# Rayhane-mamah/Tacotron-2

Measured on NVIDIA H100. Metric: wavenet_train_audio_samples_per_sec, higher is better.
Workload: dtype bf16

## Files before the change

### include/t2b200.h

```cpp
#ifndef T2B200_H_
#define T2B200_H_

#include <stdint.h>

#ifdef __cplusplus
extern "C" {
#endif

#define T2B200_ABI_VERSION 2

#define T2_OK 0
#define T2_ERR_INVALID_ARG (-1)
#define T2_ERR_UNSUPPORTED_SHAPE (-2)
#define T2_ERR_CUDA (-3)
#define T2_ERR_NCCL (-4)

const char* t2_last_error(void);
int t2_abi_version(void);
int t2_struct_size(const char* name);
long long t2_launch_count(void);

int t2_dbg_conv_gemm(const void* d_a, int B, int T, int C, int ld, const int* shifts, int nshift,
                     const void* d_w, int N, int BN, const float* d_bias, int relu, void* d_out_bf16,
                     float* d_out_f32, void* stream);
// ... 65 lines not shown
typedef struct {
  int layers, stacks, residual_channels, gate_channels, skip_out_channels, kernel_size;
  int cin_channels;
  int out_channels;
  int quantize_channels;
  int input_type;
  int legacy, residual_legacy;
  int upsample_type;
  int n_upsample;
  int upsample_scales[4];
  int freq_axis_kernel_size;
  float dropout;
  float log_scale_min;
  int B, T, Tc;
  int c_pre_upsampled;
  float log_scale_min_gauss;
  int cdf_loss;
  int split_bf16;
  int gin_channels;
  int n_speakers;
  int upsample_activation;
  float leaky_alpha;
} t2_wn_config_t;

typedef struct {
  long long n_params;
  long long packed_bytes;
  long long workspace_bytes;
  int n_tensors;
} t2_wn_sizes_t;

int t2_wn_sizes(const t2_wn_config_t* cfg, t2_wn_sizes_t* out);
int t2_wn_param_info(const t2_wn_config_t* cfg, int i, char* name, int name_cap, long long* offset, int* ndim,
                     int* shape4);
int t2_wn_init(const t2_wn_config_t* cfg, void* d_packed, void* d_workspace, void* stream);
int t2_wn_pack_weights(const t2_wn_config_t* cfg, const float* d_params, void* d_packed, void* d_workspace,
                       void* stream);
int t2_wn_forward(const t2_wn_config_t* cfg, const float* d_params, const void* d_packed, void* d_workspace,
                  const void* d_x, const float* d_c, const void* d_targets, const int* d_lengths, float* d_loss,
                  float* d_logits, int save_for_backward, unsigned long long seed,
                  const unsigned long long* d_step, void* stream);
int t2_wn_backward(const t2_wn_config_t* cfg, const float* d_params, const void* d_packed, void* d_workspace,
                   const void* d_x, const float* d_c, float* d_grads, unsigned long long seed,
                   const unsigned long long* d_step, void* stream);
int t2_wn_backward_phased(const t2_wn_config_t* cfg, const float* d_params, const void* d_packed, void* d_workspace,
                          const void* d_x, const float* d_c, float* d_grads, unsigned long long seed,
                          const unsigned long long* d_step, int phase, int n_groups, void* stream);
int t2_wn_time_kernel(const t2_wn_config_t* cfg, const float* d_params, const void* d_packed, void* d_workspace,
                      int which, int layer, int reps, float* ms_per_launch, void* stream);
int t2_wn_workspace_tensor(const t2_wn_config_t* cfg, void* d_workspace, const char* name, void** ptr,
                           long long* count, int* elem_bytes);
int t2_wn_set_speakers(const t2_wn_config_t* cfg, void* d_workspace, const int* d_speaker_ids, void* stream);
#define T2_DBG_WN_UP_FWD 1
#define T2_DBG_WN_UP_BWD_PARAM 2
#define T2_DBG_WN_UP_BWD_INPUT 3
int t2_dbg_wn_kernel(const t2_dbg_kernel_t* call, void* stream);


int t2_wn_ar_sizes(const t2_wn_config_t* cfg, int cluster_size, long long* packed_bytes, long long* workspace_bytes);
int t2_wn_ar_pack(const t2_wn_config_t* cfg, int cluster_size, const float* d_params, void* d_packed_ar,
                  void* d_workspace, void* stream);
int t2_wn_ar_generate(const t2_wn_config_t* cfg, int cluster_size, const float* d_params, const void* d_packed_ar,
                      void* d_workspace, const float* d_c, const void* d_initial, const void* d_test_inputs,
                      const float* d_u_a, const float* d_u_b, unsigned long long seed, void* d_out_samples,
                      float* d_out_raw, void* stream);
int t2_wn_ar_set_speakers(const t2_wn_config_t* cfg, int cluster_size, const float* d_params, const void* d_packed_ar,
                          void* d_workspace, const int* d_speaker_ids, void* stream);


typedef struct {
  int B, T_in, T_out;
  int n_symbols, num_mels, embedding_dim;
  int enc_conv_layers, enc_conv_kernel, enc_conv_channels, encoder_lstm_units;
  int attention_dim, attention_filters, attention_kernel;
  int prenet1, prenet2, decoder_lstm_units;
  int postnet_layers, postnet_kernel, postnet_channels;
  int clip_outputs;
  float dropout_rate;
  float zoneout_rate;
  float reg_weight;
  float max_abs_value, lower_bound_decay;
  int split_bf16;
  int mask_decoder;
  float cross_entropy_pos_weight;
  int unmasked_encoder;
  int noncumulative_weights;
  float teacher_forcing_ratio;
} t2_taco_config_t;

int t2_taco_sizes(const t2_taco_config_t* cfg, long long* n_params, long long* packed_bytes, long long* workspace_bytes,
                  int* n_tensors);
int t2_taco_param_info(const t2_taco_config_t* cfg, int i, char* name, int name_cap, long long* offset, int* ndim,
                       int* shape4, int* trainable);
int t2_taco_init(const t2_taco_config_t* cfg, void* d_packed, void* d_workspace, void* stream);
int t2_taco_pack_weights(const t2_taco_config_t* cfg, const float* d_params, void* d_packed, void* d_workspace, void* stream);
int t2_taco_forward(const t2_taco_config_t* cfg, float* d_params, const void* d_packed, void* d_workspace,
                    const int* d_inputs, const int* d_input_lengths, const float* d_mel_targets,
                    const float* d_stop_targets, float* d_loss, int training, unsigned long long seed,
                    const unsigned long long* d_step, void* stream);
int t2_taco_set_target_lengths(const t2_taco_config_t* cfg, void* d_workspace, const int* d_target_lengths, void* stream);
int t2_taco_backward(const t2_taco_config_t* cfg, const float* d_params, const void* d_packed, void* d_workspace,
                     const int* d_inputs, const int* d_input_lengths, const float* d_mel_targets,
                     const float* d_stop_targets, float* d_grads, unsigned long long seed,
                     const unsigned long long* d_step, void* stream);
int t2_taco_backward_ex(const t2_taco_config_t* cfg, const float* d_params, const void* d_packed, void* d_workspace,
                     const int* d_inputs, const int* d_input_lengths, const float* d_mel_targets,
                     const float* d_stop_targets, float* d_grads, const float* d_mel_outputs_grad, unsigned long long seed,
                     const unsigned long long* d_step, void* stream);
int t2_taco_infer_begin(const t2_taco_config_t* cfg, float* d_params, const void* d_packed, void* d_workspace,
                        const int* d_inputs, const int* d_input_lengths, void* stream);
int t2_taco_infer_steps(const t2_taco_config_t* cfg, float* d_params, const void* d_packed, void* d_workspace,
                        const int* d_input_lengths, int t_begin, int t_end, unsigned long long seed, void* stream);
int t2_taco_infer_finish(const t2_taco_config_t* cfg, float* d_params, const void* d_packed, void* d_workspace, int T_used,
                         void* stream);
int t2_rng_uniform_f32(unsigned long long seed, unsigned int stream_id, long long first_index, long long n, float* d_out,
                       void* stream);
int t2_dbg_att_stamps(long long* d_buf);
int t2_dbg_ar_stamps(long long* d_buf);
int t2_taco_workspace_tensor(const t2_taco_config_t* cfg, void* d_workspace, const char* name, void** ptr,
                             long long* count, int* elem_bytes);

typedef struct {
  int B, T;
  int num_mels;
  int kernels;
  int conv_channels;
  int pool_size;
  int projection;
  int projection_kernel_size;
  int highwaynet_layers;
  int highway_units;
  int rnn_units;
  int num_freq;
  int n_priority_freq;
  int clip_outputs, mask_decoder;
  float max_abs_value, lower_bound_decay, reg_weight;
} t2_cbhg_config_t;
int t2_cbhg_sizes(const t2_cbhg_config_t* cfg, long long* n_params, long long* packed_bytes, long long* workspace_bytes, int* n_tensors);
int t2_cbhg_param_info(const t2_cbhg_config_t* cfg, int i, char* name, int name_cap, long long* offset, int* ndim, int* shape4,
                       int* trainable);
int t2_cbhg_init(const t2_cbhg_config_t* cfg, void* d_packed, void* d_workspace, void* stream);
int t2_cbhg_pack_weights(const t2_cbhg_config_t* cfg, const float* d_params, void* d_packed, void* d_workspace, void* stream);
int t2_cbhg_set_target_lengths(const t2_cbhg_config_t* cfg, void* d_workspace, const int* d_target_lengths, void* stream);
int t2_cbhg_forward(const t2_cbhg_config_t* cfg, float* d_params, const void* d_packed, void* d_workspace, const float* d_mel,
                    const float* d_linear_targets, float* d_loss, int training, void* stream);
int t2_cbhg_backward(const t2_cbhg_config_t* cfg, const float* d_params, const void* d_packed, void* d_workspace, const float* d_mel,
                     float* d_grads, float* d_mel_grad, void* stream);
int t2_cbhg_workspace_tensor(const t2_cbhg_config_t* cfg, void* d_workspace, const char* name, void** ptr, long long* count);

int t2_adam_step(float* d_params, const float* d_grads, float* d_m, float* d_v, float* d_ema,
                 const long long* d_offsets, int n_tensors, long long n_total, float lr, float beta1, float beta2,
                 float eps, int step, float grad_scale, float max_norm, float max_value, float global_norm_clip,
                 float ema_decay, float* d_scratch, void* stream);

typedef struct {
  int sample_rate, n_fft, hop_size, win_size, num_mels;
  float fmin, fmax;
  float magnitude_power;
  float min_level_db, ref_level_db, max_abs_value;
  int symmetric_mels, allow_clipping_in_normalization, signal_normalization;
} t2_audio_config_t;

int t2_stft_mel_plan_bytes(const t2_audio_config_t* cfg, long long* bytes);
int t2_stft_mel_plan_init(const t2_audio_config_t* cfg, void* d_plan, void* stream);
int t2_stft_mel_frames(const t2_audio_config_t* cfg, int n_samples);
int t2_stft_mel_f32(const t2_audio_config_t* cfg, const void* d_plan, const float* d_wav, int B, int n_samples,
                    float preemphasis, float gain, float* d_mel, float* d_linear, int time_major, void* stream);
int t2_mel_basis_f64(const t2_audio_config_t* cfg, double* h_basis);
int t2_griffin_lim_bytes(const t2_audio_config_t* cfg, int B, int frames, long long* bytes);
int t2_griffin_lim_f32(const t2_audio_config_t* cfg, const void* d_plan, const float* d_mag, float* d_phase_io, int B, int frames,
                       int iters, unsigned long long seed, void* d_workspace, float* d_wav, void* stream);
int t2_preemphasis_f32(const float* d_x, float* d_y, int B, int n_samples, float k, void* stream);
int t2_mulaw_quantize_f32_i32(const float* d_in, int* d_out, long long n, void* stream);
int t2_inv_mulaw_quantize_i32_f32(const int* d_in, float* d_out, long long n, void* stream);
int t2_mulaw_f32(const float* d_in, float* d_out, long long n, void* stream);
int t2_inv_mulaw_f32(const float* d_in, float* d_out, long long n, void* stream);

#ifdef __cplusplus
}
#endif
#endif
```

### tacotron-2_b200/csrc/t2_common.cuh

```cuda
#pragma once
#include <cuda.h>
#include <cuda_bf16.h>
#include <cuda_runtime.h>
#include <stdint.h>

#define T2_OK 0
#define T2_ERR_INVALID_ARG (-1)
#define T2_ERR_UNSUPPORTED_SHAPE (-2)
#define T2_ERR_CUDA (-3)
#define T2_ERR_NCCL (-4)

int t2_set_error(int code, const char* fmt, ...);
void t2_count_launch(int n = 1);
#define T2_CHECK_CUDA(expr)                                                              \
  do {                                                                                   \
    cudaError_t _e = (expr);                                                             \
    if (_e != cudaSuccess)                                                               \
      return t2_set_error(T2_ERR_CUDA, "%s:%d %s -> %s", __FILE__, __LINE__, #expr,      \
                          cudaGetErrorString(_e));                                       \
  } while (0)
#define T2_REQUIRE(cond, code, ...)                                                      \
  do {                                                                                   \
    if (!(cond)) return t2_set_error(code, __VA_ARGS__);                                 \
  } while (0)

namespace t2 {

__device__ __forceinline__ uint32_t smem_u32(const void* p) {
  return static_cast<uint32_t>(__cvta_generic_to_shared(p));
}
__device__ __forceinline__ bool elect_one() {
  uint32_t pred = 0;
  asm volatile(
      "{\n\t.reg .pred P;\n\telect.sync _|P, 0xffffffff;\n\tselp.u32 %0, 1, 0, P;\n\t}\n"
      : "=r"(pred));
  return pred != 0;
}
__device__ __forceinline__ float warp_sum(float v) {
#pragma unroll
  for (int o = 16; o > 0; o >>= 1) v += __shfl_xor_sync(0xffffffffu, v, o);
  return v;
}
__device__ __forceinline__ float warp_max(float v) {
#pragma unroll
  for (int o = 16; o > 0; o >>= 1) v = fmaxf(v, __shfl_xor_sync(0xffffffffu, v, o));
  return v;
}
__device__ __forceinline__ float frcp_fast(float x) {
  float r;
  asm("rcp.approx.ftz.f32 %0, %1;" : "=f"(r) : "f"(x));
  return r;
}
__device__ __forceinline__ float sigmoidf_(float x) { return frcp_fast(1.f + __expf(-x)); }
__device__ __forceinline__ float tanhf_(float x) {
  const float e = __expf(-2.f * fabsf(x));
  const float t = (1.f - e) * frcp_fast(1.f + e);
  return copysignf(t, x);
}
__device__ __forceinline__ float tanh_approx_(float x) {
  float y;
  asm("tanh.approx.f32 %0, %1;" : "=f"(y) : "f"(x));
  return y;
}
__device__ __forceinline__ float sigmoid_approx_(float x) { return fmaf(0.5f, tanh_approx_(0.5f * x), 0.5f); }
__device__ __forceinline__ uint32_t pack_bf16x2(float lo, float hi) {
  __nv_bfloat162 v = __floats2bfloat162_rn(lo, hi);
  return *reinterpret_cast<uint32_t*>(&v);
}
__device__ __forceinline__ float bf16lo(uint32_t v) { return __uint_as_float(v << 16); }
__device__ __forceinline__ float bf16hi(uint32_t v) { return __uint_as_float(v & 0xffff0000u); }

__device__ __forceinline__ long long globaltimer_ns() {
  long long t;
  asm volatile("mov.u64 %0, %%globaltimer;" : "=l"(t));
  return t;
}
__device__ __forceinline__ long long smid() {
  unsigned int r;
  asm volatile("mov.u32 %0, %%smid;" : "=r"(r));
  return r;
}

__device__ __host__ __forceinline__ uint32_t hash_u32(uint64_t seed, uint64_t idx) {
  uint64_t z = seed + 0x9E3779B97F4A7C15ull * (idx + 1);
  z = (z ^ (z >> 30)) * 0xBF58476D1CE4E5B9ull;
  z = (z ^ (z >> 27)) * 0x94D049BB133111EBull;
  z = z ^ (z >> 31);
  return static_cast<uint32_t>(z >> 32);
}
__device__ __host__ __forceinline__ float hash_uniform(uint64_t seed, uint64_t idx) {
  return (hash_u32(seed, idx) >> 8) * (1.0f / 16777216.0f);
}
__device__ __host__ __forceinline__ uint32_t hash_seed(uint64_t seed, uint32_t stream) {
  return hash_u32(seed, stream);
}
__device__ __host__ __forceinline__ uint32_t hash_bits32(uint32_t hs, uint64_t idx) {
  uint32_t h = hs ^ (uint32_t(idx) * 0x9E3779B1u) ^ (uint32_t(idx >> 32) * 0x85EBCA77u);
  h ^= h >> 16; h *= 0x85EBCA6Bu; h ^= h >> 13; h *= 0xC2B2AE35u; h ^= h >> 16;
  return h;
}
__device__ __host__ __forceinline__ float hash_uniform32(uint32_t hs, uint64_t idx) {
  return (hash_bits32(hs, idx) >> 8) * (1.0f / 16777216.0f);
}
__device__ __host__ __forceinline__ bool hash_keep16(uint32_t hs, uint64_t idx, uint32_t thr16) {
  const uint32_t h = hash_bits32(hs, idx >> 1);
  return ((idx & 1) ? (h >> 16) : (h & 0xFFFFu)) >= thr16;
}

constexpr long long kFxPoison = -0x7fffffffffffffffll - 1;
constexpr long long kFxRange = 1ll << 62;
__device__ __forceinline__ bool fx_in_range(long long a) { return a > -kFxRange && a < kFxRange; }
struct FxAdd {
  unsigned long long* d;
  long long a, old;
};
__device__ __forceinline__ FxAdd fx_issue(long long* dst, float v) {
  FxAdd x{reinterpret_cast<unsigned long long*>(dst), 0, 0};
  if (!(fabsf(v) < 4194304.f)) {
    x.old = kFxPoison;
  } else {
    x.a = llrintf(v * 1099511627776.f);
    x.old = static_cast<long long>(atomicAdd(x.d, static_cast<unsigned long long>(x.a)));
  }
  return x;
}
__device__ __forceinline__ FxAdd fx_issue_total(long long* dst, long long v) {
  FxAdd x{reinterpret_cast<unsigned long long*>(dst), 0, kFxPoison};
  if (fx_in_range(v)) {
    x.a = v;
    x.old = static_cast<long long>(atomicAdd(x.d, static_cast<unsigned long long>(v)));
  }
  return x;
}
__device__ __forceinline__ void fx_check(const FxAdd& x) {
  if (!fx_in_range(x.old) || !fx_in_range(x.old + x.a)) atomicExch(x.d, static_cast<unsigned long long>(kFxPoison));
}
__device__ __forceinline__ void fx_add(long long* dst, float v) { fx_check(fx_issue(dst, v)); }
__device__ __forceinline__ float fx_value(long long a) {
  return fx_in_range(a) ? float(double(a) * (1.0 / 1099511627776.0)) : __int_as_float(0x7fffffff);
}
int launch_fx_finalize(const long long* acc, float* out, long long n, cudaStream_t st);

__device__ __forceinline__ void mbar_init(uint64_t* bar, uint32_t count) {
  asm volatile("mbarrier.init.shared::cta.b64 [%0], %1;\n" ::"r"(smem_u32(bar)), "r"(count));
}
__device__ __forceinline__ void fence_barrier_init() {
  asm volatile("fence.mbarrier_init.release.cluster;\n" ::: "memory");
}
__device__ __forceinline__ void fence_proxy_async() {
  asm volatile("fence.proxy.async.shared::cta;\n" ::: "memory");
}
__device__ __forceinline__ void mbar_expect_tx(uint64_t* bar, uint32_t bytes) {
  asm volatile("mbarrier.arrive.expect_tx.shared::cta.b64 _, [%0], %1;\n" ::"r"(smem_u32(bar)),
               "r"(bytes)
               : "memory");
}
__device__ __forceinline__ void mbar_arrive(uint64_t* bar) {
  asm volatile("mbarrier.arrive.shared::cta.b64 _, [%0];\n" ::"r"(smem_u32(bar)) : "memory");
}
__device__ __forceinline__ bool mbar_try_wait(uint64_t* bar, uint32_t parity) {
  uint32_t ok;
  asm volatile(
      "{\n\t.reg .pred P;\n\t"
      "mbarrier.try_wait.parity.shared::cta.b64 P, [%1], %2;\n\t"
      "selp.u32 %0, 1, 0, P;\n\t}\n"
      : "=r"(ok)
      : "r"(smem_u32(bar)), "r"(parity)
      : "memory");
  return ok != 0;
}
__device__ __forceinline__ void mbar_wait(uint64_t* bar, uint32_t parity) {
  while (!mbar_try_wait(bar, parity)) {
  }
}

__device__ __forceinline__ void tma_prefetch_desc(const CUtensorMap* m) {
  asm volatile("prefetch.tensormap [%0];\n" ::"l"(reinterpret_cast<uint64_t>(m)) : "memory");
}
__device__ __forceinline__ void tma_load_2d(void* smem, const CUtensorMap* m, uint64_t* bar, int c0,
                                            int c1) {
  asm volatile(
      "cp.async.bulk.tensor.2d.shared::cluster.global.tile.mbarrier::complete_tx::bytes "
      "[%0], [%1, {%3, %4}], [%2];\n" ::"r"(smem_u32(smem)),
      "l"(reinterpret_cast<uint64_t>(m)), "r"(smem_u32(bar)), "r"(c0), "r"(c1)
      : "memory");
}
__device__ __forceinline__ void tma_load_3d(void* smem, const CUtensorMap* m, uint64_t* bar, int c0,
                                            int c1, int c2) {
  asm volatile(
      "cp.async.bulk.tensor.3d.shared::cluster.global.tile.mbarrier::complete_tx::bytes "
      "[%0], [%1, {%3, %4, %5}], [%2];\n" ::"r"(smem_u32(smem)),
      "l"(reinterpret_cast<uint64_t>(m)), "r"(smem_u32(bar)), "r"(c0), "r"(c1), "r"(c2)
      : "memory");
}
__device__ __forceinline__ void tma_load_4d(void* smem, const CUtensorMap* m, uint64_t* bar, int c0,
                                            int c1, int c2, int c3) {
  asm volatile(
      "cp.async.bulk.tensor.4d.shared::cluster.global.tile.mbarrier::complete_tx::bytes "
      "[%0], [%1, {%3, %4, %5, %6}], [%2];\n" ::"r"(smem_u32(smem)),
      "l"(reinterpret_cast<uint64_t>(m)), "r"(smem_u32(bar)), "r"(c0), "r"(c1), "r"(c2), "r"(c3)
      : "memory");
}

__device__ __forceinline__ void tma_load_3d_mc(void* smem, const CUtensorMap* m, uint64_t* bar, int c0, int c1, int c2, uint16_t cta_mask) {
  asm volatile(
      "cp.async.bulk.tensor.3d.shared::cluster.global.tile.mbarrier::complete_tx::bytes.multicast::cluster "
      "[%0], [%1, {%3, %4, %5}], [%2], %6;\n" ::"r"(smem_u32(smem)),
      "l"(reinterpret_cast<uint64_t>(m)), "r"(smem_u32(bar)), "r"(c0), "r"(c1), "r"(c2), "h"(cta_mask)
      : "memory");
}
__device__ __forceinline__ void tma_store_3d(const CUtensorMap* m, const void* smem, int c0, int c1, int c2) {
  asm volatile("cp.async.bulk.tensor.3d.global.shared::cta.bulk_group [%0, {%2, %3, %4}], [%1];\n" ::"l"(reinterpret_cast<uint64_t>(m)),
               "r"(smem_u32(smem)), "r"(c0), "r"(c1), "r"(c2)
               : "memory");
}
__device__ __forceinline__ void bulk_commit() { asm volatile("cp.async.bulk.commit_group;\n" ::: "memory"); }
template <int N>
__device__ __forceinline__ void bulk_wait_read() { asm volatile("cp.async.bulk.wait_group.read %0;\n" ::"n"(N) : "memory"); }
__device__ __forceinline__ void bulk_wait_all() { asm volatile("cp.async.bulk.wait_group 0;\n" ::: "memory"); }
__device__ __forceinline__ void fence_proxy_async_smem() { asm volatile("fence.proxy.async.shared::cta;\n" ::: "memory"); }
__device__ __forceinline__ uint32_t mapa_cluster(const void* ptr, uint32_t rank) {
  uint32_t r;
  asm volatile("mapa.shared::cluster.u32 %0, %1, %2;" : "=r"(r) : "r"(smem_u32(ptr)), "r"(rank));
  return r;
}
__device__ __forceinline__ uint32_t cluster_ctarank() {
  uint32_t r;
  asm volatile("mov.u32 %0, %%cluster_ctarank;" : "=r"(r));
  return r;
}
__device__ __forceinline__ uint32_t cluster_nctarank() {
  uint32_t r;
  asm volatile("mov.u32 %0, %%cluster_nctarank;" : "=r"(r));
  return r;
}
__device__ __forceinline__ void cluster_sync_all() {
  asm volatile("barrier.cluster.arrive.release.aligned;\n" ::: "memory");
  asm volatile("barrier.cluster.wait.acquire.aligned;\n" ::: "memory");
}
__device__ __forceinline__ void mbar_arrive_cluster(uint64_t* bar, uint32_t rank) {
  asm volatile("mbarrier.arrive.release.cluster.shared::cluster.b64 _, [%0];\n" ::"r"(mapa_cluster(bar, rank)) : "memory");
}

__device__ __forceinline__ void bulk_load_1d(void* smem_dst, const void* gmem_src, uint32_t bytes, uint64_t* bar) {
  asm volatile("cp.async.bulk.shared::cluster.global.mbarrier::complete_tx::bytes [%0], [%1], %2, [%3];\n" ::"r"(smem_u32(smem_dst)),
               "l"(gmem_src), "r"(bytes), "r"(smem_u32(bar))
               : "memory");
}

__device__ __forceinline__ void pdl_wait() { asm volatile("griddepcontrol.wait;" ::: "memory"); }
__device__ __forceinline__ void pdl_launch_dependents() { asm volatile("griddepcontrol.launch_dependents;" ::: "memory"); }

__device__ __forceinline__ void wgmma_fence() { asm volatile("wgmma.fence.sync.aligned;\n" ::: "memory"); }
__device__ __forceinline__ void wgmma_commit() { asm volatile("wgmma.commit_group.sync.aligned;\n" ::: "memory"); }
template <int N>
__device__ __forceinline__ void wgmma_wait() { asm volatile("wgmma.wait_group.sync.aligned %0;\n" ::"n"(N) : "memory"); }
template <int R>
__device__ __forceinline__ void wgmma_fence_regs(float (&d)[R]) {
#pragma unroll
  for (int i = 0; i < R; ++i) asm volatile("" : "+f"(d[i])::"memory");
}
template <int N, int TA, int TB> struct Wgmma;
template <int TA, int TB>
struct Wgmma<16, TA, TB> {
  static __device__ __forceinline__ void mma(float (&d)[8], uint64_t da, uint64_t db, uint32_t scale_d) {
    asm volatile(
        "{\n.reg .pred p;\nsetp.ne.b32 p, %10, 0;\n"
        "wgmma.mma_async.sync.aligned.m64n16k16.f32.bf16.bf16 {"
        "%0, %1, %2, %3, %4, %5, %6, %7"
        "}, %8, %9, p, 1, 1, %11, %12;\n}\n"
        : "+f"(d[0]), "+f"(d[1]), "+f"(d[2]), "+f"(d[3]), "+f"(d[4]), "+f"(d[5]), "+f"(d[6]), "+f"(d[7])
        : "l"(da), "l"(db), "r"(scale_d), "n"(TA), "n"(TB));
  }
};
template <int TA, int TB>
struct Wgmma<64, TA, TB> {
  static __device__ __forceinline__ void mma(float (&d)[32], uint64_t da, uint64_t db, uint32_t scale_d) {
    asm volatile(
        "{\n.reg .pred p;\nsetp.ne.b32 p, %34, 0;\n"
        "wgmma.mma_async.sync.aligned.m64n64k16.f32.bf16.bf16 {"
        "%0, %1, %2, %3, %4, %5, %6, %7, %8, %9, %10, %11, %12, %13, %14, %15, "
        "%16, %17, %18, %19, %20, %21, %22, %23, %24, %25, %26, %27, %28, %29, %30, %31"
        "}, %32, %33, p, 1, 1, %35, %36;\n}\n"
        : "+f"(d[0]), "+f"(d[1]), "+f"(d[2]), "+f"(d[3]), "+f"(d[4]), "+f"(d[5]), "+f"(d[6]), "+f"(d[7]),
          "+f"(d[8]), "+f"(d[9]), "+f"(d[10]), "+f"(d[11]), "+f"(d[12]), "+f"(d[13]), "+f"(d[14]), "+f"(d[15]),
          "+f"(d[16]), "+f"(d[17]), "+f"(d[18]), "+f"(d[19]), "+f"(d[20]), "+f"(d[21]), "+f"(d[22]), "+f"(d[23]),
          "+f"(d[24]), "+f"(d[25]), "+f"(d[26]), "+f"(d[27]), "+f"(d[28]), "+f"(d[29]), "+f"(d[30]), "+f"(d[31])
        : "l"(da), "l"(db), "r"(scale_d), "n"(TA), "n"(TB));
  }
};
template <int TA, int TB>
struct Wgmma<128, TA, TB> {
  static __device__ __forceinline__ void mma(float (&d)[64], uint64_t da, uint64_t db, uint32_t scale_d) {
    asm volatile(
// ... 92 lines not shown
```

### tacotron-2_b200/csrc/t2_optim.cu

```cuda
#include "../../include/t2b200.h"
#include "t2_common.cuh"

namespace t2 {
namespace {

__device__ __forceinline__ int find_tensor(const long long* __restrict__ offs, int n, long long e) {
  int lo = 0, hi = n;
  while (hi - lo > 1) {
    const int mid = (lo + hi) >> 1;
    if (offs[mid] <= e) lo = mid; else hi = mid;
  }
  return lo;
}

__global__ void sumsq_kernel(const float* __restrict__ g, const long long* __restrict__ offs, int nt, long long n,
                             float gscale, float* __restrict__ norms) {
  const long long chunk = 4096;
  const long long e0 = blockIdx.x * chunk;
  const long long e1 = e0 + chunk < n ? e0 + chunk : n;
  int t = find_tensor(offs, nt, e0);
  float acc = 0.f;
  __shared__ float red[8];
  long long e = e0 + threadIdx.x;
  while (true) {
    const long long tend = offs[t + 1] < e1 ? offs[t + 1] : e1;
    acc = 0.f;
    for (; e < tend; e += blockDim.x) {
      const float v = g[e] * gscale;
      acc += v * v;
    }
    acc = warp_sum(acc);
    if ((threadIdx.x & 31) == 0) red[threadIdx.x >> 5] = acc;
    __syncthreads();
    if (threadIdx.x == 0) {
      float s = 0.f;
      for (int i = 0; i < (blockDim.x >> 5); ++i) s += red[i];
      if (s != 0.f) atomicAdd(norms + t, s);
    }
    __syncthreads();
    if (tend >= e1) break;
    ++t;
    e = offs[t] + threadIdx.x;
  }
}

struct AdamArgs {
  float* p; const float* g; float* m; float* v; float* ema;
  const long long* offs; int nt; long long n;
  float lr_t, b1, b2, eps, gscale, max_norm, max_value, gclip, ema_decay;
  const float* norms;
};
__global__ void adam_kernel(AdamArgs a) {
  const long long e = (blockIdx.x * (long long)blockDim.x + threadIdx.x) * 4;
  if (e >= a.n) return;
  float gs = a.gscale;
  if (a.gclip > 0.f) {
    gs *= a.gclip / fmaxf(sqrtf(a.norms[a.nt]), a.gclip);
  } else if (a.max_norm > 0.f) {
    const int t = find_tensor(a.offs, a.nt, e);
    gs *= a.max_norm / fmaxf(sqrtf(a.norms[t]), a.max_norm);
  }
  const float4 g4 = *reinterpret_cast<const float4*>(a.g + e);
  float4 m4 = *reinterpret_cast<const float4*>(a.m + e);
  float4 v4 = *reinterpret_cast<const float4*>(a.v + e);
  float4 p4 = *reinterpret_cast<const float4*>(a.p + e);
  float4 e4 = a.ema ? *reinterpret_cast<const float4*>(a.ema + e) : make_float4(0, 0, 0, 0);
  float* gp = const_cast<float*>(reinterpret_cast<const float*>(&g4));
  float* mp = reinterpret_cast<float*>(&m4);
  float* vp = reinterpret_cast<float*>(&v4);
  float* pp = reinterpret_cast<float*>(&p4);
  float* ep = reinterpret_cast<float*>(&e4);
#pragma unroll
  for (int i = 0; i < 4; ++i) {
    float g = gp[i] * gs;
    if (a.max_value > 0.f) g = fminf(fmaxf(g, -a.max_value), a.max_value);
    mp[i] = a.b1 * mp[i] + (1.f - a.b1) * g;
    vp[i] = a.b2 * vp[i] + (1.f - a.b2) * g * g;
    pp[i] = pp[i] - a.lr_t * mp[i] / (sqrtf(vp[i]) + a.eps);
    ep[i] -= (1.f - a.ema_decay) * (ep[i] - pp[i]);
  }
  *reinterpret_cast<float4*>(a.m + e) = m4;
  *reinterpret_cast<float4*>(a.v + e) = v4;
  *reinterpret_cast<float4*>(a.p + e) = p4;
  if (a.ema) *reinterpret_cast<float4*>(a.ema + e) = e4;
}
__global__ void total_kernel(float* norms, int nt) {
  float s = 0.f;
  for (int i = threadIdx.x; i < nt; i += 32) s += norms[i];
  s = warp_sum(s);
  if (threadIdx.x == 0) norms[nt] = s;
}

}
}

extern "C" int t2_adam_step(float* d_params, const float* d_grads, float* d_m, float* d_v, float* d_ema,
                            const long long* d_offsets, int n_tensors, long long n_total, float lr, float beta1,
                            float beta2, float eps, int step, float grad_scale, float max_norm, float max_value,
                            float global_norm_clip, float ema_decay, float* d_scratch, void* stream) {
  using namespace t2;
  T2_REQUIRE(d_params && d_grads && d_m && d_v && d_offsets && d_scratch, T2_ERR_INVALID_ARG, "adam: null pointer");
  T2_REQUIRE(step >= 1 && n_tensors >= 1 && n_total >= 1, T2_ERR_INVALID_ARG, "adam: bad step / sizes");
  cudaStream_t st = static_cast<cudaStream_t>(stream);
  const bool need_norms = max_norm > 0.f || global_norm_clip > 0.f;
  if (need_norms) {
    T2_CHECK_CUDA(cudaMemsetAsync(d_scratch, 0, (n_tensors + 1) * sizeof(float), st));
    sumsq_kernel<<<(unsigned)((n_total + 4095) / 4096), 256, 0, st>>>(d_grads, d_offsets, n_tensors, n_total, grad_scale, d_scratch); t2_count_launch();
    if (global_norm_clip > 0.f) total_kernel<<<1, 32, 0, st>>>(d_scratch, n_tensors); t2_count_launch();
  }
  AdamArgs a;
  a.p = d_params; a.g = d_grads; a.m = d_m; a.v = d_v; a.ema = d_ema; a.offs = d_offsets; a.nt = n_tensors; a.n = n_total;
  a.lr_t = float(double(lr) * sqrt(1.0 - pow(double(beta2), step)) / (1.0 - pow(double(beta1), step)));
  a.b1 = beta1; a.b2 = beta2; a.eps = eps; a.gscale = grad_scale; a.max_norm = max_norm; a.max_value = max_value;
  a.gclip = global_norm_clip; a.ema_decay = ema_decay; a.norms = d_scratch;
  T2_REQUIRE(n_total % 4 == 0, T2_ERR_INVALID_ARG, "adam: flat buffers must hold a multiple of 4 elements (16-byte aligned tensors)");
  adam_kernel<<<(unsigned)((n_total / 4 + 255) / 256), 256, 0, st>>>(a); t2_count_launch();
  T2_CHECK_CUDA(cudaGetLastError());
  return T2_OK;
}
```

### tacotron-2_b200/csrc/t2_wavenet.cu

```cuda
#include <stdlib.h>
#include <math.h>
#include <stdio.h>
#include <string.h>

#include <algorithm>
#include <string>
#include <vector>

#include "../../include/t2b200.h"
#include "t2_common.cuh"
#include "t2_gemm.h"

namespace t2 {
namespace {

typedef __nv_bfloat16 bf16;

struct PackJob {
  long long src_off;
  int K, N;
  long long dst_off;
  int dst_ld;
  int transpose;
  int col0;
  float scale;
  int perm_gh;
  int part;
};
struct ColsumJob {
  long long src_off;
  long long rows;
  int C, ld;
  long long dst_off, dst2_off;
  float scale;
  int div_scalar;
};

inline long long align_up(long long v, long long a) { return (v + a - 1) / a * a; }

struct ParamT {
  std::string name;
  long long off;
  int ndim;
  int shape[4];
};

struct Layout {
  t2_wn_config_t c;
  int L, R, G, Gh, S, C, O, Q, B, T, Tc, Kg, ldo, Op;
  bool split;
  int xm;
  bool scalar_in, mol, gauss;
  int Gi, NS;
  float res_scale;
  std::vector<float> skip_scale;
  std::vector<ParamT> params;
  long long n_params;
  long long p_in_k, p_in_b, p_f1_k, p_f1_b, p_f2_k, p_f2_b;
  std::vector<long long> p_dil_k, p_dil_b, p_c_k, p_c_b, p_s_k, p_s_b, p_o_k, p_o_b, p_up_k, p_up_b;
  std::vector<long long> p_g_k, p_g_b;
  long long p_emb;
  long long layer_stride;
  long long k_Wg, k_Wo, k_Ws, k_Wf1, k_Wf2, k_WozT, k_WdT, k_WcT, k_Wf1T, k_Wf2T, k_bias_g, k_bias_skip;
  long long packed_bytes;
  long long w_cup, w_x, w_xd, w_ta, w_sb, w_z, w_h1, w_h2, w_dlog, w_dh2, w_dskip, w_dxin, w_dg, w_dcup;
  long long w_skipsum;
  long long w_spk;
  long long w_gbias;
  long long w_gsum;
  long long w_gfx;
  long long w_upgrad[2], w_scalars, w_tiles_main, w_tiles_head, w_packjobs, w_colsum, w_tables;
  std::vector<long long> w_upout;
  std::vector<int> up_w;
  long long workspace_bytes;
  int n_tiles_main, n_tiles_head, n_packjobs, n_colsum;
  std::vector<PackJob> packjobs;
  std::vector<ColsumJob> colsums;
  std::vector<WgradTile> tiles_main, tiles_head;
  std::vector<int> tile_start;
  int dil(int l) const { return 1 << (l % (L / c.stacks)); }
};

long long add_param(Layout& lo, const std::string& name, std::initializer_list<int> shape) {
  ParamT p;
  p.name = name;
  p.off = lo.n_params;
  p.ndim = int(shape.size());
  long long n = 1;
  int i = 0;
  for (int s : shape) { p.shape[i++] = s; n *= s; }
  for (; i < 4; ++i) p.shape[i] = 1;
  lo.n_params += align_up(n, 4);
  lo.params.push_back(p);
  return p.off;
}

int build_layout(const t2_wn_config_t* cfg, Layout& lo) {
  T2_REQUIRE(cfg != nullptr, T2_ERR_INVALID_ARG, "null config");
  lo.c = *cfg;
  lo.L = cfg->layers; lo.R = cfg->residual_channels; lo.G = cfg->gate_channels; lo.Gh = lo.G / 2;
  lo.S = cfg->skip_out_channels; lo.C = cfg->cin_channels; lo.O = cfg->out_channels;
  lo.Q = cfg->quantize_channels; lo.B = cfg->B; lo.T = cfg->T; lo.Tc = cfg->Tc;
  lo.split = cfg->split_bf16 != 0;
  lo.xm = lo.split ? 2 : 1;
  T2_REQUIRE(!lo.split || cfg->dropout == 0.f, T2_ERR_INVALID_ARG, "split_bf16 (fp32-class forward) needs dropout = 0");
  lo.scalar_in = cfg->input_type != 2;
  lo.mol = lo.scalar_in;
  T2_REQUIRE(lo.L >= 1 && cfg->stacks >= 1 && lo.L % cfg->stacks == 0, T2_ERR_INVALID_ARG, "layers %% stacks != 0");
  T2_REQUIRE(cfg->kernel_size == 3, T2_ERR_UNSUPPORTED_SHAPE, "kernel_size must be 3");
  T2_REQUIRE(lo.R == 128 || lo.R == 256, T2_ERR_UNSUPPORTED_SHAPE, "residual_channels must be 128 or 256 (got %d)", lo.R);
  T2_REQUIRE(lo.S == 128 || lo.S == 256, T2_ERR_UNSUPPORTED_SHAPE, "skip_out_channels must be 128 or 256 (got %d)", lo.S);
  T2_REQUIRE(lo.Gh == 128 || lo.Gh == 256, T2_ERR_UNSUPPORTED_SHAPE, "gate_channels must be 256 or 512 (got %d)", lo.G);
  T2_REQUIRE(lo.C == 0 || (lo.C % 8 == 0 && lo.C <= 128), T2_ERR_UNSUPPORTED_SHAPE, "cin_channels must be 0 or a multiple of 8 <= 128");
  lo.gauss = lo.scalar_in && lo.O == 2;
  if (lo.mol) {
    T2_REQUIRE(lo.gauss || (lo.O % 3 == 0 && lo.O >= 3 && lo.O <= 30), T2_ERR_UNSUPPORTED_SHAPE,
               "scalar input needs out_channels = 2 (Gaussian) or 3 * nr_mix <= 30 (mixture of logistics), got %d", lo.O);
  } else {
    T2_REQUIRE(lo.O == 256 && lo.Q == 256, T2_ERR_UNSUPPORTED_SHAPE, "mulaw-quantize needs out_channels == quantize_channels == 256");
  }
  T2_REQUIRE(lo.B >= 1 && lo.T >= 1, T2_ERR_INVALID_ARG, "bad B/T");
  lo.Gi = cfg->gin_channels; lo.NS = cfg->n_speakers;
  T2_REQUIRE(lo.Gi >= 0 && (lo.Gi == 0 || lo.NS >= 1), T2_ERR_INVALID_ARG,
             "gin_channels must be >= 0, and n_speakers >= 1 when gin_channels > 0 (got %d / %d)", lo.Gi, lo.NS);
  T2_REQUIRE(cfg->upsample_type >= 0 && cfg->upsample_type <= 2, T2_ERR_INVALID_ARG,
             "upsample_type must be 0 (SubPixel), 1 (2D) or 2 (1D), got %d", cfg->upsample_type);
  T2_REQUIRE(cfg->upsample_activation >= 0 && cfg->upsample_activation <= 2, T2_ERR_INVALID_ARG,
             "upsample_activation must be 0 (ReLU), 1 (LeakyReLU) or 2 (none), got %d", cfg->upsample_activation);
  T2_REQUIRE(cfg->leaky_alpha >= 0.f && cfg->leaky_alpha <= 1.f, T2_ERR_INVALID_ARG, "leaky_alpha must be in [0, 1], got %g",
             double(cfg->leaky_alpha));
  lo.Kg = 3 * lo.R + (lo.C > 0 ? 128 : 0);
  lo.ldo = lo.mol ? 64 : 512;
  lo.Op = lo.mol ? 64 : 512;
  lo.res_scale = cfg->residual_legacy ? float(sqrt(0.5)) : 1.f;
  lo.skip_scale.resize(lo.L);
  for (int l = 0; l < lo.L; ++l) {
    int e = cfg->legacy ? (l == 0 ? lo.L - 1 : lo.L - l) : 0;
    lo.skip_scale[l] = float(pow(sqrt(0.5), e));
  }
  lo.up_w.clear();
  if (lo.C > 0 && !cfg->c_pre_upsampled) {
    T2_REQUIRE(cfg->n_upsample >= 1 && cfg->n_upsample <= 4, T2_ERR_INVALID_ARG, "n_upsample out of range");
    T2_REQUIRE(cfg->upsample_type == 2 || cfg->freq_axis_kernel_size == 3, T2_ERR_UNSUPPORTED_SHAPE,
               "freq_axis_kernel_size must be 3");
    for (int i = 0; i < cfg->n_upsample; ++i)
      T2_REQUIRE(cfg->upsample_scales[i] >= 1, T2_ERR_INVALID_ARG, "upsample_scales[%d] = %d < 1", i, cfg->upsample_scales[i]);
    int w = lo.Tc;
    for (int i = 0; i < cfg->n_upsample; ++i) { w *= cfg->upsample_scales[i]; lo.up_w.push_back(w); }
    T2_REQUIRE(w == lo.T, T2_ERR_INVALID_ARG, "Tc * prod(upsample_scales) = %d != T = %d", w, lo.T);
  }
  lo.n_params = 0;
  lo.params.clear();
  const int cin = lo.scalar_in ? 1 : lo.Q;
  lo.p_in_k = add_param(lo, "input_convolution/kernel", {1, cin, lo.R});
  lo.p_in_b = add_param(lo, "input_convolution/bias", {lo.R});
  for (int l = 0; l < lo.L; ++l) {
    char p[64];
    snprintf(p, sizeof(p), "ResidualConv1DGLU_%d/", l);
    std::string s(p);
    lo.p_dil_k.push_back(add_param(lo, s + "residual_block_causal_conv/kernel", {3, lo.R, lo.G}));
    lo.p_dil_b.push_back(add_param(lo, s + "residual_block_causal_conv/bias", {lo.G}));
    if (lo.C > 0) {
      lo.p_c_k.push_back(add_param(lo, s + "residual_block_cin_conv/kernel", {1, lo.C, lo.G}));
      lo.p_c_b.push_back(add_param(lo, s + "residual_block_cin_conv/bias", {lo.G}));
    }
    if (lo.Gi > 0) {
      lo.p_g_k.push_back(add_param(lo, s + "residual_block_gin_conv/kernel", {1, lo.Gi, lo.G}));
      lo.p_g_b.push_back(add_param(lo, s + "residual_block_gin_conv/bias", {lo.G}));
    }
    lo.p_s_k.push_back(add_param(lo, s + "residual_block_skip_conv/kernel", {1, lo.Gh, lo.S}));
    lo.p_s_b.push_back(add_param(lo, s + "residual_block_skip_conv/bias", {lo.S}));
    lo.p_o_k.push_back(add_param(lo, s + "residual_block_out_conv/kernel", {1, lo.Gh, lo.R}));
    lo.p_o_b.push_back(add_param(lo, s + "residual_block_out_conv/bias", {lo.R}));
  }
  lo.p_f1_k = add_param(lo, "final_convolution_1/kernel", {1, lo.S, lo.S});
  lo.p_f1_b = add_param(lo, "final_convolution_1/bias", {lo.S});
  lo.p_f2_k = add_param(lo, "final_convolution_2/kernel", {1, lo.S, lo.O});
  lo.p_f2_b = add_param(lo, "final_convolution_2/bias", {lo.O});
  lo.p_emb = lo.Gi > 0 ? add_param(lo, "gc_embedding", {lo.NS, lo.Gi}) : -1;
  lo.layer_stride = lo.L > 1 ? lo.p_dil_k[1] - lo.p_dil_k[0] : 0;
  for (size_t i = 0; i < lo.up_w.size(); ++i) {
    char p[64];
    snprintf(p, sizeof(p), "local_conditioning_upsampling_%d/", int(i) + 1);
    std::string s(p);
    const int sc = cfg->upsample_scales[i];
    if (cfg->upsample_type == 0) {
      lo.p_up_k.push_back(add_param(lo, s + "kernel", {3, 3, 1, sc}));
      lo.p_up_b.push_back(add_param(lo, s + "bias", {sc}));
    } else if (cfg->upsample_type == 2) {
      lo.p_up_k.push_back(add_param(lo, s + "kernel", {1, sc, lo.C, lo.C}));
      lo.p_up_b.push_back(add_param(lo, s + "bias", {lo.C}));
    } else {
      lo.p_up_k.push_back(add_param(lo, s + "kernel", {3, sc, 1, 1}));
      lo.p_up_b.push_back(add_param(lo, s + "bias", {1}));
    }
  }
  long long o = 0;
  auto takeb = [&](long long bytes) { long long r = o; o = align_up(o + bytes, 256); return r; };
  const long long L = lo.L;
  const long long km = lo.split ? 3 : 1;
  lo.k_Wg = takeb(L * lo.G * lo.Kg * km * 2);
  lo.k_Wo = takeb(L * lo.R * lo.Gh * km * 2);
  lo.k_Ws = takeb((long long)lo.S * L * lo.Gh * km * 2);
  lo.k_Wf1 = takeb((long long)lo.S * lo.S * km * 2);
  lo.k_Wf2 = takeb((long long)(lo.O < 32 ? 32 : lo.O) * lo.S * km * 2);
  lo.k_WozT = takeb(L * lo.Gh * (lo.R + lo.S) * 2);
  lo.k_WdT = takeb(L * lo.R * 3 * lo.G * 2);
  lo.k_WcT = takeb((long long)(lo.C > 0 ? lo.C : 8) * L * lo.G * 2);
  lo.k_Wf1T = takeb((long long)lo.S * lo.S * 2);
  lo.k_Wf2T = takeb((long long)lo.S * lo.Op * 2);
  lo.k_bias_g = takeb(L * lo.G * 4);
  lo.k_bias_skip = takeb(lo.S * 4);
  lo.packed_bytes = o;
  o = 0;
  const long long BT = (long long)lo.B * lo.T;
  lo.w_cup = takeb(BT * (lo.split ? 256 : (lo.C > 0 ? lo.C : 8)) * 2);
  lo.w_upout.clear();
  for (size_t i = 0; i < lo.up_w.size(); ++i) lo.w_upout.push_back(takeb((long long)lo.B * lo.C * lo.up_w[i] * 4));
  lo.w_upgrad[0] = takeb(BT * (lo.C > 0 ? lo.C : 8) * 4);
  lo.w_upgrad[1] = takeb(BT * (lo.C > 0 ? lo.C : 8) * 4);
  lo.w_x = takeb(L * BT * lo.R * 2 * lo.xm);
  lo.w_xd = cfg->dropout > 0.f ? takeb(L * BT * lo.R * 2) : lo.w_x;
  lo.w_ta = takeb(L * BT * lo.Gh * 2);
  lo.w_sb = takeb(L * BT * lo.Gh * 2);
  lo.w_z = takeb(L * BT * lo.Gh * 2 * lo.xm);
  lo.w_h1 = takeb(BT * lo.S * 2 * lo.xm);
  lo.w_h2 = takeb(BT * lo.S * 2 * lo.xm);
  lo.w_dlog = takeb(BT * lo.ldo * 2);
  lo.w_dh2 = takeb(BT * lo.S * 2);
  lo.w_dskip = takeb(BT * lo.S * 2);
  lo.w_dxin = takeb(L * BT * lo.R * 2);
  lo.w_dg = takeb(L * BT * lo.G * 2);
  lo.w_dcup = takeb(BT * (lo.C > 0 ? lo.C : 8) * 4);
  lo.w_scalars = takeb(64 * 4);
  lo.w_skipsum = takeb(lo.S * 8);
  lo.w_gfx = takeb(lo.n_params * 8);

  lo.packjobs.clear();
  auto pj = [&](long long src, int K, int N, long long dst_bytes, int ld, int transpose, int col0, float scale, int perm) {
    PackJob j; j.src_off = src; j.K = K; j.N = N; j.dst_off = dst_bytes / 2; j.dst_ld = ld; j.transpose = transpose;
    j.col0 = col0; j.scale = scale; j.perm_gh = perm; j.part = 0; lo.packjobs.push_back(j);
  };
  auto pj3 = [&](long long src, int K, int N, long long dst_bytes, int ld, int col_hi, int col_lo, int slot, float scale, int perm) {
    pj(src, K, N, dst_bytes, ld, 1, col_hi, scale, perm);
    pj(src, K, N, dst_bytes, ld, 1, col_hi + slot, scale, perm);
    pj(src, K, N, dst_bytes, ld, 1, col_lo, scale, perm);
    lo.packjobs.back().part = 2;
  };
  for (int l = 0; l < lo.L; ++l) {
    const long long wg = lo.k_Wg + (long long)l * lo.G * lo.Kg * km * 2;
    if (lo.split) {
      const int R = lo.R, Gh = lo.Gh;
      for (int j = 0; j < 3; ++j) pj3(lo.p_dil_k[l] + (long long)j * R * lo.G, R, lo.G, wg, 3 * lo.Kg, j * 3 * R, j * 3 * R + 2 * R, R, 1.f, Gh);
      if (lo.C > 0) pj3(lo.p_c_k[l], lo.C, lo.G, wg, 3 * lo.Kg, 9 * R, 9 * R + 256, 128, 1.f, Gh);
      pj3(lo.p_o_k[l], Gh, R, lo.k_Wo + (long long)l * R * Gh * 3 * 2, 3 * Gh, 0, 2 * Gh, Gh, 1.f, 0);
      pj3(lo.p_s_k[l], Gh, lo.S, lo.k_Ws, 3 * lo.L * Gh, l * 2 * Gh, 2 * lo.L * Gh + l * Gh, Gh, lo.skip_scale[l], 0);
    } else {
    for (int j = 0; j < 3; ++j) pj(lo.p_dil_k[l] + (long long)j * lo.R * lo.G, lo.R, lo.G, wg, lo.Kg, 1, j * lo.R, 1.f, lo.Gh);
    if (lo.C > 0) pj(lo.p_c_k[l], lo.C, lo.G, wg, lo.Kg, 1, 3 * lo.R, 1.f, lo.Gh);
    pj(lo.p_o_k[l], lo.Gh, lo.R, lo.k_Wo + (long long)l * lo.R * lo.Gh * 2, lo.Gh, 1, 0, 1.f, 0);
    pj(lo.p_s_k[l], lo.Gh, lo.S, lo.k_Ws, lo.L * lo.Gh, 1, l * lo.Gh, lo.skip_scale[l], 0);
    }
    const long long woz = lo.k_WozT + (long long)l * lo.Gh * (lo.R + lo.S) * 2;
    pj(lo.p_o_k[l], lo.Gh, lo.R, woz, lo.R + lo.S, 0, 0, lo.res_scale, 0);
    pj(lo.p_s_k[l], lo.Gh, lo.S, woz, lo.R + lo.S, 0, lo.R, lo.skip_scale[l], 0);
    const long long wd = lo.k_WdT + (long long)l * lo.R * 3 * lo.G * 2;
    for (int j = 0; j < 3; ++j) pj(lo.p_dil_k[l] + (long long)j * lo.R * lo.G, lo.R, lo.G, wd, 3 * lo.G, 0, j * lo.G, 1.f, 0);
    if (lo.C > 0) pj(lo.p_c_k[l], lo.C, lo.G, lo.k_WcT, lo.L * lo.G, 0, l * lo.G, 1.f, 0);
  }
  if (lo.split) {
    pj3(lo.p_f1_k, lo.S, lo.S, lo.k_Wf1, 3 * lo.S, 0, 2 * lo.S, lo.S, 1.f, 0);
    pj3(lo.p_f2_k, lo.S, lo.O, lo.k_Wf2, 3 * lo.S, 0, 2 * lo.S, lo.S, 1.f, 0);
  } else {
    pj(lo.p_f1_k, lo.S, lo.S, lo.k_Wf1, lo.S, 1, 0, 1.f, 0);
    pj(lo.p_f2_k, lo.S, lo.O, lo.k_Wf2, lo.S, 1, 0, 1.f, 0);
  }
  pj(lo.p_f1_k, lo.S, lo.S, lo.k_Wf1T, lo.S, 0, 0, 1.f, 0);
  pj(lo.p_f2_k, lo.S, lo.O, lo.k_Wf2T, lo.Op, 0, 0, 1.f, 0);
  if (!lo.mol) pj(lo.p_f2_k, lo.S, lo.O, lo.k_Wf2T, lo.Op, 0, 256, 1.f, 0);
  lo.n_packjobs = int(lo.packjobs.size());

  lo.tiles_main.clear();
  auto wt = [&](std::vector<WgradTile>& v, int am, int ach, int ash, int al, int bm, int bch, int bl, long long off,
                int ldc, int mv, int nv, float scale, const float* div) {
    WgradTile t; memset(&t, 0, sizeof(t));
    t.a_map = am; t.a_ch0 = ach; t.a_shift = ash; t.a_layer = al; t.b_map = bm; t.b_ch0 = bch; t.b_shift = 0; t.b_layer = bl;
    t.out_off = off; t.ldc = ldc; t.m_valid = mv; t.n_valid = nv; t.scale = scale; t.accumulate = 0; t.div = div;
    v.push_back(t);
  };
  const int WN = 256;
  auto nmin = [&](int rem) { return rem < WN ? rem : WN; };
  lo.tile_start.assign(lo.L + 1, 0);
  for (int l = 0; l < lo.L; ++l) {
    const int d = lo.dil(l);
    lo.tile_start[l] = int(lo.tiles_main.size());
    for (int j = 0; j < 3; ++j)
      for (int m0 = 0; m0 < lo.R; m0 += 128)
        for (int n0 = 0; n0 < lo.G; n0 += WN)
          wt(lo.tiles_main, 0, m0, -(2 - j) * d, l, 1, n0, l, lo.p_dil_k[l] + (long long)j * lo.R * lo.G + (long long)m0 * lo.G + n0,
             lo.G, 128, nmin(lo.G - n0), 1.f, nullptr);
    if (lo.C > 0)
      for (int n0 = 0; n0 < lo.G; n0 += WN)
        wt(lo.tiles_main, 2, 0, 0, 0, 1, n0, l, lo.p_c_k[l] + n0, lo.G, lo.C, nmin(lo.G - n0), 1.f, nullptr);
    for (int m0 = 0; m0 < lo.Gh; m0 += 128) {
      if (l < lo.L - 1)
        for (int n0 = 0; n0 < lo.R; n0 += WN)
          wt(lo.tiles_main, 3, m0, 0, l, 4, n0, l + 1, lo.p_o_k[l] + (long long)m0 * lo.R + n0, lo.R, 128, nmin(lo.R - n0), lo.res_scale, nullptr);
      for (int n0 = 0; n0 < lo.S; n0 += WN)
        wt(lo.tiles_main, 3, m0, 0, l, 5, n0, 0, lo.p_s_k[l] + (long long)m0 * lo.S + n0, lo.S, 128, nmin(lo.S - n0), lo.skip_scale[l], nullptr);
    }
  }
  lo.tiles_head.clear();
  for (int m0 = 0; m0 < lo.S; m0 += 128) {
    for (int n0 = 0; n0 < lo.S; n0 += WN)
      wt(lo.tiles_head, 0, m0, 0, 0, 1, n0, 0, lo.p_f1_k + (long long)m0 * lo.S + n0, lo.S, 128, nmin(lo.S - n0), 1.f, nullptr);
    for (int n0 = 0; n0 < lo.O; n0 += WN)
      for (int part = 0; part < (lo.mol ? 1 : 2); ++part) {
        wt(lo.tiles_head, 2, m0, 0, 0, 3, part * 256 + n0, 0, lo.p_f2_k + (long long)m0 * lo.O + n0, lo.O, 128,
           nmin(lo.O - n0), 1.f, reinterpret_cast<const float*>(1) );
        lo.tiles_head.back().accumulate = 2;
      }
  }
  lo.n_tiles_main = int(lo.tiles_main.size());
  lo.tile_start[lo.L] = lo.n_tiles_main;
  lo.n_tiles_head = int(lo.tiles_head.size());

  lo.colsums.clear();
  auto cs = [&](long long src, long long rows, int C, int ld, long long dst, long long dst2, float scale, int div) {
    ColsumJob j; j.src_off = src; j.rows = rows; j.C = C; j.ld = ld; j.dst_off = dst; j.dst2_off = dst2; j.scale = scale;
    j.div_scalar = div; lo.colsums.push_back(j);
  };
  cs(lo.w_dlog, BT, lo.O, lo.ldo, lo.p_f2_b, -1, 1.f, 1);
  if (!lo.mol) cs(lo.w_dlog + 256 * 2, BT, lo.O, lo.ldo, lo.p_f2_b, -1, 1.f, 1);
  lo.n_colsum = int(lo.colsums.size());

  lo.w_tiles_main = takeb((long long)lo.n_tiles_main * sizeof(WgradTile));
  lo.w_tiles_head = takeb((long long)lo.n_tiles_head * sizeof(WgradTile));
  lo.w_packjobs = takeb((long long)lo.n_packjobs * sizeof(PackJob));
  lo.w_colsum = takeb((long long)lo.n_colsum * sizeof(ColsumJob));
  lo.w_tables = takeb((long long)lo.L * (3 * sizeof(long long) + sizeof(float)));
  lo.w_spk = lo.w_gbias = lo.w_gsum = -1;
  if (lo.Gi > 0) {
    lo.w_spk = takeb((1LL + lo.B) * 4);
    lo.w_gbias = takeb(L * lo.B * lo.G * 4);
    lo.w_gsum = takeb(L * lo.B * lo.G * 8);
  }
  lo.workspace_bytes = o;
  return T2_OK;
}

__global__ void pack_kernel(const float* __restrict__ params, bf16* __restrict__ packed, const PackJob* __restrict__ jobs) {
  __shared__ float tile[64][65];
  const PackJob j = jobs[blockIdx.y];
  const int tiles_n = (j.N + 63) / 64, tiles_k = (j.K + 63) / 64;
  const int tx = threadIdx.x, ty = threadIdx.y;
  const bool vec_src = ((j.N | int(j.src_off)) & 1) == 0;
  const bool vec_dst = ((j.dst_ld | j.col0 | int(j.dst_off)) & 1) == 0;
  for (int ti = blockIdx.x; ti < tiles_n * tiles_k; ti += gridDim.x) {
    const int k0 = (ti / tiles_n) * 64, n0 = (ti % tiles_n) * 64;
    for (int r = ty; r < 64; r += 8) {
      const int k = k0 + r, n = n0 + 2 * tx;
      float a = 0.f, b = 0.f;
      if (k < j.K) {
        const float* src = params + j.src_off + (long long)k * j.N + n;
        if (vec_src && n + 1 < j.N) { const float2 v = *reinterpret_cast<const float2*>(src); a = v.x; b = v.y; }
        else { if (n < j.N) a = src[0]; if (n + 1 < j.N) b = src[1]; }
      }
      a *= j.scale; b *= j.scale;
      if (j.part == 2) { a -= __bfloat162float(__float2bfloat16(a)); b -= __bfloat162float(__float2bfloat16(b)); }
      tile[r][2 * tx] = a; tile[r][2 * tx + 1] = b;
    }
    __syncthreads();
    if (j.transpose) {
      for (int r = ty; r < 64; r += 8) {
        const int n = n0 + r, k = k0 + 2 * tx;
        if (n < j.N && k < j.K) {
          int row = n;
          if (j.perm_gh > 0) {
            const int half = n / j.perm_gh, idx = n % j.perm_gh;
            row = (idx / 128) * 256 + half * 128 + (idx % 128);
          }
          bf16* dst = packed + j.dst_off + (long long)row * j.dst_ld + j.col0 + k;
          if (vec_dst && k + 1 < j.K) *reinterpret_cast<uint32_t*>(dst) = pack_bf16x2(tile[2 * tx][r], tile[2 * tx + 1][r]);
          else { dst[0] = __float2bfloat16(tile[2 * tx][r]); if (k + 1 < j.K) dst[1] = __float2bfloat16(tile[2 * tx + 1][r]); }
        }
      }
    } else {
      for (int r = ty; r < 64; r += 8) {
        const int k = k0 + r, n = n0 + 2 * tx;
        if (n < j.N && k < j.K) {
          bf16* dst = packed + j.dst_off + (long long)k * j.dst_ld + j.col0 + n;
          if (vec_dst && n + 1 < j.N) *reinterpret_cast<uint32_t*>(dst) = pack_bf16x2(tile[r][2 * tx], tile[r][2 * tx + 1]);
          else { dst[0] = __float2bfloat16(tile[r][2 * tx]); if (n + 1 < j.N) dst[1] = __float2bfloat16(tile[r][2 * tx + 1]); }
        }
      }
    }
    __syncthreads();
  }
}

struct DerivedArgs {
  const float* params;
  float* bias_g;
  float* bias_skip;
  const long long* offs;
  const float* scales;
  int L, G, S;
};
__global__ void derived_bias_kernel(DerivedArgs a) {
  const int i = blockIdx.x * blockDim.x + threadIdx.x;
  if (i < a.L * a.G) {
    const int l = i / a.G, g = i % a.G;
    float v = a.params[a.offs[3 * l] + g];
    if (a.offs[3 * l + 1] >= 0) v += a.params[a.offs[3 * l + 1] + g];
    a.bias_g[i] = v;
  }
  if (i < a.S) {
    float v = 0.f;
    for (int l = 0; l < a.L; ++l) v += a.scales[l] * a.params[a.offs[3 * l + 2] + i];
    a.bias_skip[i] = v;
  }
}

struct GinArgs {
  const float* params;
  const float* bias;
  long long bias_ld;
  const int* on;
  const int* ids;
  float* out;
  long long out_l, out_b;
  long long p_k, p_b, p_stride, p_emb;
  int L, B, G, Gi, NS;
};
__global__ void gin_bias_kernel(GinArgs a) {
  const long long i = blockIdx.x * (long long)blockDim.x + threadIdx.x;
  if (i >= (long long)a.L * a.B * a.G) return;
  const int g = int(i % a.G), b = int((i / a.G) % a.B), l = int(i / ((long long)a.G * a.B));
  float v = a.bias[l * a.bias_ld + g];
  if (a.ids && (!a.on || *a.on)) {
    const int id = a.ids[b];
    float s = __int_as_float(0x7fffffff);
    if (id >= 0 && id < a.NS) {
      const float* W = a.params + a.p_k + l * a.p_stride + g;
      const float* e = a.params + a.p_emb + (long long)id * a.Gi;
      s = a.params[a.p_b + l * a.p_stride + g];
      for (int k = 0; k < a.Gi; ++k) s += W[(long long)k * a.G] * e[k];
    }
    v += s;
  }
  a.out[l * a.out_l + b * a.out_b + g] = v;
}
__global__ void set_speakers_kernel(int* __restrict__ spk, const int* __restrict__ ids, int B) {
  const int i = blockIdx.x * blockDim.x + threadIdx.x;
  if (i == 0) spk[0] = ids != nullptr;
  if (ids && i < B) spk[1 + i] = ids[i];
}
struct GinGradArgs {
  const float* params;
  const int* spk;
  const long long* S;
  long long* gfx;
  float* grads;
  const long long* offs;
  long long p_k, p_b, p_stride, p_emb;
  int L, B, G, Gi, NS;
};
__global__ void gin_wgrad_kernel(GinGradArgs a) {
  const int i = blockIdx.x * blockDim.x + threadIdx.x;
  if (i >= a.L * a.G) return;
  const int l = i / a.G, g = i % a.G;
  const long long* S = a.S + (long long)l * a.B * a.G + g;
  long long tot = 0;
  bool poison = false;
  for (int b = 0; b < a.B; ++b) {
    const long long s = S[(long long)b * a.G];
    if (!fx_in_range(s)) poison = true;
    else if (!fx_in_range(tot += s)) poison = true;
  }
  if (poison) tot = kFxPoison;
  a.gfx[a.offs[3 * l] + g] = tot;
  if (a.offs[3 * l + 1] >= 0) a.gfx[a.offs[3 * l + 1] + g] = tot;
  if (!a.spk[0]) return;
  a.gfx[a.p_b + l * a.p_stride + g] = tot;
  float* dW = a.grads + a.p_k + l * a.p_stride + g;
  for (int k = 0; k < a.Gi; ++k) {
    float acc = 0.f;
    for (int b = 0; b < a.B; ++b) {
      const int id = a.spk[1 + b];
      const float e = (id >= 0 && id < a.NS) ? a.params[a.p_emb + (long long)id * a.Gi + k] : __int_as_float(0x7fffffff);
      acc += e * fx_value(S[(long long)b * a.G]);
    }
    dW[(long long)k * a.G] = acc;
  }
}
constexpr int kGinThreads = 256;
__global__ void __launch_bounds__(kGinThreads) gin_demb_kernel(GinGradArgs a) {
  __shared__ float red[kGinThreads];
  if (!a.spk[0]) return;
  const int s = blockIdx.x, k = blockIdx.y, tid = threadIdx.x;
  {
    float acc = 0.f;
    for (int b = 0; b < a.B; ++b) {
      if (a.spk[1 + b] != s) continue;
      float part = 0.f;
      for (int l = 0; l < a.L; ++l) {
        const float* W = a.params + a.p_k + l * a.p_stride + (long long)k * a.G;
        const long long* S = a.S + ((long long)l * a.B + b) * a.G;
        for (int g = tid; g < a.G; g += kGinThreads) part += W[g] * fx_value(S[g]);
      }
      red[tid] = part;
      __syncthreads();
      for (int h = kGinThreads / 2; h > 0; h >>= 1) {
        if (tid < h) red[tid] += red[tid + h];
        __syncthreads();
      }
      if (tid == 0) acc += red[0];
      __syncthreads();
    }
    if (tid == 0) a.grads[a.p_emb + (long long)s * a.Gi + k] = acc;
  }
}

__global__ void first_conv_kernel(const void* __restrict__ xin, int scalar_in, const float* __restrict__ W,
                                  const float* __restrict__ bias, bf16* __restrict__ x, bf16* __restrict__ xd,
                                  long long npos, int R, float p, unsigned long long seed,
                                  const unsigned long long* __restrict__ step, int split) {
  if (step) seed += *step;
  const long long e8 = blockIdx.x * (long long)blockDim.x + threadIdx.x;
  const int R8 = R >> 3;
  if (e8 >= npos * R8) return;
  const long long pos = e8 / R8;
  const int r = int(e8 % R8) * 8;
  float v[8];
  const float4 b0 = __ldg(reinterpret_cast<const float4*>(bias + r)), b1 = __ldg(reinterpret_cast<const float4*>(bias + r + 4));
  if (scalar_in) {
    const float xv = static_cast<const float*>(xin)[pos];
    const float4 w0 = __ldg(reinterpret_cast<const float4*>(W + r)), w1 = __ldg(reinterpret_cast<const float4*>(W + r + 4));
    v[0] = xv * w0.x + b0.x; v[1] = xv * w0.y + b0.y; v[2] = xv * w0.z + b0.z; v[3] = xv * w0.w + b0.w;
    v[4] = xv * w1.x + b1.x; v[5] = xv * w1.y + b1.y; v[6] = xv * w1.z + b1.z; v[7] = xv * w1.w + b1.w;
  } else {
    const float* row = W + (long long)static_cast<const int*>(xin)[pos] * R + r;
    const float4 w0 = __ldg(reinterpret_cast<const float4*>(row)), w1 = __ldg(reinterpret_cast<const float4*>(row + 4));
    v[0] = w0.x + b0.x; v[1] = w0.y + b0.y; v[2] = w0.z + b0.z; v[3] = w0.w + b0.w;
    v[4] = w1.x + b1.x; v[5] = w1.y + b1.y; v[6] = w1.z + b1.z; v[7] = w1.w + b1.w;
  }
  const long long e = pos * R + r;
  uint4 o;
  if (split) {
    float hi[8], lo8[8];
#pragma unroll
    for (int j = 0; j < 8; ++j) { hi[j] = __bfloat162float(__float2bfloat16(v[j])); lo8[j] = v[j] - hi[j]; }
    o.x = pack_bf16x2(hi[0], hi[1]); o.y = pack_bf16x2(hi[2], hi[3]); o.z = pack_bf16x2(hi[4], hi[5]); o.w = pack_bf16x2(hi[6], hi[7]);
    *reinterpret_cast<uint4*>(x + pos * 2 * R + r) = o;
    o.x = pack_bf16x2(lo8[0], lo8[1]); o.y = pack_bf16x2(lo8[2], lo8[3]); o.z = pack_bf16x2(lo8[4], lo8[5]); o.w = pack_bf16x2(lo8[6], lo8[7]);
    *reinterpret_cast<uint4*>(x + pos * 2 * R + R + r) = o;
    return;
  }
  o.x = pack_bf16x2(v[0], v[1]); o.y = pack_bf16x2(v[2], v[3]); o.z = pack_bf16x2(v[4], v[5]); o.w = pack_bf16x2(v[6], v[7]);
  *reinterpret_cast<uint4*>(x + e) = o;
  if (xd != x && xd != nullptr) {
    const float keep_inv = 1.f / (1.f - p);
    const uint32_t hs = hash_seed(seed, 0u), thr = uint32_t(p * 65536.f);
#pragma unroll
    for (int j = 0; j < 8; ++j) v[j] = hash_keep16(hs, (unsigned long long)(e + j), thr) ? v[j] * keep_inv : 0.f;
    o.x = pack_bf16x2(v[0], v[1]); o.y = pack_bf16x2(v[2], v[3]); o.z = pack_bf16x2(v[4], v[5]); o.w = pack_bf16x2(v[6], v[7]);
    *reinterpret_cast<uint4*>(xd + e) = o;
  }
}
__global__ void first_conv_bwd_kernel(const void* __restrict__ xin, int scalar_in, const bf16* __restrict__ dx0,
                                      long long* __restrict__ dW, long long npos, int R) {
  const int r = threadIdx.x;
  const long long p0 = (long long)blockIdx.x * 64;
  if (scalar_in) {
    float acc = 0.f;
    for (int i = 0; i < 64 && p0 + i < npos; ++i)
      acc += static_cast<const float*>(xin)[p0 + i] * __bfloat162float(dx0[(p0 + i) * R + r]);
    fx_add(dW + r, acc);
  } else {
    const int n = npos - p0 < 64 ? int(npos - p0) : 64;
    for (int i0 = 0; i0 < n; i0 += 8) {
      FxAdd x[8];
#pragma unroll
      for (int i = 0; i < 8; ++i)
        if (i0 + i < n)
          x[i] = fx_issue(dW + (long long)static_cast<const int*>(xin)[p0 + i0 + i] * R + r, __bfloat162float(dx0[(p0 + i0 + i) * R + r]));
#pragma unroll
      for (int i = 0; i < 8; ++i)
        if (i0 + i < n) fx_check(x[i]);
    }
  }
}

__global__ void colsum_kernel(const uint8_t* __restrict__ ws, long long* __restrict__ grads, const ColsumJob* __restrict__ jobs,
                              const float* __restrict__ scalars) {
  const ColsumJob j = jobs[blockIdx.y];
  const bf16* src = reinterpret_cast<const bf16*>(ws + j.src_off);
  const long long rows_per = (j.rows + gridDim.x - 1) / gridDim.x;
  const long long r0 = blockIdx.x * rows_per;
  const long long r1 = r0 + rows_per < j.rows ? r0 + rows_per : j.rows;
  float sc = j.scale;
  if (j.div_scalar >= 0) sc /= fmaxf(scalars[j.div_scalar], 1e-20f);
  for (int c = 2 * threadIdx.x; c < j.C; c += 2 * blockDim.x) {
    float a0 = 0.f, a1 = 0.f;
    long long r = r0;
    for (; r + 4 <= r1; r += 4) {
      uint32_t u[4];
#pragma unroll
      for (int i = 0; i < 4; ++i) u[i] = __ldg(reinterpret_cast<const uint32_t*>(src + (r + i) * j.ld + c));
#pragma unroll
      for (int i = 0; i < 4; ++i) { a0 += bf16lo(u[i]); a1 += bf16hi(u[i]); }
    }
    for (; r < r1; ++r) {
      const uint32_t u = __ldg(reinterpret_cast<const uint32_t*>(src + r * j.ld + c));
      a0 += bf16lo(u); a1 += bf16hi(u);
    }
    a0 *= sc; a1 *= sc;
    const bool two = c + 1 < j.C, dup = j.dst2_off >= 0;
    FxAdd x[4];
    x[0] = fx_issue(grads + j.dst_off + c, a0);
    if (two) x[1] = fx_issue(grads + j.dst_off + c + 1, a1);
    if (dup) {
      x[2] = fx_issue(grads + j.dst2_off + c, a0);
      if (two) x[3] = fx_issue(grads + j.dst2_off + c + 1, a1);
    }
    fx_check(x[0]);
    if (two) fx_check(x[1]);
    if (dup) {
      fx_check(x[2]);
      if (two) fx_check(x[3]);
    }
  }
}

__device__ __forceinline__ float up_act(float x, int act, float alpha) {
  return act == 0 ? fmaxf(x, 0.f) : act == 1 ? fmaxf(alpha * x, x) : x;
}
// ... 209 lines not shown
        const float v = up_act(bias[co] + acc[k], act, alpha);
        out[((long long)b * C + co) * Wo + xo] = v;
        if (out_cl && split) {
          const bf16 hi = __float2bfloat16(v);
          bf16* row = out_cl + ((long long)b * Wo + xo) * 256;
          row[co] = hi;
          row[128 + co] = __float2bfloat16(v - __bfloat162float(hi));
        } else if (out_cl) out_cl[((long long)b * Wo + xo) * C + co] = __float2bfloat16(v);
      }
    }
  }
}
__global__ void __launch_bounds__(kUp1Tw * kUp1Rows) up1d_bwd_input_kernel(const float* __restrict__ out, const float* __restrict__ dout,
                                                                          const float* __restrict__ K, float* __restrict__ din, int C, int W,
                                                                          int s, int act, float alpha) {
  extern __shared__ float sm[];
  float* kt = sm;
  float* gs = sm + C * C;
  const int tx = threadIdx.x, ty = threadIdx.y, tid = ty * kUp1Tw + tx;
  const int w0 = blockIdx.x * kUp1Tw, b = blockIdx.y;
  const int nw = min(kUp1Tw, W - w0);
  const long long Wo = (long long)W * s;
  float acc[kUp1MaxK];
#pragma unroll
  for (int k = 0; k < kUp1MaxK; ++k) acc[k] = 0.f;
  for (int j = 0; j < s; ++j) {
    __syncthreads();
    const float* Kj = K + (long long)j * C * C;
    for (int e = tid; e < C * C; e += kUp1Tw * kUp1Rows) kt[e] = Kj[(e % C) * C + e / C];
    for (int e = tid; e < C * kUp1Tw; e += kUp1Tw * kUp1Rows) {
      const int co = e / kUp1Tw, t = e % kUp1Tw;
      float g = 0.f;
      if (t < nw) {
        const long long i = ((long long)b * C + co) * Wo + (long long)(w0 + t) * s + j;
        g = up_dact(out[i], dout[i], act, alpha);
      }
      gs[e] = g;
    }
    __syncthreads();
    if ((C & 3) == 0) {
      for (int co = 0; co < C; co += 4) {
        const float g0 = gs[co * kUp1Tw + tx], g1 = gs[(co + 1) * kUp1Tw + tx], g2 = gs[(co + 2) * kUp1Tw + tx], g3 = gs[(co + 3) * kUp1Tw + tx];
#pragma unroll
        for (int k = 0; k < kUp1MaxK; ++k) {
          const int ci = ty + kUp1Rows * k;
          if (ci < C) {
            const float4 kv = *reinterpret_cast<const float4*>(kt + ci * C + co);
            acc[k] = fmaf(kv.x, g0, acc[k]); acc[k] = fmaf(kv.y, g1, acc[k]); acc[k] = fmaf(kv.z, g2, acc[k]); acc[k] = fmaf(kv.w, g3, acc[k]);
          }
        }
      }
    } else {
      for (int co = 0; co < C; ++co) {
        const float g = gs[co * kUp1Tw + tx];
#pragma unroll
        for (int k = 0; k < kUp1MaxK; ++k) {
          const int ci = ty + kUp1Rows * k;
          if (ci < C) acc[k] = fmaf(kt[ci * C + co], g, acc[k]);
        }
      }
    }
  }
  if (tx < nw) {
#pragma unroll
    for (int k = 0; k < kUp1MaxK; ++k) {
      const int ci = ty + kUp1Rows * k;
      if (ci < C) din[((long long)b * C + ci) * W + w0 + tx] = acc[k];
    }
  }
}
constexpr int kUp1MaxM = 4;
inline size_t up1d_param_smem(int C) { return sizeof(float) * 2 * kUp1Tw * size_t(C + 1); }
__global__ void __launch_bounds__(kUp1Tw * kUp1Rows) up1d_bwd_param_kernel(const float* __restrict__ in, const float* __restrict__ out,
                                                                          const float* __restrict__ dout, long long* __restrict__ dK,
                                                                          long long* __restrict__ dbias, int B, int C, int W, int s, int act,
                                                                          float alpha) {
  extern __shared__ float sm[];
  const int ld = C + 1;
  float* xs = sm;
  float* gs = sm + kUp1Tw * ld;
  const int tx = threadIdx.x, ty = threadIdx.y, tid = ty * kUp1Tw + tx;
  const int j = blockIdx.x;
  const long long npos = (long long)B * W, Wo = (long long)W * s;
  const long long nchunk = (npos + kUp1Tw - 1) / kUp1Tw;
  float acc[kUp1MaxM][kUp1MaxK];
#pragma unroll
  for (int m = 0; m < kUp1MaxM; ++m)
#pragma unroll
    for (int k = 0; k < kUp1MaxK; ++k) acc[m][k] = 0.f;
  float bsum = 0.f;
  for (long long ch = blockIdx.y; ch < nchunk; ch += gridDim.y) {
    __syncthreads();
    for (int e = tid; e < C * kUp1Tw; e += kUp1Tw * kUp1Rows) {
      const int c = e / kUp1Tw, t = e % kUp1Tw;
      const long long p = ch * kUp1Tw + t;
      float x = 0.f, g = 0.f;
      if (p < npos) {
        const long long b = p / W, w = p % W;
        x = in[(b * C + c) * W + w];
        const long long i = (b * C + c) * Wo + w * s + j;
        g = up_dact(out[i], dout[i], act, alpha);
      }
      xs[t * ld + c] = x;
      gs[t * ld + c] = g;
    }
    __syncthreads();
    if (tid < C)
      for (int t = 0; t < kUp1Tw; ++t) bsum += gs[t * ld + tid];
    for (int t = 0; t < kUp1Tw; ++t) {
      float x[kUp1MaxM];
#pragma unroll
      for (int m = 0; m < kUp1MaxM; ++m) x[m] = tx + kUp1Tw * m < C ? xs[t * ld + tx + kUp1Tw * m] : 0.f;
#pragma unroll
      for (int k = 0; k < kUp1MaxK; ++k) {
        const int co = ty + kUp1Rows * k;
        if (co < C) {
          const float g = gs[t * ld + co];
#pragma unroll
          for (int m = 0; m < kUp1MaxM; ++m) acc[m][k] = fmaf(g, x[m], acc[m][k]);
        }
      }
    }
  }
  long long* dKj = dK + (long long)j * C * C;
#pragma unroll
  for (int k = 0; k < kUp1MaxK; ++k) {
    const int co = ty + kUp1Rows * k;
    if (co >= C) continue;
    FxAdd xa[kUp1MaxM];
#pragma unroll
    for (int m = 0; m < kUp1MaxM; ++m) {
      const int ci = tx + kUp1Tw * m;
      if (ci < C && acc[m][k] != 0.f) xa[m] = fx_issue(dKj + (long long)co * C + ci, acc[m][k]);
    }
#pragma unroll
    for (int m = 0; m < kUp1MaxM; ++m) {
      const int ci = tx + kUp1Tw * m;
      if (ci < C && acc[m][k] != 0.f) fx_check(xa[m]);
    }
  }
  if (tid < C && bsum != 0.f) fx_add(dbias + tid, bsum);
}
__global__ void skip_bias_kernel(const long long* __restrict__ skipsum, float* __restrict__ grads, const long long* __restrict__ offs,
                                 const float* __restrict__ scales, int L, int S) {
  const int i = blockIdx.x * blockDim.x + threadIdx.x;
  if (i >= L * S) return;
  const int l = i / S, s = i % S;
  grads[offs[3 * l + 2] + s] = scales[l] * fx_value(skipsum[s]);
}
__global__ void fx_finalize_kernel(const long long* __restrict__ acc, float* __restrict__ grads, long long n) {
  const long long e = blockIdx.x * (long long)blockDim.x + threadIdx.x;
  if (e < n && acc[e] != 0) grads[e] += fx_value(acc[e]);
}
__global__ void f32_to_bf16_kernel(const float* __restrict__ in, bf16* __restrict__ out, long long n) {
  const long long e = blockIdx.x * (long long)blockDim.x + threadIdx.x;
  if (e < n) out[e] = __float2bfloat16(in[e]);
}

ActGemmCall make_gate_call(const Layout& lo, uint8_t* ws, const uint8_t* pk, int l, bool save) {
  const long long BT = (long long)lo.B * lo.T;
  const int d = lo.dil(l);
  ActGemmCall g;
  memset(&g, 0, sizeof(g));
  if (lo.split) {
    g.a[0] = make_act(ws + lo.w_xd, 2 * lo.R, lo.T, lo.B, lo.L);
    g.a[1] = make_act(ws + lo.w_cup, 256, lo.T, lo.B, 1);
    g.na = lo.C > 0 ? 2 : 1;
    const int shifts[3] = {-2 * d, -d, 0};
    g.nseg = 0;
    for (int j = 0; j < 3; ++j) {
      g.seg[g.nseg++] = Seg{0, shifts[j], 0, 2 * lo.R / kBK, l, 1};
      g.seg[g.nseg++] = Seg{0, shifts[j], 0, lo.R / kBK, l, 1};
    }
    if (lo.C > 0) { g.seg[g.nseg++] = Seg{1, 0, 0, 4, 0, 1}; g.seg[g.nseg++] = Seg{1, 0, 0, 2, 0, 1}; }
    g.w = pk + lo.k_Wg; g.wN = lo.G; g.wK = 3 * lo.Kg; g.wL = lo.L; g.w_layer = l; g.w_k0 = 0;
  } else {
  g.a[0] = make_act(ws + lo.w_xd, lo.R, lo.T, lo.B, lo.L);
  g.a[1] = make_act(ws + lo.w_cup, lo.C > 0 ? lo.C : 8, lo.T, lo.B, 1);
  g.na = lo.C > 0 ? 2 : 1;
  g.seg[0] = Seg{0, -2 * d, 0, lo.R / kBK, l, 1};
  g.seg[1] = Seg{0, -d, 0, lo.R / kBK, l, 1};
  g.seg[2] = Seg{0, 0, 0, lo.R / kBK, l, 1};
  g.nseg = 3;
  if (lo.C > 0) { g.seg[3] = Seg{1, 0, 0, 2, 0, 1}; g.nseg = 4; }
  g.w = pk + lo.k_Wg; g.wN = lo.G; g.wK = lo.Kg; g.wL = lo.L; g.w_layer = l; g.w_k0 = 0;
  }
  g.T = lo.T; g.B = lo.B; g.n_tiles = lo.G / 256;
  const long long lofs = (long long)l * BT * lo.Gh;
  g.epi.ptr[0] = save ? reinterpret_cast<bf16*>(ws + lo.w_ta) + lofs : nullptr;
  g.epi.ptr[1] = save ? reinterpret_cast<bf16*>(ws + lo.w_sb) + lofs : nullptr;
  g.epi.ptr[2] = reinterpret_cast<bf16*>(ws + lo.w_z) + lofs * lo.xm;
  g.epi.i[11] = lo.split ? 1 : 0;
  g.epi.ptr[3] = const_cast<float*>(reinterpret_cast<const float*>(pk + lo.k_bias_g) + (long long)l * lo.G);
  if (lo.Gi > 0) {
    g.epi.ptr[3] = reinterpret_cast<float*>(ws + lo.w_gbias) + (long long)l * lo.B * lo.G;
    g.epi.i[2] = lo.G;
  }
  g.epi.i[0] = lo.Gh;
  return g;
}

ActGemmCall make_out_call(const Layout& lo, uint8_t* ws, const uint8_t* pk, const float* params, int l, float p,
                          unsigned long long seed, const unsigned long long* d_step) {
  const long long BT = (long long)lo.B * lo.T;
  bf16* x_all = reinterpret_cast<bf16*>(ws + lo.w_x);
  bf16* xd_all = reinterpret_cast<bf16*>(ws + lo.w_xd);
  ActGemmCall o;
  memset(&o, 0, sizeof(o));
  o.a[0] = make_act(ws + lo.w_z, lo.Gh * lo.xm, lo.T, lo.B, lo.L); o.na = 1;
  o.seg[0] = Seg{0, 0, 0, lo.Gh * lo.xm / kBK, l, 1}; o.nseg = 1;
  if (lo.split) { o.seg[1] = Seg{0, 0, 0, lo.Gh / kBK, l, 1}; o.nseg = 2; }
  o.w = pk + lo.k_Wo; o.wN = lo.R; o.wK = lo.Gh * (lo.split ? 3 : 1); o.wL = lo.L; o.w_layer = l;
  o.T = lo.T; o.B = lo.B; o.n_tiles = 1;
  o.epi.ptr[0] = x_all + (long long)l * BT * lo.R * lo.xm;
  o.epi.ptr[1] = x_all + (long long)(l + 1) * BT * lo.R * lo.xm;
  o.epi.i[11] = lo.split ? 1 : 0;
  o.epi.ptr[2] = p > 0.f ? xd_all + (long long)(l + 1) * BT * lo.R : nullptr;
  o.epi.ptr[3] = const_cast<float*>(params + lo.p_o_b[l]);
  o.epi.f[0] = lo.res_scale; o.epi.f[1] = p; o.epi.i[1] = l + 1; o.epi.seed = seed;
  o.epi.ptr[7] = const_cast<unsigned long long*>(d_step);
  return o;
}

ActGemmCall make_dz_call(const Layout& lo, uint8_t* ws, const uint8_t* pk, int l, long long* grads) {
  const long long BT = (long long)lo.B * lo.T;
  const bool top = l == lo.L - 1;
  ActGemmCall g;
  memset(&g, 0, sizeof(g));
  g.a[0] = make_act(ws + lo.w_dxin, lo.R, lo.T, lo.B, lo.L);
  g.a[1] = make_act(ws + lo.w_dskip, lo.S, lo.T, lo.B, 1);
  g.na = 2;
  if (top) {
    g.seg[0] = Seg{1, 0, 0, lo.S / kBK, 0, 1}; g.nseg = 1; g.w_k0 = lo.R;
  } else {
    g.seg[0] = Seg{0, 0, 0, lo.R / kBK, l + 1, 1};
    g.seg[1] = Seg{1, 0, 0, lo.S / kBK, 0, 1};
    g.nseg = 2; g.w_k0 = 0;
  }
  const int bn_z = lo.Gh >= 256 ? 256 : 128;
  g.w = pk + lo.k_WozT; g.wN = lo.Gh; g.wK = lo.R + lo.S; g.wL = lo.L; g.w_layer = l;
  g.T = lo.T; g.B = lo.B; g.n_tiles = lo.Gh / bn_z;
  const long long lofs = (long long)l * BT * lo.Gh;
  g.epi.ptr[0] = reinterpret_cast<bf16*>(ws + lo.w_ta) + lofs;
  g.epi.ptr[1] = reinterpret_cast<bf16*>(ws + lo.w_sb) + lofs;
  g.epi.ptr[2] = reinterpret_cast<bf16*>(ws + lo.w_dg) + (long long)l * BT * lo.G;
  g.epi.ptr[3] = grads ? grads + lo.p_dil_b[l] : nullptr;
  g.epi.ptr[4] = (grads && lo.C > 0) ? grads + lo.p_c_b[l] : nullptr;
  if (grads && lo.Gi > 0) {
    g.epi.ptr[3] = reinterpret_cast<long long*>(ws + lo.w_gsum) + (long long)l * lo.B * lo.G;
    g.epi.ptr[4] = nullptr;
    g.epi.i[1] = lo.G;
  }
  g.epi.i[0] = lo.Gh;
  return g;
}

ActGemmCall make_dx_call(const Layout& lo, uint8_t* ws, const uint8_t* pk, int l, float p, unsigned long long seed,
                         const unsigned long long* d_step, long long* grads) {
  const long long BT = (long long)lo.B * lo.T;
  const int d = lo.dil(l);
  const bool top = l == lo.L - 1;
  bf16* dxin = reinterpret_cast<bf16*>(ws + lo.w_dxin);
  ActGemmCall g;
  memset(&g, 0, sizeof(g));
  g.a[0] = make_act(ws + lo.w_dg, lo.G, lo.T, lo.B, lo.L); g.na = 1;
  for (int j = 0; j < 3; ++j) g.seg[j] = Seg{0, (2 - j) * d, 0, lo.G / kBK, l, 1};
  g.nseg = 3;
  g.w = pk + lo.k_WdT; g.wN = lo.R; g.wK = 3 * lo.G; g.wL = lo.L; g.w_layer = l;
  g.T = lo.T; g.B = lo.B; g.n_tiles = 1;
  g.epi.ptr[0] = top ? nullptr : dxin + (long long)(l + 1) * BT * lo.R;
  g.epi.ptr[1] = dxin + (long long)l * BT * lo.R;
  g.epi.f[0] = lo.res_scale; g.epi.f[1] = p; g.epi.i[1] = l; g.epi.seed = seed;
  g.epi.ptr[7] = const_cast<unsigned long long*>(d_step);
  g.epi.ptr[2] = grads ? grads + (l > 0 ? lo.p_o_b[l - 1] : lo.p_in_b) : nullptr;
  g.epi.f[2] = l > 0 ? lo.res_scale : 1.f;
  return g;
}

inline dim3 grid1d(long long n, int block = 256) { return dim3((unsigned)((n + block - 1) / block)); }

int up1d_smem_limit(const void* fn, size_t smem) {
  if (smem > 48 * 1024) T2_CHECK_CUDA(cudaFuncSetAttribute(fn, cudaFuncAttributeMaxDynamicSharedMemorySize, int(smem)));
  return T2_OK;
}
int launch_upsample_fwd(const float* in, const float* K, const float* bias, float* out, bf16* c_up, int B, int C, int W, int s, int type,
                        int act, float alpha, int split, cudaStream_t st) {
  if (type == 2) {
    const size_t smem = up1d_smem(C);
    const int rc = up1d_smem_limit(reinterpret_cast<const void*>(up1d_fwd_kernel), smem);
    if (rc) return rc;
    const long long wt = (W + kUp1Tw - 1) / kUp1Tw;
    const int jz = int(std::max(1LL, std::min<long long>(s, (264 + wt * B - 1) / (wt * B))));
    up1d_fwd_kernel<<<dim3(unsigned(wt), B, jz), dim3(kUp1Tw, kUp1Rows), smem, st>>>(in, K, bias, out, c_up, C, W, s, act, alpha, split);
  } else {
    upsample_fwd_kernel<<<grid1d((long long)B * C * W * s), 256, 0, st>>>(in, K, bias, out, c_up, B, C, W, s, type, act, alpha, split);
  }
  t2_count_launch();
  T2_CHECK_CUDA(cudaGetLastError());
  return T2_OK;
}
int launch_upsample_bwd_param(const float* in, const float* out, const float* dout, long long* dK, long long* dbias, int B, int C, int W,
                              int s, int type, int act, float alpha, cudaStream_t st) {
  if (type == 2) {
    const long long nchunk = ((long long)B * W + kUp1Tw - 1) / kUp1Tw;
    const int G = int(std::min<long long>(nchunk, (264 + s - 1) / s));
    up1d_bwd_param_kernel<<<dim3(s, G), dim3(kUp1Tw, kUp1Rows), up1d_param_smem(C), st>>>(in, out, dout, dK, dbias, B, C, W, s, act, alpha);
  } else {
    T2_REQUIRE(s <= 32, T2_ERR_UNSUPPORTED_SHAPE, "upsample scale %d > 32, the limit of the SubPixel / 2D weight-gradient kernel", s);
    upsample_bwd_param_kernel<<<s * ((296 + s - 1) / s), 256, 0, st>>>(in, out, dout, dK, dbias, B, C, W, s, type, act, alpha);
  }
  t2_count_launch();
  T2_CHECK_CUDA(cudaGetLastError());
  return T2_OK;
}
int launch_upsample_bwd_input(const float* out, const float* dout, const float* K, float* din, int B, int C, int W, int s, int type, int act,
                              float alpha, cudaStream_t st) {
  if (type == 2) {
    const size_t smem = up1d_smem(C);
    const int rc = up1d_smem_limit(reinterpret_cast<const void*>(up1d_bwd_input_kernel), smem);
    if (rc) return rc;
    up1d_bwd_input_kernel<<<dim3((W + kUp1Tw - 1) / kUp1Tw, B), dim3(kUp1Tw, kUp1Rows), smem, st>>>(out, dout, K, din, C, W, s, act, alpha);
  } else {
    upsample_bwd_input_kernel<<<grid1d(4LL * B * C * W), 256, 0, st>>>(out, dout, 0, K, din, B, C, W, s, type, act, alpha);
  }
  t2_count_launch();
  T2_CHECK_CUDA(cudaGetLastError());
  return T2_OK;
}

GinArgs gin_args(const Layout& lo, const float* params) {
  GinArgs a;
  memset(&a, 0, sizeof(a));
  a.params = params;
  a.p_k = lo.p_g_k[0]; a.p_b = lo.p_g_b[0]; a.p_stride = lo.layer_stride; a.p_emb = lo.p_emb;
  a.L = lo.L; a.B = lo.B; a.G = lo.G; a.Gi = lo.Gi; a.NS = lo.NS;
  return a;
}

}

int launch_fx_finalize(const long long* acc, float* out, long long n, cudaStream_t st) {
  if (n <= 0) return T2_OK;
  fx_finalize_kernel<<<unsigned((n + 255) / 256), 256, 0, st>>>(acc, out, n);
  t2_count_launch();
  T2_CHECK_CUDA(cudaGetLastError());
  return T2_OK;
}
}

using namespace t2;

extern "C" int t2_wn_sizes(const t2_wn_config_t* cfg, t2_wn_sizes_t* out) {
  Layout lo;
  int rc = build_layout(cfg, lo);
  if (rc) return rc;
  T2_REQUIRE(out != nullptr, T2_ERR_INVALID_ARG, "null out");
  out->n_params = lo.n_params;
  out->packed_bytes = lo.packed_bytes;
  out->workspace_bytes = lo.workspace_bytes;
  out->n_tensors = int(lo.params.size());
  return T2_OK;
}

extern "C" int t2_wn_param_info(const t2_wn_config_t* cfg, int i, char* name, int name_cap, long long* offset,
                                int* ndim, int* shape4) {
  Layout lo;
  int rc = build_layout(cfg, lo);
  if (rc) return rc;
  T2_REQUIRE(i >= 0 && i < int(lo.params.size()), T2_ERR_INVALID_ARG, "tensor index %d out of range", i);
  const ParamT& p = lo.params[i];
  snprintf(name, name_cap, "%s", p.name.c_str());
  *offset = p.off;
  *ndim = p.ndim;
  for (int k = 0; k < 4; ++k) shape4[k] = p.shape[k];
  return T2_OK;
}

extern "C" int t2_wn_init(const t2_wn_config_t* cfg, void* d_packed, void* d_workspace, void* stream) {
  Layout lo;
  int rc = build_layout(cfg, lo);
  if (rc) return rc;
  cudaStream_t st = static_cast<cudaStream_t>(stream);
  uint8_t* ws = static_cast<uint8_t*>(d_workspace);
  T2_CHECK_CUDA(cudaMemsetAsync(d_packed, 0, lo.packed_bytes, st));
  T2_CHECK_CUDA(cudaMemsetAsync(d_workspace, 0, lo.workspace_bytes, st));
  float* scalars = reinterpret_cast<float*>(ws + lo.w_scalars);
  for (auto& t : lo.tiles_head)
    if (t.div != nullptr) t.div = scalars + 1;
  T2_CHECK_CUDA(cudaMemcpyAsync(ws + lo.w_tiles_main, lo.tiles_main.data(), lo.tiles_main.size() * sizeof(WgradTile), cudaMemcpyHostToDevice, st));
  T2_CHECK_CUDA(cudaMemcpyAsync(ws + lo.w_tiles_head, lo.tiles_head.data(), lo.tiles_head.size() * sizeof(WgradTile), cudaMemcpyHostToDevice, st));
  T2_CHECK_CUDA(cudaMemcpyAsync(ws + lo.w_packjobs, lo.packjobs.data(), lo.packjobs.size() * sizeof(PackJob), cudaMemcpyHostToDevice, st));
  T2_CHECK_CUDA(cudaMemcpyAsync(ws + lo.w_colsum, lo.colsums.data(), lo.colsums.size() * sizeof(ColsumJob), cudaMemcpyHostToDevice, st));
  std::vector<long long> offs(3 * lo.L);
  for (int l = 0; l < lo.L; ++l) {
    offs[3 * l] = lo.p_dil_b[l];
    offs[3 * l + 1] = lo.C > 0 ? lo.p_c_b[l] : -1;
    offs[3 * l + 2] = lo.p_s_b[l];
  }
  T2_CHECK_CUDA(cudaMemcpyAsync(ws + lo.w_tables, offs.data(), offs.size() * sizeof(long long), cudaMemcpyHostToDevice, st));
  T2_CHECK_CUDA(cudaMemcpyAsync(ws + lo.w_tables + 3 * lo.L * sizeof(long long), lo.skip_scale.data(), lo.L * sizeof(float),
                                cudaMemcpyHostToDevice, st));
  T2_CHECK_CUDA(cudaStreamSynchronize(st));
  return T2_OK;
}

extern "C" int t2_wn_pack_weights(const t2_wn_config_t* cfg, const float* d_params, void* d_packed,
                                  void* d_workspace, void* stream) {
  Layout lo;
  int rc = build_layout(cfg, lo);
  if (rc) return rc;
  cudaStream_t st = static_cast<cudaStream_t>(stream);
  uint8_t* ws = static_cast<uint8_t*>(d_workspace);
  uint8_t* pk = static_cast<uint8_t*>(d_packed);
  pack_kernel<<<dim3(16, lo.n_packjobs), dim3(32, 8), 0, st>>>(d_params, reinterpret_cast<bf16*>(pk),
                                                       reinterpret_cast<const PackJob*>(ws + lo.w_packjobs)); t2_count_launch();
  T2_CHECK_CUDA(cudaGetLastError());
  long long* d_offs = reinterpret_cast<long long*>(ws + lo.w_tables);
  float* d_scales = reinterpret_cast<float*>(ws + lo.w_tables + 3 * lo.L * sizeof(long long));
  DerivedArgs a;
  a.params = d_params; a.bias_g = reinterpret_cast<float*>(pk + lo.k_bias_g); a.bias_skip = reinterpret_cast<float*>(pk + lo.k_bias_skip);
  a.offs = d_offs; a.scales = d_scales; a.L = lo.L; a.G = lo.G; a.S = lo.S;
  derived_bias_kernel<<<grid1d((long long)lo.L * lo.G), 256, 0, st>>>(a); t2_count_launch();
  T2_CHECK_CUDA(cudaGetLastError());
  return T2_OK;
}

extern "C" int t2_wn_forward(const t2_wn_config_t* cfg, const float* d_params, const void* d_packed,
                             void* d_workspace, const void* d_x, const float* d_c, const void* d_targets,
                             const int* d_lengths, float* d_loss, float* d_logits, int save_for_backward,
                             unsigned long long seed, const unsigned long long* d_step, void* stream) {
  Layout lo;
  int rc = build_layout(cfg, lo);
  if (rc) return rc;
  cudaStream_t st = static_cast<cudaStream_t>(stream);
  uint8_t* ws = static_cast<uint8_t*>(d_workspace);
  const uint8_t* pk = static_cast<const uint8_t*>(d_packed);
  const long long BT = (long long)lo.B * lo.T;
  float* scalars = reinterpret_cast<float*>(ws + lo.w_scalars);
  const float p = cfg->dropout;
  T2_CHECK_CUDA(cudaMemsetAsync(scalars, 0, 16 * sizeof(float), st));

  T2_REQUIRE(!lo.split || (!save_for_backward && !cfg->c_pre_upsampled), T2_ERR_INVALID_ARG,
             "split_bf16 (fp32-class) mode is forward / loss only (save_for_backward = 0) and needs the upsampling net");
  if (lo.Gi > 0) {
    GinArgs a = gin_args(lo, d_params);
    const int* spk = reinterpret_cast<const int*>(ws + lo.w_spk);
    a.bias = reinterpret_cast<const float*>(pk + lo.k_bias_g); a.bias_ld = lo.G;
    a.on = spk; a.ids = spk + 1;
    a.out = reinterpret_cast<float*>(ws + lo.w_gbias); a.out_l = (long long)lo.B * lo.G; a.out_b = lo.G;
    gin_bias_kernel<<<grid1d((long long)lo.L * lo.B * lo.G), 256, 0, st>>>(a); t2_count_launch();
    T2_CHECK_CUDA(cudaGetLastError());
  }
  bf16* c_up = reinterpret_cast<bf16*>(ws + lo.w_cup);
  if (lo.split) T2_CHECK_CUDA(cudaMemsetAsync(c_up, 0, (size_t)BT * 256 * 2, st));
  if (lo.C > 0) {
    T2_REQUIRE(d_c != nullptr, T2_ERR_INVALID_ARG, "local conditioning enabled but d_c is NULL");
    if (cfg->c_pre_upsampled) {
      f32_to_bf16_kernel<<<grid1d(BT * lo.C), 256, 0, st>>>(d_c, c_up, BT * lo.C); t2_count_launch();
    } else {
      const float* in = d_c;
      int W = lo.Tc;
      for (size_t i = 0; i < lo.up_w.size(); ++i) {
        const int s = cfg->upsample_scales[i];
        float* out = reinterpret_cast<float*>(ws + lo.w_upout[i]);
        const bool last = i + 1 == lo.up_w.size();
        rc = launch_upsample_fwd(in, d_params + lo.p_up_k[i], d_params + lo.p_up_b[i], out, last ? c_up : nullptr, lo.B, lo.C, W, s,
                                 cfg->upsample_type, cfg->upsample_activation, cfg->leaky_alpha, lo.split ? 1 : 0, st);
        if (rc) return rc;
        in = out;
        W *= s;
      }
    }
    T2_CHECK_CUDA(cudaGetLastError());
  }
  bf16* x_all = reinterpret_cast<bf16*>(ws + lo.w_x);
  bf16* xd_all = reinterpret_cast<bf16*>(ws + lo.w_xd);
  first_conv_kernel<<<grid1d(BT * (lo.R / 8)), 256, 0, st>>>(d_x, lo.scalar_in ? 1 : 0, d_params + lo.p_in_k, d_params + lo.p_in_b,
                                                       x_all, p > 0.f ? xd_all : x_all, BT, lo.R, p, seed, d_step, lo.split ? 1 : 0); t2_count_launch();
  T2_CHECK_CUDA(cudaGetLastError());
  bf16* z_all = reinterpret_cast<bf16*>(ws + lo.w_z);
  const ActT a_z = make_act(z_all, lo.Gh * lo.xm, lo.T, lo.B, lo.L);
  for (int l = 0; l < lo.L; ++l) {
    ActGemmCall g = make_gate_call(lo, ws, pk, l, save_for_backward != 0);
    rc = launch_act_gemm(EPI_GATE, 256, g, st);
    if (rc) return rc;
    if (l + 1 < lo.L) {
      ActGemmCall o = make_out_call(lo, ws, pk, d_params, l, p, seed, d_step);
      rc = launch_act_gemm(EPI_RES, lo.R, o, st);
      if (rc) return rc;
    }
  }
  bf16* h1 = reinterpret_cast<bf16*>(ws + lo.w_h1);
  bf16* h2 = reinterpret_cast<bf16*>(ws + lo.w_h2);
  {
    ActGemmCall g;
    memset(&g, 0, sizeof(g));
    g.a[0] = a_z; g.na = 1;
    g.seg[0] = Seg{0, 0, 0, lo.Gh * lo.xm / kBK, 0, lo.L}; g.nseg = 1;
    if (lo.split) { g.seg[1] = Seg{0, 0, 0, lo.Gh / kBK, 0, lo.L}; g.nseg = 2; }
    g.w = pk + lo.k_Ws; g.wN = lo.S; g.wK = lo.L * lo.Gh * (lo.split ? 3 : 1); g.wL = 1;
    g.T = lo.T; g.B = lo.B; g.n_tiles = 1;
    g.epi.ptr[0] = h1; g.epi.ptr[1] = const_cast<float*>(reinterpret_cast<const float*>(pk + lo.k_bias_skip));
    g.epi.i[0] = lo.S; g.epi.i[1] = 1; g.epi.i[2] = lo.S; g.epi.i[11] = lo.split ? 1 : 0;
    rc = launch_act_gemm(EPI_BIAS_ACT, lo.S, g, st);
    if (rc) return rc;
  }
  {
    ActGemmCall g;
    memset(&g, 0, sizeof(g));
    g.a[0] = make_act(h1, lo.S * lo.xm, lo.T, lo.B); g.na = 1;
    g.seg[0] = Seg{0, 0, 0, lo.S * lo.xm / kBK, 0, 1}; g.nseg = 1;
    if (lo.split) { g.seg[1] = Seg{0, 0, 0, lo.S / kBK, 0, 1}; g.nseg = 2; }
    g.w = pk + lo.k_Wf1; g.wN = lo.S; g.wK = lo.S * (lo.split ? 3 : 1); g.wL = 1;
    g.T = lo.T; g.B = lo.B; g.n_tiles = 1;
    g.epi.ptr[0] = h2; g.epi.ptr[1] = const_cast<float*>(d_params + lo.p_f1_b);
    g.epi.i[0] = lo.S; g.epi.i[1] = 1; g.epi.i[2] = lo.S; g.epi.i[11] = lo.split ? 1 : 0;
    rc = launch_act_gemm(EPI_BIAS_ACT, lo.S, g, st);
    if (rc) return rc;
  }
  {
    ActGemmCall g;
    memset(&g, 0, sizeof(g));
    g.a[0] = make_act(h2, lo.S * lo.xm, lo.T, lo.B); g.na = 1;
    g.seg[0] = Seg{0, 0, 0, lo.S * lo.xm / kBK, 0, 1}; g.nseg = 1;
    if (lo.split) { g.seg[1] = Seg{0, 0, 0, lo.S / kBK, 0, 1}; g.nseg = 2; }
    g.w = pk + lo.k_Wf2; g.wN = lo.O; g.wK = lo.S * (lo.split ? 3 : 1); g.wL = 1;
    g.T = lo.T; g.B = lo.B; g.n_tiles = 1;
    g.epi.ptr[0] = const_cast<void*>(d_targets);
    g.epi.ptr[1] = const_cast<int*>(d_lengths);
    g.epi.ptr[2] = const_cast<float*>(d_params + lo.p_f2_b);
    g.epi.ptr[3] = scalars + 0; g.epi.ptr[4] = scalars + 1;
    g.epi.ptr[5] = save_for_backward ? ws + lo.w_dlog : nullptr;
    g.epi.ptr[6] = d_logits;
    g.epi.i[1] = lo.ldo;
    if (lo.mol) {
      g.epi.f[0] = cfg->log_scale_min;
      g.epi.f[1] = 1.f / float(lo.Q - 1);
      g.epi.f[2] = logf(float(lo.Q - 1) / 2.f);
      g.epi.i[0] = lo.gauss ? 0 : lo.O / 3;
      g.epi.i[2] = lo.gauss ? (cfg->cdf_loss ? 2 : 1) : 0;
      g.epi.f[3] = cfg->log_scale_min_gauss;
      rc = launch_act_gemm(EPI_MOL, 32, g, st);
    } else {
      rc = launch_act_gemm(EPI_CE, 256, g, st);
    }
    if (rc) return rc;
  }
  if (d_loss) T2_CHECK_CUDA(cudaMemcpyAsync(d_loss, scalars, 2 * sizeof(float), cudaMemcpyDeviceToDevice, st));
  return T2_OK;
}

struct SideStream { cudaStream_t s; cudaEvent_t fork, fork2, join; };
static SideStream* side_stream() {
  static SideStream ss;
  static int state = 0;
  if (state == 0) {
    const char* e = getenv("T2_SIDE_STREAM");
    if (e && e[0] == '0') state = -1;
    else if (cudaStreamCreateWithFlags(&ss.s, cudaStreamNonBlocking) == cudaSuccess &&
             cudaEventCreateWithFlags(&ss.fork, cudaEventDisableTiming) == cudaSuccess &&
             cudaEventCreateWithFlags(&ss.fork2, cudaEventDisableTiming) == cudaSuccess &&
             cudaEventCreateWithFlags(&ss.join, cudaEventDisableTiming) == cudaSuccess) state = 1;
    else state = -1;
  }
  return state == 1 ? &ss : nullptr;
}

extern "C" int t2_wn_backward(const t2_wn_config_t* cfg, const float* d_params, const void* d_packed,
                              void* d_workspace, const void* d_x, const float* d_c, float* d_grads,
                              unsigned long long seed, const unsigned long long* d_step, void* stream) {
  return t2_wn_backward_phased(cfg, d_params, d_packed, d_workspace, d_x, d_c, d_grads, seed, d_step, -1, 1, stream);
}

extern "C" int t2_wn_backward_phased(const t2_wn_config_t* cfg, const float* d_params, const void* d_packed,
                                     void* d_workspace, const void* d_x, const float* d_c, float* d_grads,
                                     unsigned long long seed, const unsigned long long* d_step, int phase, int n_groups, void* stream) {
  Layout lo;
  int rc = build_layout(cfg, lo);
  if (rc) return rc;
  cudaStream_t st = static_cast<cudaStream_t>(stream);
  T2_REQUIRE(!lo.split, T2_ERR_INVALID_ARG, "split_bf16 (fp32-class) mode has no backward pass");
  T2_REQUIRE(n_groups >= 1 && n_groups <= lo.L && (phase == -1 || phase == 100 || (phase >= 0 && phase <= n_groups)), T2_ERR_INVALID_ARG,
             "backward_phased: bad phase %d / n_groups %d", phase, n_groups);
  if (phase >= 1 && phase <= n_groups) {
    uint8_t* ws = static_cast<uint8_t*>(d_workspace);
    const int g = phase - 1;
    const int l0 = int((long long)lo.L * g / n_groups), l1 = int((long long)lo.L * (g + 1) / n_groups);
    const int t0 = lo.tile_start[l0], t1 = lo.tile_start[l1];
    ActT maps[6] = {make_act(ws + lo.w_xd, lo.R, lo.T, lo.B, lo.L), make_act(ws + lo.w_dg, lo.G, lo.T, lo.B, lo.L),
                    make_act(ws + lo.w_cup, lo.C > 0 ? lo.C : 8, lo.T, lo.B, 1),
                    make_act(ws + lo.w_z, lo.Gh, lo.T, lo.B, lo.L), make_act(ws + lo.w_dxin, lo.R, lo.T, lo.B, lo.L),
                    make_act(ws + lo.w_dskip, lo.S, lo.T, lo.B, 1)};
    return launch_wgrad(maps, 6, reinterpret_cast<const WgradTile*>(ws + lo.w_tiles_main) + t0, t1 - t0, d_grads, lo.T, lo.B, st);
  }
  if (phase == 100) {
    SideStream* side = side_stream();
    if (side) {
      T2_CHECK_CUDA(cudaEventRecord(side->join, side->s));
      T2_CHECK_CUDA(cudaStreamWaitEvent(st, side->join, 0));
    }
    return launch_fx_finalize(reinterpret_cast<const long long*>(static_cast<uint8_t*>(d_workspace) + lo.w_gfx), d_grads, lo.n_params, st);
  }
  uint8_t* ws = static_cast<uint8_t*>(d_workspace);
  const uint8_t* pk = static_cast<const uint8_t*>(d_packed);
  const long long BT = (long long)lo.B * lo.T;
  float* scalars = reinterpret_cast<float*>(ws + lo.w_scalars);
  const float p = cfg->dropout;
  T2_CHECK_CUDA(cudaMemsetAsync(d_grads, 0, lo.n_params * sizeof(float), st));
  T2_CHECK_CUDA(cudaMemsetAsync(ws + lo.w_skipsum, 0, lo.S * sizeof(long long), st));
  T2_CHECK_CUDA(cudaMemsetAsync(ws + lo.w_gfx, 0, lo.n_params * sizeof(long long), st));
  if (lo.Gi > 0) T2_CHECK_CUDA(cudaMemsetAsync(ws + lo.w_gsum, 0, (size_t)lo.L * lo.B * lo.G * sizeof(long long), st));
  long long* gfx = reinterpret_cast<long long*>(ws + lo.w_gfx);
  bf16* h1 = reinterpret_cast<bf16*>(ws + lo.w_h1);
  bf16* h2 = reinterpret_cast<bf16*>(ws + lo.w_h2);
  bf16* dlog = reinterpret_cast<bf16*>(ws + lo.w_dlog);
  bf16* dh2 = reinterpret_cast<bf16*>(ws + lo.w_dh2);
  bf16* dskip = reinterpret_cast<bf16*>(ws + lo.w_dskip);
  bf16* dxin = reinterpret_cast<bf16*>(ws + lo.w_dxin);
  bf16* dg = reinterpret_cast<bf16*>(ws + lo.w_dg);
  bf16* ta_all = reinterpret_cast<bf16*>(ws + lo.w_ta);
  bf16* sb_all = reinterpret_cast<bf16*>(ws + lo.w_sb);
  {
    ActGemmCall g;
    memset(&g, 0, sizeof(g));
    g.a[0] = make_act(dlog, lo.ldo, lo.T, lo.B); g.na = 1;
    g.seg[0] = Seg{0, 0, 0, lo.Op / kBK, 0, 1}; g.nseg = 1;
    g.w = pk + lo.k_Wf2T; g.wN = lo.S; g.wK = lo.Op; g.wL = 1;
    g.T = lo.T; g.B = lo.B; g.n_tiles = 1;
    g.epi.ptr[0] = dh2; g.epi.ptr[1] = h2; g.epi.ptr[2] = scalars + 1; g.epi.f[0] = 1.f; g.epi.i[0] = lo.S;
    g.epi.ptr[3] = gfx + lo.p_f1_b;
    rc = launch_act_gemm(EPI_SCALE_RELUMASK, lo.S, g, st);
    if (rc) return rc;
  }
  {
    ActGemmCall g;
    memset(&g, 0, sizeof(g));
    g.a[0] = make_act(dh2, lo.S, lo.T, lo.B); g.na = 1;
    g.seg[0] = Seg{0, 0, 0, lo.S / kBK, 0, 1}; g.nseg = 1;
    g.w = pk + lo.k_Wf1T; g.wN = lo.S; g.wK = lo.S; g.wL = 1;
    g.T = lo.T; g.B = lo.B; g.n_tiles = 1;
    g.epi.ptr[0] = dskip; g.epi.ptr[1] = h1; g.epi.ptr[2] = nullptr; g.epi.f[0] = 1.f; g.epi.i[0] = lo.S;
    g.epi.ptr[3] = ws + lo.w_skipsum;
    rc = launch_act_gemm(EPI_SCALE_RELUMASK, lo.S, g, st);
    if (rc) return rc;
  }
  skip_bias_kernel<<<grid1d((long long)lo.L * lo.S), 256, 0, st>>>(reinterpret_cast<const long long*>(ws + lo.w_skipsum), d_grads,
      reinterpret_cast<const long long*>(ws + lo.w_tables), reinterpret_cast<const float*>(ws + lo.w_tables + 3 * lo.L * sizeof(long long)), lo.L, lo.S);
  t2_count_launch();
  SideStream* side = side_stream();
  cudaStream_t sb = st;
  if (side) {
    T2_CHECK_CUDA(cudaEventRecord(side->fork, st));
    T2_CHECK_CUDA(cudaStreamWaitEvent(side->s, side->fork, 0));
    sb = side->s;
  }
  {
    ActT hmaps[4] = {make_act(h1, lo.S, lo.T, lo.B), make_act(dh2, lo.S, lo.T, lo.B), make_act(h2, lo.S, lo.T, lo.B),
                     make_act(dlog, lo.ldo, lo.T, lo.B)};
    rc = launch_wgrad(hmaps, 4, reinterpret_cast<const WgradTile*>(ws + lo.w_tiles_head), lo.n_tiles_head, d_grads, lo.T, lo.B, sb);
    if (rc) return rc;
    colsum_kernel<<<dim3(96, lo.n_colsum), 256, 0, sb>>>(ws, gfx, reinterpret_cast<const ColsumJob*>(ws + lo.w_colsum), scalars); t2_count_launch();
    T2_CHECK_CUDA(cudaGetLastError());
  }
  const ActT a_dxin = make_act(dxin, lo.R, lo.T, lo.B, lo.L);
  const ActT a_dskip = make_act(dskip, lo.S, lo.T, lo.B, 1);
  const ActT a_dg = make_act(dg, lo.G, lo.T, lo.B, lo.L);
  const int bn_z = lo.Gh >= 256 ? 256 : 128;
  for (int l = lo.L - 1; l >= 0; --l) {
    ActGemmCall gz = make_dz_call(lo, ws, pk, l, gfx);
    rc = launch_act_gemm(EPI_GATE_BWD, bn_z, gz, st);
    if (rc) return rc;
    ActGemmCall gx = make_dx_call(lo, ws, pk, l, p, seed, d_step, gfx);
    rc = launch_act_gemm(EPI_DX, lo.R, gx, st);
    if (rc) return rc;
  }
  if (lo.Gi > 0) {
    GinGradArgs a;
    a.params = d_params; a.spk = reinterpret_cast<const int*>(ws + lo.w_spk);
    a.S = reinterpret_cast<const long long*>(ws + lo.w_gsum); a.gfx = gfx; a.grads = d_grads;
    a.offs = reinterpret_cast<const long long*>(ws + lo.w_tables);
    a.p_k = lo.p_g_k[0]; a.p_b = lo.p_g_b[0]; a.p_stride = lo.layer_stride; a.p_emb = lo.p_emb;
    a.L = lo.L; a.B = lo.B; a.G = lo.G; a.Gi = lo.Gi; a.NS = lo.NS;
    gin_wgrad_kernel<<<grid1d((long long)lo.L * lo.G), 256, 0, st>>>(a); t2_count_launch();
    gin_demb_kernel<<<dim3(lo.NS, lo.Gi), kGinThreads, 0, st>>>(a); t2_count_launch();
    T2_CHECK_CUDA(cudaGetLastError());
  }
  if (side) {
    T2_CHECK_CUDA(cudaEventRecord(side->fork2, st));
    T2_CHECK_CUDA(cudaStreamWaitEvent(side->s, side->fork2, 0));
  }
  if (phase == -1) {
    ActT maps[6] = {make_act(ws + lo.w_xd, lo.R, lo.T, lo.B, lo.L), a_dg,
                    make_act(ws + lo.w_cup, lo.C > 0 ? lo.C : 8, lo.T, lo.B, 1),
                    make_act(ws + lo.w_z, lo.Gh, lo.T, lo.B, lo.L), a_dxin, a_dskip};
    rc = launch_wgrad(maps, 6, reinterpret_cast<const WgradTile*>(ws + lo.w_tiles_main), lo.n_tiles_main, d_grads, lo.T, lo.B, st);
    if (rc) return rc;
  }
  first_conv_bwd_kernel<<<dim3((unsigned)((BT + 63) / 64)), lo.R, 0, sb>>>(d_x, lo.scalar_in ? 1 : 0, dxin, gfx + lo.p_in_k, BT, lo.R); t2_count_launch();
  T2_CHECK_CUDA(cudaGetLastError());
  if (lo.C > 0 && !cfg->c_pre_upsampled) {
    float* dcup = reinterpret_cast<float*>(ws + lo.w_dcup);
    ActGemmCall g;
    memset(&g, 0, sizeof(g));
    g.a[0] = a_dg; g.na = 1;
    g.seg[0] = Seg{0, 0, 0, lo.G / kBK, 0, lo.L}; g.nseg = 1;
    g.w = pk + lo.k_WcT; g.wN = lo.C; g.wK = lo.L * lo.G; g.wL = 1;
    g.T = lo.T; g.B = lo.B; g.n_tiles = 1;
    g.epi.ptr[0] = nullptr; g.epi.ptr[1] = nullptr; g.epi.ptr[2] = dcup;
    g.epi.i[0] = lo.C; g.epi.i[1] = 0; g.epi.i[2] = lo.C;
    rc = launch_act_gemm(EPI_BIAS_ACT, 128, g, sb);
    if (rc) return rc;
    float* dchw = reinterpret_cast<float*>(ws + lo.w_upgrad[1]);
    cl_to_chw_kernel<<<dim3((lo.T + 31) / 32, (lo.C + 31) / 32, lo.B), dim3(32, 8), 0, sb>>>(dcup, dchw, lo.T, lo.C); t2_count_launch();
    const float* dout = dchw;
    int pp = 0;
    for (int i = int(lo.up_w.size()) - 1; i >= 0; --i) {
      const int s = cfg->upsample_scales[i];
      const int W = lo.up_w[i] / s;
      const float* layer_in = i == 0 ? d_c : reinterpret_cast<const float*>(ws + lo.w_upout[i - 1]);
      const float* out = reinterpret_cast<const float*>(ws + lo.w_upout[i]);
      rc = launch_upsample_bwd_param(layer_in, out, dout, gfx + lo.p_up_k[i], gfx + lo.p_up_b[i], lo.B, lo.C, W, s, cfg->upsample_type,
                                     cfg->upsample_activation, cfg->leaky_alpha, sb);
      if (rc) return rc;
      if (i > 0) {
        float* din = reinterpret_cast<float*>(ws + lo.w_upgrad[pp]);
        rc = launch_upsample_bwd_input(out, dout, d_params + lo.p_up_k[i], din, lo.B, lo.C, W, s, cfg->upsample_type, cfg->upsample_activation,
                                       cfg->leaky_alpha, sb);
        if (rc) return rc;
        dout = din;
        pp ^= 1;
      }
    }
  }
  if (side && phase == -1) {
    T2_CHECK_CUDA(cudaEventRecord(side->join, sb));
    T2_CHECK_CUDA(cudaStreamWaitEvent(st, side->join, 0));
  }
  if (phase == -1) {
    const int rc = launch_fx_finalize(gfx, d_grads, lo.n_params, st);
    if (rc) return rc;
  }
  return T2_OK;
}

extern "C" int t2_wn_set_speakers(const t2_wn_config_t* cfg, void* d_workspace, const int* d_speaker_ids, void* stream) {
  Layout lo;
  int rc = build_layout(cfg, lo);
  if (rc) return rc;
  T2_REQUIRE(lo.Gi > 0, T2_ERR_INVALID_ARG, "speaker ids need gin_channels > 0");
  cudaStream_t st = static_cast<cudaStream_t>(stream);
  set_speakers_kernel<<<grid1d(lo.B), 256, 0, st>>>(reinterpret_cast<int*>(static_cast<uint8_t*>(d_workspace) + lo.w_spk), d_speaker_ids, lo.B);
  t2_count_launch();
  T2_CHECK_CUDA(cudaGetLastError());
  return T2_OK;
}

extern "C" int t2_wn_workspace_tensor(const t2_wn_config_t* cfg, void* d_workspace, const char* name, void** ptr,
                                      long long* count, int* elem_bytes) {
  Layout lo;
  int rc = build_layout(cfg, lo);
  if (rc) return rc;
  uint8_t* ws = static_cast<uint8_t*>(d_workspace);
  const long long BT = (long long)lo.B * lo.T;
  struct E { const char* n; long long off; long long cnt; int eb; };
  const E table[] = {
      {"c_up", lo.w_cup, BT * lo.C, 2},       {"x", lo.w_x, lo.L * BT * lo.R, 2},    {"xd", lo.w_xd, lo.L * BT * lo.R, 2},
      {"ta", lo.w_ta, lo.L * BT * lo.Gh, 2},  {"sb", lo.w_sb, lo.L * BT * lo.Gh, 2}, {"z", lo.w_z, lo.L * BT * lo.Gh, 2},
      {"h1", lo.w_h1, BT * lo.S, 2},          {"h2", lo.w_h2, BT * lo.S, 2},         {"dlog", lo.w_dlog, BT * lo.ldo, 2},
      {"dh2", lo.w_dh2, BT * lo.S, 2},        {"dskip", lo.w_dskip, BT * lo.S, 2},   {"dxin", lo.w_dxin, lo.L * BT * lo.R, 2},
      {"dg", lo.w_dg, lo.L * BT * lo.G, 2},   {"dc_up", lo.w_dcup, BT * lo.C, 4},    {"scalars", lo.w_scalars, 16, 4},
  };
  for (const E& e : table)
    if (strcmp(e.n, name) == 0) {
      *ptr = ws + e.off; *count = e.cnt; *elem_bytes = e.eb;
      return T2_OK;
    }
  return t2_set_error(T2_ERR_INVALID_ARG, "unknown workspace tensor '%s'", name);
}

extern "C" int t2_dbg_wn_kernel(const t2_dbg_kernel_t* call, void* stream) {
  T2_REQUIRE(call != nullptr, T2_ERR_INVALID_ARG, "dbg_wn_kernel: null call");
  cudaStream_t st = static_cast<cudaStream_t>(stream);
  void* const* p = call->p;
  const long long* i = call->i;
  const long long B = i[0], C = i[1], W = i[2], s = i[3], type = i[4], act = i[5];
  const float alpha = call->f[0];
  T2_REQUIRE(B >= 1 && B <= 65535 && C >= 1 && C <= 128 && W >= 1 && s >= 1 && W * s <= (1LL << 28) && B * C * W * s <= (1LL << 31) &&
                 type >= 0 && type <= 2 && act >= 0 && act <= 2 && alpha >= 0.f && alpha <= 1.f,
             T2_ERR_INVALID_ARG, "dbg_wn_kernel: bad shape, type, activation or alpha");
  const int b = int(B), c = int(C), w = int(W), sc = int(s), ty = int(type), ac = int(act);
  switch (call->kernel) {
    case T2_DBG_WN_UP_FWD:
      T2_REQUIRE(p[0] && p[1] && p[2] && p[3] && (i[6] == 0 || i[6] == 1), T2_ERR_INVALID_ARG, "dbg_wn_kernel UP_FWD: bad arguments");
      return launch_upsample_fwd(static_cast<const float*>(p[0]), static_cast<const float*>(p[1]), static_cast<const float*>(p[2]),
                                 static_cast<float*>(p[3]), static_cast<bf16*>(p[4]), b, c, w, sc, ty, ac, alpha, int(i[6]), st);
    case T2_DBG_WN_UP_BWD_PARAM: {
      T2_REQUIRE(p[0] && p[1] && p[2] && p[3] && p[4] && p[5], T2_ERR_INVALID_ARG, "dbg_wn_kernel UP_BWD_PARAM: null pointer argument");
      T2_REQUIRE(ty == 2 || sc <= 32, T2_ERR_UNSUPPORTED_SHAPE, "dbg_wn_kernel UP_BWD_PARAM: upsample scale %d > 32 (SubPixel / 2D)", sc);
      const long long nK = ty == 0 ? 9LL * sc : ty == 1 ? 3LL * sc : s * C * C, nb = ty == 0 ? sc : ty == 1 ? 1 : C;
      long long* acc = static_cast<long long*>(p[5]);
      float* dK = static_cast<float*>(p[3]);
      float* db = static_cast<float*>(p[4]);
      T2_CHECK_CUDA(cudaMemsetAsync(acc, 0, size_t(nK + nb) * sizeof(long long), st));
      int rc = launch_upsample_bwd_param(static_cast<const float*>(p[0]), static_cast<const float*>(p[1]), static_cast<const float*>(p[2]),
                                         acc, acc + nK, b, c, w, sc, ty, ac, alpha, st);
      if (rc) return rc;
      T2_CHECK_CUDA(cudaMemsetAsync(dK, 0, size_t(nK) * sizeof(float), st));
      T2_CHECK_CUDA(cudaMemsetAsync(db, 0, size_t(nb) * sizeof(float), st));
      rc = launch_fx_finalize(acc, dK, nK, st);
      return rc ? rc : launch_fx_finalize(acc + nK, db, nb, st);
    }
    case T2_DBG_WN_UP_BWD_INPUT:
      T2_REQUIRE(p[0] && p[1] && p[2] && p[3], T2_ERR_INVALID_ARG, "dbg_wn_kernel UP_BWD_INPUT: null pointer argument");
      return launch_upsample_bwd_input(static_cast<const float*>(p[0]), static_cast<const float*>(p[1]), static_cast<const float*>(p[2]),
                                       static_cast<float*>(p[3]), b, c, w, sc, ty, ac, alpha, st);
    default:
      return t2_set_error(T2_ERR_INVALID_ARG, "dbg_wn_kernel: unknown kernel id %d", call->kernel);
  }
}

extern "C" int t2_wn_time_kernel(const t2_wn_config_t* cfg, const float* d_params, const void* d_packed, void* d_workspace,
                                 int which, int layer, int reps, float* ms_per_launch, void* stream) {
  Layout lo;
  int rc = build_layout(cfg, lo);
  if (rc) return rc;
  T2_REQUIRE(layer >= 0 && layer < lo.L && reps >= 1 && ms_per_launch && which >= 0 && which <= 4, T2_ERR_INVALID_ARG,
             "time_kernel: bad arguments");
  T2_REQUIRE(which != 1 || layer + 1 < lo.L, T2_ERR_INVALID_ARG, "the last layer has no out GEMM");
  cudaStream_t st = static_cast<cudaStream_t>(stream);
  uint8_t* ws = static_cast<uint8_t*>(d_workspace);
  const uint8_t* pk = static_cast<const uint8_t*>(d_packed);
  ActGemmCall g;
  int epi, bn;
  if (which == 0 || which == 4) { g = make_gate_call(lo, ws, pk, layer, which == 0); epi = EPI_GATE; bn = 256; }
  else if (which == 1) { g = make_out_call(lo, ws, pk, d_params, layer, cfg->dropout, 1, nullptr); epi = EPI_RES; bn = lo.R; }
  else if (which == 2) { g = make_dz_call(lo, ws, pk, layer, nullptr); epi = EPI_GATE_BWD; bn = lo.Gh >= 256 ? 256 : 128; }
  else { g = make_dx_call(lo, ws, pk, layer, cfg->dropout, 1, nullptr, nullptr); epi = EPI_DX; bn = lo.R; }
  T2_CHECK_CUDA(cudaStreamSynchronize(st));
  cudaStream_t ps;
  T2_CHECK_CUDA(cudaStreamCreateWithFlags(&ps, cudaStreamNonBlocking));
  cudaEvent_t e0, e1;
  T2_CHECK_CUDA(cudaEventCreate(&e0));
  T2_CHECK_CUDA(cudaEventCreate(&e1));
  rc = launch_act_gemm(epi, bn, g, ps);
  if (rc) return rc;
  T2_CHECK_CUDA(cudaStreamSynchronize(ps));
  cudaGraph_t graph;
  cudaGraphExec_t exec;
  T2_CHECK_CUDA(cudaStreamBeginCapture(ps, cudaStreamCaptureModeThreadLocal));
  for (int i = 0; i < reps && rc == 0; ++i) rc = launch_act_gemm(epi, bn, g, ps);
  cudaError_t ce = cudaStreamEndCapture(ps, &graph);
  if (rc) return rc;
  T2_CHECK_CUDA(ce);
  T2_CHECK_CUDA(cudaGraphInstantiate(&exec, graph, 0));
  T2_CHECK_CUDA(cudaGraphLaunch(exec, ps));
  T2_CHECK_CUDA(cudaEventRecord(e0, ps));
  T2_CHECK_CUDA(cudaGraphLaunch(exec, ps));
  T2_CHECK_CUDA(cudaEventRecord(e1, ps));
  T2_CHECK_CUDA(cudaEventSynchronize(e1));
  float ms = 0.f;
  T2_CHECK_CUDA(cudaEventElapsedTime(&ms, e0, e1));
  *ms_per_launch = ms / reps;
  cudaGraphExecDestroy(exec);
  cudaGraphDestroy(graph);
  cudaEventDestroy(e0);
  cudaEventDestroy(e1);
  cudaStreamDestroy(ps);
  return T2_OK;
}

#include <cooperative_groups.h>
namespace cg = cooperative_groups;

namespace t2 {
namespace {

constexpr int kArThreads = 512;
__device__ long long* g_ar_dbg = nullptr;
#define AR_STAMP(i) do { if (g_ar_dbg && blockIdx.x == 0 && threadIdx.x == 0 && t == 64 && l == 7) g_ar_dbg[i] = clock64(); } while (0)
constexpr int kArMaxItems = 4;

struct ArLayout {
  int CS, ZC, RC, SC, FC, OC, K1;
  long long per_rank_layer;
  long long o_head1, o_head2;
  long long n_weights;
  long long o_bias;
  long long packed_bytes;
  long long ring_slots_total;
  long long workspace_bytes, w_cup, w_upout_base, w_ring, w_ringoff;
  long long w_gbias;
  std::vector<int> ring_slots, ring_off;
// ... 618 lines not shown
```

### tacotron-2_b200/wavenet.py

```python
import ctypes
import math

import torch

from . import lib as L


class WnConfig(ctypes.Structure):
    _fields_ = [
        ("layers", ctypes.c_int), ("stacks", ctypes.c_int), ("residual_channels", ctypes.c_int),
        ("gate_channels", ctypes.c_int), ("skip_out_channels", ctypes.c_int), ("kernel_size", ctypes.c_int),
        ("cin_channels", ctypes.c_int), ("out_channels", ctypes.c_int), ("quantize_channels", ctypes.c_int),
        ("input_type", ctypes.c_int), ("legacy", ctypes.c_int), ("residual_legacy", ctypes.c_int),
        ("upsample_type", ctypes.c_int), ("n_upsample", ctypes.c_int), ("upsample_scales", ctypes.c_int * 4),
        ("freq_axis_kernel_size", ctypes.c_int), ("dropout", ctypes.c_float), ("log_scale_min", ctypes.c_float),
        ("B", ctypes.c_int), ("T", ctypes.c_int), ("Tc", ctypes.c_int), ("c_pre_upsampled", ctypes.c_int),
        ("log_scale_min_gauss", ctypes.c_float), ("cdf_loss", ctypes.c_int), ("split_bf16", ctypes.c_int),
        ("gin_channels", ctypes.c_int), ("n_speakers", ctypes.c_int),
        ("upsample_activation", ctypes.c_int), ("leaky_alpha", ctypes.c_float),
    ]


class WnSizes(ctypes.Structure):
    _fields_ = [("n_params", ctypes.c_longlong), ("packed_bytes", ctypes.c_longlong),
# ... 27 lines not shown
    need("kernel_size", lambda v: v == 3, "kernel_size 3")
    need("upsample_type", lambda v: v in _UPSAMPLE_TYPES or v == "NearestNeighbor", "Resize upsampler: modules.py:657-693")
    need("upsample_activation", lambda v: v in _UPSAMPLE_ACTIVATIONS, "Relu | LeakyRelu | None: wavenet.py:197-203")
    if getattr(hp, "upsample_activation", None) == "LeakyRelu":
        need("leaky_alpha", _leaky_alpha_ok, "LeakyRelu slope in [0, 1] (max(alpha * x, x) is leaky_relu only there)")
    if getattr(hp, "upsample_type", None) != "1D":
        need("freq_axis_kernel_size", lambda v: v == 3, "freq_axis_kernel_size 3")
    need("input_type", lambda v: v in _INPUT_TYPES, "raw | mulaw | mulaw-quantize")
    need("wavenet_synth_debug", lambda v: not v, "teacher-forced synthesis debugging from wavenet_debug_wavs: synthesizer.py:54-57,85-97")
    need("wavenet_natural_eval", lambda v: not v, "free-running evaluation: wavenet.py:386 (evaluation here is teacher forced)")
    return bad


def make_config(hp, B, T, c_pre_upsampled=False, dropout=None, precision="bf16"):
    bad = unsupported_hparams(hp)
    if bad:
        raise L.T2Error("hparams not implemented on the H100 WaveNet path (they would change the model): " + "; ".join(bad))
    cfg = WnConfig()
    cfg.layers, cfg.stacks = hp.layers, hp.stacks
    cfg.residual_channels, cfg.gate_channels, cfg.skip_out_channels = (
        hp.residual_channels, hp.gate_channels, hp.skip_out_channels)
    cfg.kernel_size = hp.kernel_size
    cfg.cin_channels = max(hp.cin_channels, 0)
    cfg.out_channels, cfg.quantize_channels = hp.out_channels, hp.quantize_channels
    cfg.input_type = _INPUT_TYPES[hp.input_type]
    cfg.legacy, cfg.residual_legacy = int(hp.legacy), int(hp.residual_legacy)
    if hp.upsample_type == "NearestNeighbor":
        c_pre_upsampled = True
    elif hp.upsample_type not in _UPSAMPLE_TYPES:
        raise L.T2Error("upsample_type %r is not implemented on the H100 path" % hp.upsample_type)
    cfg.upsample_type = _UPSAMPLE_TYPES.get(hp.upsample_type, 0)
    act = getattr(hp, "upsample_activation", "Relu")
    cfg.upsample_activation = _UPSAMPLE_ACTIVATIONS[act]
    cfg.leaky_alpha = float(hp.leaky_alpha) if act == "LeakyRelu" else 0.0
    scales = list(hp.upsample_scales)
    cfg.n_upsample = len(scales)
    for i, s in enumerate(scales):
        cfg.upsample_scales[i] = s
    cfg.freq_axis_kernel_size = hp.freq_axis_kernel_size
    cfg.dropout = hp.wavenet_dropout if dropout is None else dropout
    cfg.log_scale_min = hp.log_scale_min
    cfg.log_scale_min_gauss = getattr(hp, "log_scale_min_gauss", -7.0)
    cfg.cdf_loss = int(getattr(hp, "cdf_loss", False))
    if precision not in ("bf16", "fp32-class"):
        raise L.T2Error("precision must be 'bf16' or 'fp32-class'")
    cfg.split_bf16 = int(precision == "fp32-class")
    if (getattr(hp, "gin_channels", None) or 0) > 0:
        cfg.gin_channels, cfg.n_speakers = hp.gin_channels, hp.n_speakers
    cfg.B, cfg.T = B, T
    hop = 1
    for s in scales:
        hop *= s
    cfg.c_pre_upsampled = int(c_pre_upsampled)
    if cfg.cin_channels > 0 and not c_pre_upsampled:
        if T % hop:
            raise L.T2Error("T=%d is not a multiple of prod(upsample_scales)=%d" % (T, hop))
        cfg.Tc = T // hop
    else:
        cfg.Tc = T
    return cfg


def param_table(cfg):
    lib = L.load()
    sz = WnSizes()
    L.check(lib.t2_wn_sizes(ctypes.byref(cfg), ctypes.byref(sz)))
    name = ctypes.create_string_buffer(160)
    off, nd, shp = ctypes.c_longlong(), ctypes.c_int(), (ctypes.c_int * 4)()
    out = []
    for i in range(sz.n_tensors):
        L.check(lib.t2_wn_param_info(ctypes.byref(cfg), i, name, 160, ctypes.byref(off), ctypes.byref(nd), shp))
        out.append((name.value.decode(), off.value, tuple(shp[k] for k in range(nd.value))))
    return out, sz.n_params


def grad_buckets(tensors, n_layers, n_params, n_groups):
    off = {t[0]: t[1] for t in tensors}
    first = lambda l: off["ResidualConv1DGLU_%d/residual_block_causal_conv/kernel" % l]
    stack_end = off["final_convolution_1/kernel"]
    bounds = [first(n_layers * g // n_groups) for g in range(n_groups)] + [stack_end]
    groups = [(bounds[g], bounds[g + 1]) for g in range(n_groups)]
    rest = [(0, first(0)), (stack_end, n_params)]
    return groups, [r for r in rest if r[1] > r[0]]


def speaker_ids(speakers, B, n_speakers):
    ids = torch.as_tensor(speakers).detach().cpu().reshape(-1)
    if ids.numel() != B or ids.is_floating_point() or ids.is_complex():
        raise ValueError("speaker ids must be %d integers ([B] or [B, 1]), got %s %s" % (B, tuple(torch.as_tensor(speakers).shape), ids.dtype))
    bad = [int(v) for v in ids.tolist() if not 0 <= int(v) < n_speakers]
    if bad:
        raise ValueError("speaker id(s) %s outside [0, n_speakers=%d)" % (bad, n_speakers))
    return ids.to(torch.int32)


def nn_upsample(hp, c, T):
    hop = hp.hop_size
    up = c.transpose(1, 2).repeat_interleave(hop, dim=1)
    if up.shape[1] < T:
        raise L.T2Error("conditioning of %d frames x hop %d is shorter than T=%d" % (c.shape[2], hop, T))
    return up[:, :T].contiguous()


class WaveNet(object):

    def __init__(self, hparams, B, T, device="cuda", c_pre_upsampled=False, dropout=None, training=True, precision="bf16"):
        self.hp = hparams
        self.lib = L.load()
        self.device = torch.device(device)
        self.precision = precision
        if precision == "fp32-class":
            dropout = 0.0
        self.cfg = make_config(hparams, B, T, c_pre_upsampled, dropout, precision)
        self.training = training
        sz = WnSizes()
        L.check(self.lib.t2_wn_sizes(ctypes.byref(self.cfg), ctypes.byref(sz)))
        self.sizes = sz
        self.n_params = sz.n_params
        self.params = torch.zeros(sz.n_params, dtype=torch.float32, device=self.device)
        self.packed = torch.empty(sz.packed_bytes, dtype=torch.uint8, device=self.device)
        self.workspace = torch.empty(sz.workspace_bytes, dtype=torch.uint8, device=self.device)
        self.loss_buf = torch.zeros(2, dtype=torch.float32, device=self.device)
        self.grads = self.m = self.v = self.ema = None
        self.tensors = []
        name = ctypes.create_string_buffer(160)
        off = ctypes.c_longlong()
        nd = ctypes.c_int()
        shp = (ctypes.c_int * 4)()
        for i in range(sz.n_tensors):
            L.check(self.lib.t2_wn_param_info(ctypes.byref(self.cfg), i, name, 160, ctypes.byref(off),
                                              ctypes.byref(nd), shp))
            self.tensors.append((name.value.decode(), off.value, tuple(shp[k] for k in range(nd.value))))
        offs = [t[1] for t in self.tensors] + [sz.n_params]
        self.offsets = torch.tensor(offs, dtype=torch.int64, device=self.device)
        self.opt_scratch = torch.zeros(sz.n_tensors + 2, dtype=torch.float32, device=self.device)
        self.global_step = 0
        self.seed = int(hparams.wavenet_random_seed)
        self.step_dev = torch.zeros(1, dtype=torch.int64, device=self.device)
        self._spk = torch.zeros(B, dtype=torch.int32, device=self.device) if self.cfg.gin_channels > 0 else None
        self._graph = None
        with torch.cuda.device(self.device):
            L.check(self.lib.t2_wn_init(ctypes.byref(self.cfg), L.ptr(self.packed), L.ptr(self.workspace),
                                        L.stream_ptr()))
        self._packed_dirty = True

    def load_params(self, params):
        flat = torch.zeros(self.n_params, dtype=torch.float32)
        for name, off, shape in self.tensors:
            t = params[name].detach().to(torch.float32).reshape(-1)
            n = int(math.prod(shape))
            assert t.numel() == n, "%s: expected %s got %s" % (name, shape, tuple(params[name].shape))
            flat[off:off + n] = t
        self.params.copy_(flat.to(self.device))
        self._packed_dirty = True

    def init_variables(self, seed=None):
        from . import init
        self.load_params(init.wavenet_variables(self.hp, self.tensors, seed))

    def unflatten(self, flat):
        flat = flat.detach().float().cpu()
        return {name: flat[off:off + int(math.prod(shape))].reshape(shape).clone() for name, off, shape in self.tensors}

    def export_params(self):
        return self.unflatten(self.params)

    def export_grads(self):
        return self.unflatten(self.grads)

    def pack(self):
        L.check(self.lib.t2_wn_pack_weights(ctypes.byref(self.cfg), L.ptr(self.params), L.ptr(self.packed),
                                            L.ptr(self.workspace), L.stream_ptr()))
        self._packed_dirty = False

    def set_speakers(self, speakers):
        if self._spk is None:
            raise L.T2Error("speaker ids need gin_channels > 0")
        if speakers is None:
            L.check(self.lib.t2_wn_set_speakers(ctypes.byref(self.cfg), L.ptr(self.workspace), None, L.stream_ptr()))
            return
        self._spk.copy_(speaker_ids(speakers, self.cfg.B, self.cfg.n_speakers))
        L.check(self.lib.t2_wn_set_speakers(ctypes.byref(self.cfg), L.ptr(self.workspace), L.ptr(self._spk), L.stream_ptr()))

    def forward(self, x, c, targets, lengths, logits=None, save_for_backward=True, seed=None, speakers=None):
        if speakers is not None:
            self.set_speakers(speakers)
        if self._packed_dirty:
            self.pack()
        if self.hp.upsample_type == "NearestNeighbor" and c is not None and c.dim() == 3 and c.shape[1] == self.cfg.cin_channels and c.shape[2] != self.cfg.T:
            c = nn_upsample(self.hp, c, self.cfg.T)
        self._last_x, self._last_c = x, c
        self._last_seed = self.seed if seed is None else seed
        L.check(self.lib.t2_wn_forward(ctypes.byref(self.cfg), L.ptr(self.params), L.ptr(self.packed),
                                       L.ptr(self.workspace), L.ptr(x), L.ptr(c), L.ptr(targets), L.ptr(lengths),
                                       L.ptr(self.loss_buf), L.ptr(logits), int(save_for_backward),
                                       ctypes.c_ulonglong(self._last_seed), L.ptr(self.step_dev), L.stream_ptr()))
        return self.loss_buf

    def backward(self, phase=-1, n_groups=1):
        if self.grads is None:
            self.grads = torch.zeros_like(self.params)
        L.check(self.lib.t2_wn_backward_phased(ctypes.byref(self.cfg), L.ptr(self.params), L.ptr(self.packed),
                                               L.ptr(self.workspace), L.ptr(self._last_x), L.ptr(self._last_c),
                                               L.ptr(self.grads), ctypes.c_ulonglong(self._last_seed),
                                               L.ptr(self.step_dev), int(phase), int(n_groups), L.stream_ptr()))
        return self.grads

    def grad_buckets(self, n_groups):
        return grad_buckets(self.tensors, self.cfg.layers, self.n_params, n_groups)

    def capture(self, x, c, targets, lengths, overlap_groups=1):
        self._static = (x, c, targets, lengths)
        if self.grads is None:
            self.grads = torch.zeros_like(self.params)
        G = max(1, int(overlap_groups))
        side = torch.cuda.Stream(device=self.device)
        side.wait_stream(torch.cuda.current_stream())
        with torch.cuda.stream(side):
            self.pack()
            self.forward(x, c, targets, lengths)
            self.backward()
            if G > 1:
                self.backward(0, G)
                self.backward(100, G)
                for g in range(G):
                    self.backward(1 + g, G)
        torch.cuda.current_stream().wait_stream(side)
        torch.cuda.synchronize()
        n0 = self.lib.t2_launch_count()
        self._graphs = []
        if G == 1:
            self._graph = torch.cuda.CUDAGraph()
            with torch.cuda.graph(self._graph):
                self.step_dev.add_(1)
                self.pack()
                self.forward(x, c, targets, lengths)
                self.backward()
        else:
            pool = None
            for g in range(G):
                gr = torch.cuda.CUDAGraph()
                with torch.cuda.graph(gr, pool=pool):
                    if g == 0:
                        self.step_dev.add_(1)
                        self.pack()
                        self.forward(x, c, targets, lengths)
                        self.backward(0, G)
                        self.backward(100, G)
                    self.backward(1 + g, G)
                pool = gr.pool()
                self._graphs.append(gr)
            self._graph = self._graphs[0]
            self._buckets = self.grad_buckets(G)
        self._fwd_bwd_launches = self.lib.t2_launch_count() - n0
        return self._graph

    def train_step(self, x=None, c=None, targets=None, lengths=None, world_size=1, process_group=None, speakers=None):
        if speakers is not None:
            self.set_speakers(speakers)
        if self._graph is not None and getattr(self, "_graphs", None):
            import torch.distributed as dist
            for dst, src in zip(self._static, (x, c, targets, lengths)):
                if src is not None and src is not dst:
                    dst.copy_(src, non_blocking=True)
            groups, rest = self._buckets
            works = []
            for gr, (a, b) in zip(self._graphs, groups):
                gr.replay()
                if world_size > 1:
                    works.append(dist.all_reduce(self.grads[a:b], op=dist.ReduceOp.SUM, group=process_group, async_op=True))
            if world_size > 1:
                for a, b in rest:
                    works.append(dist.all_reduce(self.grads[a:b], op=dist.ReduceOp.SUM, group=process_group, async_op=True))
                for w in works:
                    w.wait()
            n0 = self.lib.t2_launch_count()
            self.optimizer_step(grad_scale=1.0 / world_size)
            self._opt_launches = self.lib.t2_launch_count() - n0
            return self.loss_buf
        if self._graph is not None:
            for dst, src in zip(self._static, (x, c, targets, lengths)):
                if src is not None and src is not dst:
                    dst.copy_(src, non_blocking=True)
            self._graph.replay()
        else:
            n0 = self.lib.t2_launch_count()
            self.step_dev.add_(1)
            self.forward(x, c, targets, lengths)
            self.backward()
            self._fwd_bwd_launches = self.lib.t2_launch_count() - n0
        if world_size > 1:
            import torch.distributed as dist
            dist.all_reduce(self.grads, op=dist.ReduceOp.SUM, group=process_group)
        n0 = self.lib.t2_launch_count()
        self.optimizer_step(grad_scale=1.0 / world_size)
        self._opt_launches = self.lib.t2_launch_count() - n0
        return self.loss_buf

    @property
    def launches_per_step(self):
        return getattr(self, "_fwd_bwd_launches", 0) + getattr(self, "_opt_launches", 0)

    def time_kernel(self, which, layer, reps=20):
        ms = ctypes.c_float()
        L.check(self.lib.t2_wn_time_kernel(ctypes.byref(self.cfg), L.ptr(self.params), L.ptr(self.packed),
                                           L.ptr(self.workspace), which, layer, reps, ctypes.byref(ms), L.stream_ptr()))
        return ms.value

    def time_gate_gemm(self, layer, reps=20):
        return self.time_kernel(0, layer, reps)

    def learning_rate(self):
        hp = self.hp
        if hp.wavenet_lr_schedule == "noam":
            step = float(self.global_step + 1)
            w = hp.wavenet_warmup
            return max(hp.wavenet_learning_rate * w ** 0.5 * min(step * w ** -1.5, step ** -0.5), 1e-4)
        return hp.wavenet_learning_rate * hp.wavenet_decay_rate ** (self.global_step / hp.wavenet_decay_steps)

    def optimizer_step(self, grad_scale=1.0):
        hp = self.hp
        if self.m is None:
            self.m = torch.zeros_like(self.params)
            self.v = torch.zeros_like(self.params)
            self.ema = self.params.clone()
        lr = self.learning_rate()
        clip = hp.wavenet_clip_gradients
        L.check(self.lib.t2_adam_step(
            L.ptr(self.params), L.ptr(self.grads), L.ptr(self.m), L.ptr(self.v), L.ptr(self.ema),
            L.ptr(self.offsets), len(self.tensors), ctypes.c_longlong(self.n_params), ctypes.c_float(lr),
            ctypes.c_float(hp.wavenet_adam_beta1), ctypes.c_float(hp.wavenet_adam_beta2),
            ctypes.c_float(hp.wavenet_adam_epsilon), self.global_step + 1, ctypes.c_float(grad_scale),
            ctypes.c_float(hp.wavenet_gradient_max_norm if clip else 0.0),
            ctypes.c_float(hp.wavenet_gradient_max_value if clip else 0.0), ctypes.c_float(0.0),
            ctypes.c_float(hp.wavenet_ema_decay), L.ptr(self.opt_scratch), L.stream_ptr()))
        self.global_step += 1
        self._packed_dirty = True
        return lr

    def workspace_tensor(self, name, shape=None):
        p = ctypes.c_void_p()
        cnt = ctypes.c_longlong()
        eb = ctypes.c_int()
        L.check(self.lib.t2_wn_workspace_tensor(ctypes.byref(self.cfg), L.ptr(self.workspace), name.encode(),
                                                ctypes.byref(p), ctypes.byref(cnt), ctypes.byref(eb)))
        off = p.value - self.workspace.data_ptr()
        raw = self.workspace[off:off + cnt.value * eb.value]
        t = raw.view(torch.bfloat16 if eb.value == 2 else torch.float32)
        return t.reshape(shape) if shape is not None else t

    def loss_value(self):
        s, n = self.loss_buf.tolist()
        return s / max(n, 1e-20)


class WaveNetSynthesizer(object):

    def __init__(self, hparams, B, T, cluster_size=8, device="cuda"):
        self.hp = hparams
        self.lib = L.load()
        self.device = torch.device(device)
        self.cfg = make_config(hparams, B, T, False, 0.0)
        self.cs = cluster_size
        sz = WnSizes()
        L.check(self.lib.t2_wn_sizes(ctypes.byref(self.cfg), ctypes.byref(sz)))
        self.n_params = sz.n_params
        self.params = torch.zeros(sz.n_params, dtype=torch.float32, device=self.device)
        pb, wb = ctypes.c_longlong(), ctypes.c_longlong()
        L.check(self.lib.t2_wn_ar_sizes(ctypes.byref(self.cfg), self.cs, ctypes.byref(pb), ctypes.byref(wb)))
        self.packed = torch.empty(pb.value, dtype=torch.uint8, device=self.device)
        self.workspace = torch.zeros(wb.value, dtype=torch.uint8, device=self.device)
        self._spk = torch.zeros(B, dtype=torch.int32, device=self.device) if self.cfg.gin_channels > 0 else None
        self.tensors = []
        name = ctypes.create_string_buffer(160)
        off, nd, shp = ctypes.c_longlong(), ctypes.c_int(), (ctypes.c_int * 4)()
        for i in range(sz.n_tensors):
            L.check(self.lib.t2_wn_param_info(ctypes.byref(self.cfg), i, name, 160, ctypes.byref(off), ctypes.byref(nd), shp))
            self.tensors.append((name.value.decode(), off.value, tuple(shp[k] for k in range(nd.value))))

    def load_params(self, params):
        flat = torch.zeros(self.n_params, dtype=torch.float32)
        for name, off, shape in self.tensors:
            flat[off:off + int(math.prod(shape))] = params[name].detach().float().reshape(-1)
        self.params.copy_(flat.to(self.device))
        L.check(self.lib.t2_wn_ar_pack(ctypes.byref(self.cfg), self.cs, L.ptr(self.params), L.ptr(self.packed),
                                       L.ptr(self.workspace), L.stream_ptr()))

    def init_variables(self, seed=None):
        from . import init
        self.load_params(init.wavenet_variables(self.hp, self.tensors, seed))

    def generate(self, c, initial, test_inputs=None, u_a=None, u_b=None, seed=0, return_raw=False, speakers=None):
        B, T = self.cfg.B, self.cfg.T
        if speakers is not None and self._spk is None:
            raise L.T2Error("speaker ids need gin_channels > 0")
        if self._spk is not None:
            if speakers is not None:
                self._spk.copy_(speaker_ids(speakers, B, self.cfg.n_speakers))
            L.check(self.lib.t2_wn_ar_set_speakers(ctypes.byref(self.cfg), self.cs, L.ptr(self.params), L.ptr(self.packed),
                                                   L.ptr(self.workspace), None if speakers is None else L.ptr(self._spk),
                                                   L.stream_ptr()))
        if self.hp.upsample_type == "NearestNeighbor" and c is not None and c.dim() == 3 and c.shape[1] == self.cfg.cin_channels and c.shape[2] != T:
            c = nn_upsample(self.hp, c, T)
        scalar = self.cfg.input_type != 2
        out = torch.empty(B, T, dtype=torch.float32 if scalar else torch.int32, device=self.device)
        raw = torch.empty(B, T, self.cfg.out_channels, dtype=torch.float32, device=self.device) if return_raw else None
        L.check(self.lib.t2_wn_ar_generate(ctypes.byref(self.cfg), self.cs, L.ptr(self.params), L.ptr(self.packed),
                                           L.ptr(self.workspace), L.ptr(c), L.ptr(initial), L.ptr(test_inputs),
                                           L.ptr(u_a), L.ptr(u_b), ctypes.c_ulonglong(seed), L.ptr(out), L.ptr(raw),
                                           L.stream_ptr()))
        return (out, raw) if return_raw else out
```

Baseline: 3.627 million.

## Fuse Adam update with bf16 weight packing and compact fixed-point gradient buffer

Adds a WaveNet-specific optimizer step in which Adam writes updated parameters straight into the packed bf16 GEMM layout, so the separate pack pass no longer runs inside the captured forward/backward graph. It also shrinks the fixed-point gradient accumulator to only the bias and small tensors that actually use it, and zeroes only the gradient ranges that the wgrad tiles do not overwrite. The clip-norm reduction is unrolled 8-wide. This removes full-size memsets and a full re-read of the parameters for packing, at the cost of more complex host-side table construction and coverage invariants that must hold.

Measured after the change: 3.718 million, median of 6. 1.03x the previous value.

```diff
diff --git a/include/t2b200.h b/include/t2b200.h
--- a/include/t2b200.h
+++ b/include/t2b200.h
@@ -241,6 +241,9 @@
                  const long long* d_offsets, int n_tensors, long long n_total, float lr, float beta1, float beta2,
                  float eps, int step, float grad_scale, float max_norm, float max_value, float global_norm_clip,
                  float ema_decay, float* d_scratch, void* stream);
+int t2_wn_optimizer_step(const t2_wn_config_t* cfg, float* d_params, const float* d_grads, float* d_m, float* d_v, float* d_ema,
+                         void* d_packed, void* d_workspace, float lr, float beta1, float beta2, float eps, int step, float grad_scale,
+                         float max_norm, float max_value, float ema_decay, float* d_scratch, void* stream);
 
 typedef struct {
   int sample_rate, n_fft, hop_size, win_size, num_mels;
diff --git a/tacotron-2_b200/csrc/t2_common.cuh b/tacotron-2_b200/csrc/t2_common.cuh
--- a/tacotron-2_b200/csrc/t2_common.cuh
+++ b/tacotron-2_b200/csrc/t2_common.cuh
@@ -140,6 +140,8 @@
   return fx_in_range(a) ? float(double(a) * (1.0 / 1099511627776.0)) : __int_as_float(0x7fffffff);
 }
 int launch_fx_finalize(const long long* acc, float* out, long long n, cudaStream_t st);
+int launch_clip_norms(const float* g, const long long* offs, int n_tensors, long long n_total, float gscale, float* norms,
+                      cudaStream_t st);
 
 __device__ __forceinline__ void mbar_init(uint64_t* bar, uint32_t count) {
   asm volatile("mbarrier.init.shared::cta.b64 [%0], %1;\n" ::"r"(smem_u32(bar)), "r"(count));
diff --git a/tacotron-2_b200/csrc/t2_optim.cu b/tacotron-2_b200/csrc/t2_optim.cu
--- a/tacotron-2_b200/csrc/t2_optim.cu
+++ b/tacotron-2_b200/csrc/t2_optim.cu
@@ -25,6 +25,17 @@
   while (true) {
     const long long tend = offs[t + 1] < e1 ? offs[t + 1] : e1;
     acc = 0.f;
+    const long long bd = blockDim.x;
+    for (; e + 7 * bd < tend; e += 8 * bd) {
+      float x[8];
+#pragma unroll
+      for (int i = 0; i < 8; ++i) x[i] = g[e + i * bd];
+#pragma unroll
+      for (int i = 0; i < 8; ++i) {
+        const float v = x[i] * gscale;
+        acc += v * v;
+      }
+    }
     for (; e < tend; e += blockDim.x) {
       const float v = g[e] * gscale;
       acc += v * v;
@@ -92,6 +103,14 @@
 }
 
 }
+
+int launch_clip_norms(const float* g, const long long* offs, int n_tensors, long long n_total, float gscale, float* norms,
+                      cudaStream_t st) {
+  T2_CHECK_CUDA(cudaMemsetAsync(norms, 0, (n_tensors + 1) * sizeof(float), st));
+  sumsq_kernel<<<(unsigned)((n_total + 4095) / 4096), 256, 0, st>>>(g, offs, n_tensors, n_total, gscale, norms); t2_count_launch();
+  T2_CHECK_CUDA(cudaGetLastError());
+  return T2_OK;
+}
 }
 
 extern "C" int t2_adam_step(float* d_params, const float* d_grads, float* d_m, float* d_v, float* d_ema,
diff --git a/tacotron-2_b200/csrc/t2_wavenet.cu b/tacotron-2_b200/csrc/t2_wavenet.cu
--- a/tacotron-2_b200/csrc/t2_wavenet.cu
+++ b/tacotron-2_b200/csrc/t2_wavenet.cu
@@ -34,6 +34,17 @@
   long long dst_off, dst2_off;
   float scale;
   int div_scalar;
+};
+struct GradRange {
+  long long param_off, compact_off, count;
+};
+struct AdamPackGroup {
+  long long src_off;
+  int K, N, tensor, job0, njobs;
+};
+struct AdamRange {
+  long long param_off, flat_off, count;
+  int tensor;
 };
 
 inline long long align_up(long long v, long long a) { return (v + a - 1) / a * a; }
@@ -69,6 +80,8 @@
   long long w_gbias;
   long long w_gsum;
   long long w_gfx;
+  long long w_fx_ranges, w_zero_ranges;
+  long long w_fx_offs;
   long long w_upgrad[2], w_scalars, w_tiles_main, w_tiles_head, w_packjobs, w_colsum, w_tables;
   std::vector<long long> w_upout;
   std::vector<int> up_w;
@@ -78,7 +91,19 @@
   std::vector<ColsumJob> colsums;
   std::vector<WgradTile> tiles_main, tiles_head;
   std::vector<int> tile_start;
+  std::vector<GradRange> fx_ranges, zero_ranges;
+  long long n_fx, n_zero;
+  std::vector<PackJob> adam_jobs;
+  std::vector<AdamPackGroup> adam_groups;
+  std::vector<AdamRange> adam_plain;
+  long long n_adam_plain;
+  long long w_adam_jobs, w_adam_groups, w_adam_plain, w_param_offs;
   int dil(int l) const { return 1 << (l % (L / c.stacks)); }
+  long long fxo(long long p) const {
+    for (const GradRange& r : fx_ranges)
+      if (p >= r.param_off && p < r.param_off + r.count) return r.compact_off + (p - r.param_off);
+    return -1;
+  }
 };
 
 long long add_param(Layout& lo, const std::string& name, std::initializer_list<int> shape) {
@@ -195,6 +220,29 @@
       lo.p_up_b.push_back(add_param(lo, s + "bias", {1}));
     }
   }
+  auto numel = [&](long long off) {
+    for (const ParamT& p : lo.params)
+      if (p.off == off) return (long long)p.shape[0] * p.shape[1] * p.shape[2] * p.shape[3];
+    return 0LL;
+  };
+  lo.fx_ranges.clear();
+  lo.n_fx = 0;
+  auto fxr = [&](long long off) {
+    const long long n = numel(off);
+    lo.fx_ranges.push_back(GradRange{off, lo.n_fx, n});
+    lo.n_fx += align_up(n, 4);
+  };
+  fxr(lo.p_in_k);
+  fxr(lo.p_in_b);
+  for (int l = 0; l < lo.L; ++l) {
+    fxr(lo.p_dil_b[l]);
+    if (lo.C > 0) fxr(lo.p_c_b[l]);
+    if (lo.Gi > 0) fxr(lo.p_g_b[l]);
+    if (l < lo.L - 1) fxr(lo.p_o_b[l]);
+  }
+  fxr(lo.p_f1_b);
+  fxr(lo.p_f2_b);
+  for (size_t i = 0; i < lo.up_w.size(); ++i) { fxr(lo.p_up_k[i]); fxr(lo.p_up_b[i]); }
   long long o = 0;
   auto takeb = [&](long long bytes) { long long r = o; o = align_up(o + bytes, 256); return r; };
   const long long L = lo.L;
@@ -234,7 +282,7 @@
   lo.w_dcup = takeb(BT * (lo.C > 0 ? lo.C : 8) * 4);
   lo.w_scalars = takeb(64 * 4);
   lo.w_skipsum = takeb(lo.S * 8);
-  lo.w_gfx = takeb(lo.n_params * 8);
+  lo.w_gfx = takeb(lo.n_fx * 8);
 
   lo.packjobs.clear();
   auto pj = [&](long long src, int K, int N, long long dst_bytes, int ld, int transpose, int col0, float scale, int perm) {
@@ -279,6 +327,41 @@
   pj(lo.p_f2_k, lo.S, lo.O, lo.k_Wf2T, lo.Op, 0, 0, 1.f, 0);
   if (!lo.mol) pj(lo.p_f2_k, lo.S, lo.O, lo.k_Wf2T, lo.Op, 0, 256, 1.f, 0);
   lo.n_packjobs = int(lo.packjobs.size());
+  lo.adam_jobs.clear();
+  lo.adam_groups.clear();
+  lo.adam_plain.clear();
+  lo.n_adam_plain = 0;
+  if (!lo.split) {
+    std::vector<long long> srcs;
+    for (const PackJob& j : lo.packjobs) srcs.push_back(j.src_off);
+    std::sort(srcs.begin(), srcs.end());
+    srcs.erase(std::unique(srcs.begin(), srcs.end()), srcs.end());
+    long long covered = 0;
+    for (long long s : srcs) {
+      AdamPackGroup gr;
+      gr.src_off = s; gr.job0 = int(lo.adam_jobs.size()); gr.njobs = 0; gr.K = gr.N = 0; gr.tensor = 0;
+      for (const PackJob& j : lo.packjobs)
+        if (j.src_off == s) { gr.K = j.K; gr.N = j.N; lo.adam_jobs.push_back(j); ++gr.njobs; }
+      while (gr.tensor + 1 < int(lo.params.size()) && lo.params[gr.tensor + 1].off <= s) ++gr.tensor;
+      covered += (long long)gr.K * gr.N;
+      lo.adam_groups.push_back(gr);
+    }
+    size_t gi = 0;
+    auto plain = [&](long long a, long long b, int t) {
+      if (b > a) { lo.adam_plain.push_back(AdamRange{a, lo.n_adam_plain, b - a, t}); lo.n_adam_plain += b - a; }
+    };
+    for (size_t t = 0; t < lo.params.size(); ++t) {
+      const long long a = lo.params[t].off, b = t + 1 < lo.params.size() ? lo.params[t + 1].off : lo.n_params;
+      long long cur = a;
+      for (; gi < lo.adam_groups.size() && lo.adam_groups[gi].src_off < b; ++gi) {
+        plain(cur, lo.adam_groups[gi].src_off, int(t));
+        cur = lo.adam_groups[gi].src_off + (long long)lo.adam_groups[gi].K * lo.adam_groups[gi].N;
+      }
+      plain(cur, b, int(t));
+    }
+    T2_REQUIRE(covered + lo.n_adam_plain == lo.n_params, T2_ERR_INVALID_ARG, "internal: optimizer tables cover %lld of %lld parameters",
+               covered + lo.n_adam_plain, lo.n_params);
+  }
 
   lo.tiles_main.clear();
   auto wt = [&](std::vector<WgradTile>& v, int am, int ach, int ash, int al, int bm, int bch, int bl, long long off,
@@ -330,23 +413,95 @@
     ColsumJob j; j.src_off = src; j.rows = rows; j.C = C; j.ld = ld; j.dst_off = dst; j.dst2_off = dst2; j.scale = scale;
     j.div_scalar = div; lo.colsums.push_back(j);
   };
-  cs(lo.w_dlog, BT, lo.O, lo.ldo, lo.p_f2_b, -1, 1.f, 1);
-  if (!lo.mol) cs(lo.w_dlog + 256 * 2, BT, lo.O, lo.ldo, lo.p_f2_b, -1, 1.f, 1);
+  cs(lo.w_dlog, BT, lo.O, lo.ldo, lo.fxo(lo.p_f2_b), -1, 1.f, 1);
+  if (!lo.mol) cs(lo.w_dlog + 256 * 2, BT, lo.O, lo.ldo, lo.fxo(lo.p_f2_b), -1, 1.f, 1);
   lo.n_colsum = int(lo.colsums.size());
+
+  {
+    std::vector<std::pair<long long, long long>> stored;
+    long long tile_stored = 0;
+    auto st = [&](long long off) { stored.push_back({off, numel(off)}); tile_stored += numel(off); };
+    for (int l = 0; l < lo.L; ++l) {
+      st(lo.p_dil_k[l]);
+      if (lo.C > 0) st(lo.p_c_k[l]);
+      st(lo.p_s_k[l]);
+      if (l < lo.L - 1) st(lo.p_o_k[l]);
+    }
+    st(lo.p_f1_k);
+    long long tile_area = 0;
+    for (const auto* v : {&lo.tiles_main, &lo.tiles_head})
+      for (const WgradTile& t : *v)
+        if (t.accumulate == 0) tile_area += (long long)t.m_valid * t.n_valid;
+    T2_REQUIRE(tile_area == tile_stored, T2_ERR_INVALID_ARG, "internal: wgrad tiles store %lld gradient elements, expected %lld",
+               tile_area, tile_stored);
+    for (int l = 0; l < lo.L; ++l) stored.push_back({lo.p_s_b[l], numel(lo.p_s_b[l])});
+    for (const GradRange& r : lo.fx_ranges) stored.push_back({r.param_off, r.count});
+    std::sort(stored.begin(), stored.end());
+    lo.zero_ranges.clear();
+    lo.n_zero = 0;
+    long long cur = 0;
+    auto gap = [&](long long end) {
+      if (end > cur) { lo.zero_ranges.push_back(GradRange{cur, lo.n_zero, end - cur}); lo.n_zero += end - cur; }
+    };
+    for (const auto& s : stored) {
+      gap(s.first);
+      cur = std::max(cur, s.first + s.second);
+    }
+    gap(lo.n_params);
+  }
 
   lo.w_tiles_main = takeb((long long)lo.n_tiles_main * sizeof(WgradTile));
   lo.w_tiles_head = takeb((long long)lo.n_tiles_head * sizeof(WgradTile));
   lo.w_packjobs = takeb((long long)lo.n_packjobs * sizeof(PackJob));
   lo.w_colsum = takeb((long long)lo.n_colsum * sizeof(ColsumJob));
   lo.w_tables = takeb((long long)lo.L * (3 * sizeof(long long) + sizeof(float)));
-  lo.w_spk = lo.w_gbias = lo.w_gsum = -1;
+  lo.w_fx_ranges = takeb((long long)lo.fx_ranges.size() * sizeof(GradRange));
+  lo.w_zero_ranges = takeb((long long)lo.zero_ranges.size() * sizeof(GradRange));
+  lo.w_adam_jobs = takeb((long long)lo.adam_jobs.size() * sizeof(PackJob));
+  lo.w_adam_groups = takeb((long long)lo.adam_groups.size() * sizeof(AdamPackGroup));
+  lo.w_adam_plain = takeb((long long)lo.adam_plain.size() * sizeof(AdamRange));
+  lo.w_param_offs = takeb((long long)(lo.params.size() + 1) * sizeof(long long));
+  lo.w_spk = lo.w_gbias = lo.w_gsum = lo.w_fx_offs = -1;
   if (lo.Gi > 0) {
     lo.w_spk = takeb((1LL + lo.B) * 4);
     lo.w_gbias = takeb(L * lo.B * lo.G * 4);
     lo.w_gsum = takeb(L * lo.B * lo.G * 8);
+    lo.w_fx_offs = takeb(L * 3 * 8);
   }
   lo.workspace_bytes = o;
   return T2_OK;
+}
+
+__device__ __forceinline__ void store_packed_tile(const float (*tile)[65], const PackJob& j, int k0, int n0, bf16* __restrict__ packed,
+                                                  float scale) {
+  const int tx = threadIdx.x, ty = threadIdx.y;
+  const bool vec_dst = ((j.dst_ld | j.col0 | int(j.dst_off)) & 1) == 0;
+  if (j.transpose) {
+    for (int r = ty; r < 64; r += 8) {
+      const int n = n0 + r, k = k0 + 2 * tx;
+      if (n < j.N && k < j.K) {
+        int row = n;
+        if (j.perm_gh > 0) {
+          const int half = n / j.perm_gh, idx = n % j.perm_gh;
+          row = (idx / 128) * 256 + half * 128 + (idx % 128);
+        }
+        const float a = tile[2 * tx][r] * scale, b = tile[2 * tx + 1][r] * scale;
+        bf16* dst = packed + j.dst_off + (long long)row * j.dst_ld + j.col0 + k;
+        if (vec_dst && k + 1 < j.K) *reinterpret_cast<uint32_t*>(dst) = pack_bf16x2(a, b);
+        else { dst[0] = __float2bfloat16(a); if (k + 1 < j.K) dst[1] = __float2bfloat16(b); }
+      }
+    }
+  } else {
+    for (int r = ty; r < 64; r += 8) {
+      const int k = k0 + r, n = n0 + 2 * tx;
+      if (n < j.N && k < j.K) {
+        const float a = tile[r][2 * tx] * scale, b = tile[r][2 * tx + 1] * scale;
+        bf16* dst = packed + j.dst_off + (long long)k * j.dst_ld + j.col0 + n;
+        if (vec_dst && n + 1 < j.N) *reinterpret_cast<uint32_t*>(dst) = pack_bf16x2(a, b);
+        else { dst[0] = __float2bfloat16(a); if (n + 1 < j.N) dst[1] = __float2bfloat16(b); }
+      }
+    }
+  }
 }
 
 __global__ void pack_kernel(const float* __restrict__ params, bf16* __restrict__ packed, const PackJob* __restrict__ jobs) {
@@ -355,7 +510,6 @@
   const int tiles_n = (j.N + 63) / 64, tiles_k = (j.K + 63) / 64;
   const int tx = threadIdx.x, ty = threadIdx.y;
   const bool vec_src = ((j.N | int(j.src_off)) & 1) == 0;
-  const bool vec_dst = ((j.dst_ld | j.col0 | int(j.dst_off)) & 1) == 0;
   for (int ti = blockIdx.x; ti < tiles_n * tiles_k; ti += gridDim.x) {
     const int k0 = (ti / tiles_n) * 64, n0 = (ti % tiles_n) * 64;
     for (int r = ty; r < 64; r += 8) {
@@ -371,30 +525,7 @@
       tile[r][2 * tx] = a; tile[r][2 * tx + 1] = b;
     }
     __syncthreads();
-    if (j.transpose) {
-      for (int r = ty; r < 64; r += 8) {
-        const int n = n0 + r, k = k0 + 2 * tx;
-        if (n < j.N && k < j.K) {
-          int row = n;
-          if (j.perm_gh > 0) {
-            const int half = n / j.perm_gh, idx = n % j.perm_gh;
-            row = (idx / 128) * 256 + half * 128 + (idx % 128);
-          }
-          bf16* dst = packed + j.dst_off + (long long)row * j.dst_ld + j.col0 + k;
-          if (vec_dst && k + 1 < j.K) *reinterpret_cast<uint32_t*>(dst) = pack_bf16x2(tile[2 * tx][r], tile[2 * tx + 1][r]);
-          else { dst[0] = __float2bfloat16(tile[2 * tx][r]); if (k + 1 < j.K) dst[1] = __float2bfloat16(tile[2 * tx + 1][r]); }
-        }
-      }
-    } else {
-      for (int r = ty; r < 64; r += 8) {
-        const int k = k0 + r, n = n0 + 2 * tx;
-        if (n < j.N && k < j.K) {
-          bf16* dst = packed + j.dst_off + (long long)k * j.dst_ld + j.col0 + n;
-          if (vec_dst && n + 1 < j.N) *reinterpret_cast<uint32_t*>(dst) = pack_bf16x2(tile[r][2 * tx], tile[r][2 * tx + 1]);
-          else { dst[0] = __float2bfloat16(tile[r][2 * tx]); if (n + 1 < j.N) dst[1] = __float2bfloat16(tile[r][2 * tx + 1]); }
-        }
-      }
-    }
+    store_packed_tile(tile, j, k0, n0, packed, 1.f);
     __syncthreads();
   }
 }
@@ -420,6 +551,99 @@
     for (int l = 0; l < a.L; ++l) v += a.scales[l] * a.params[a.offs[3 * l + 2] + i];
     a.bias_skip[i] = v;
   }
+}
+
+struct WnAdamArgs {
+  float* p; const float* g; float* m; float* v; float* ema;
+  const float* norms;
+  float lr_t, b1, b2, eps, gscale, max_norm, max_value, ema_decay;
+  bf16* packed;
+  const PackJob* jobs;
+  const AdamPackGroup* groups;
+  const AdamRange* plain;
+  int n_plain;
+  long long n_plain_total;
+};
+__device__ __forceinline__ float wn_clip_scale(const WnAdamArgs& a, int t) {
+  float gs = a.gscale;
+  if (a.max_norm > 0.f) gs *= a.max_norm / fmaxf(sqrtf(a.norms[t]), a.max_norm);
+  return gs;
+}
+__device__ __forceinline__ void wn_adam_elem(const WnAdamArgs& a, float gs, float gv, float& m, float& v, float& p, float& e) {
+  float g = __fmul_rn(gv, gs);
+  if (a.max_value > 0.f) g = fminf(fmaxf(g, -a.max_value), a.max_value);
+  m = __fmaf_rn(__fsub_rn(1.f, a.b1), g, __fmul_rn(m, a.b1));
+  v = __fmaf_rn(g, __fmul_rn(__fsub_rn(1.f, a.b2), g), __fmul_rn(v, a.b2));
+  p = __fsub_rn(p, __fdiv_rn(__fmul_rn(a.lr_t, m), __fadd_rn(__fsqrt_rn(v), a.eps)));
+  e = __fmaf_rn(-__fsub_rn(1.f, a.ema_decay), __fsub_rn(e, p), e);
+}
+__global__ void wn_adam_pack_kernel(WnAdamArgs a) {
+  __shared__ float tile[64][65];
+  const AdamPackGroup gr = a.groups[blockIdx.y];
+  const float gs = wn_clip_scale(a, gr.tensor);
+  const int tiles_n = (gr.N + 63) / 64, tiles_k = (gr.K + 63) / 64;
+  const int tx = threadIdx.x, ty = threadIdx.y;
+  const float* __restrict__ gp = a.g;
+  float* __restrict__ mp = a.m;
+  float* __restrict__ vp = a.v;
+  float* __restrict__ pp = a.p;
+  float* __restrict__ ep = a.ema;
+  constexpr int kRows = 64 / 8;
+  for (int ti = blockIdx.x; ti < tiles_n * tiles_k; ti += gridDim.x) {
+    const int k0 = (ti / tiles_n) * 64, n0 = (ti % tiles_n) * 64;
+    const int n = n0 + 2 * tx;
+    float2 g2[kRows], m2[kRows], v2[kRows], p2[kRows], e2[kRows];
+#pragma unroll
+    for (int i = 0; i < kRows; ++i) {
+      const int k = k0 + ty + 8 * i;
+      g2[i] = m2[i] = v2[i] = p2[i] = e2[i] = make_float2(0.f, 0.f);
+      if (k < gr.K && n < gr.N) {
+        const long long e = gr.src_off + (long long)k * gr.N + n;
+        g2[i] = *reinterpret_cast<const float2*>(gp + e);
+        m2[i] = *reinterpret_cast<const float2*>(mp + e);
+        v2[i] = *reinterpret_cast<const float2*>(vp + e);
+        p2[i] = *reinterpret_cast<const float2*>(pp + e);
+        if (ep) e2[i] = *reinterpret_cast<const float2*>(ep + e);
+      }
+    }
+#pragma unroll
+    for (int i = 0; i < kRows; ++i) {
+      const int r = ty + 8 * i, k = k0 + r;
+      if (k < gr.K && n < gr.N) {
+        const long long e = gr.src_off + (long long)k * gr.N + n;
+        wn_adam_elem(a, gs, g2[i].x, m2[i].x, v2[i].x, p2[i].x, e2[i].x);
+        wn_adam_elem(a, gs, g2[i].y, m2[i].y, v2[i].y, p2[i].y, e2[i].y);
+        *reinterpret_cast<float2*>(mp + e) = m2[i];
+        *reinterpret_cast<float2*>(vp + e) = v2[i];
+        *reinterpret_cast<float2*>(pp + e) = p2[i];
+        if (ep) *reinterpret_cast<float2*>(ep + e) = e2[i];
+      } else {
+        p2[i] = make_float2(0.f, 0.f);
+      }
+      tile[r][2 * tx] = p2[i].x; tile[r][2 * tx + 1] = p2[i].y;
+    }
+    __syncthreads();
+    for (int jj = 0; jj < gr.njobs; ++jj) {
+      const PackJob j = a.jobs[gr.job0 + jj];
+      store_packed_tile(tile, j, k0, n0, a.packed, j.scale);
+    }
+    __syncthreads();
+  }
+}
+__global__ void wn_adam_plain_kernel(WnAdamArgs a) {
+  const long long i = blockIdx.x * (long long)blockDim.x + threadIdx.x;
+  if (i >= a.n_plain_total) return;
+  int lo = 0, hi = a.n_plain;
+  while (hi - lo > 1) {
+    const int mid = (lo + hi) >> 1;
+    if (a.plain[mid].flat_off <= i) lo = mid; else hi = mid;
+  }
+  const AdamRange r = a.plain[lo];
+  const long long e = r.param_off + (i - r.flat_off);
+  float m = a.m[e], v = a.v[e], p = a.p[e], ev = a.ema ? a.ema[e] : 0.f;
+  wn_adam_elem(a, wn_clip_scale(a, r.tensor), a.g[e], m, v, p, ev);
+  a.m[e] = m; a.v[e] = v; a.p[e] = p;
+  if (a.ema) a.ema[e] = ev;
 }
 
 struct GinArgs {
@@ -462,7 +686,7 @@
   const long long* S;
   long long* gfx;
   float* grads;
-  const long long* offs;
+  const long long* fx_offs;
   long long p_k, p_b, p_stride, p_emb;
   int L, B, G, Gi, NS;
 };
@@ -479,10 +703,10 @@
     else if (!fx_in_range(tot += s)) poison = true;
   }
   if (poison) tot = kFxPoison;
-  a.gfx[a.offs[3 * l] + g] = tot;
-  if (a.offs[3 * l + 1] >= 0) a.gfx[a.offs[3 * l + 1] + g] = tot;
+  a.gfx[a.fx_offs[3 * l] + g] = tot;
+  if (a.fx_offs[3 * l + 1] >= 0) a.gfx[a.fx_offs[3 * l + 1] + g] = tot;
   if (!a.spk[0]) return;
-  a.gfx[a.p_b + l * a.p_stride + g] = tot;
+  a.gfx[a.fx_offs[3 * l + 2] + g] = tot;
   float* dW = a.grads + a.p_k + l * a.p_stride + g;
   for (int k = 0; k < a.Gi; ++k) {
     float acc = 0.f;
@@ -998,6 +1222,27 @@
   const long long e = blockIdx.x * (long long)blockDim.x + threadIdx.x;
   if (e < n && acc[e] != 0) grads[e] += fx_value(acc[e]);
 }
+__device__ __forceinline__ long long grad_range_dst(const GradRange* __restrict__ r, int n, long long e) {
+  int lo = 0, hi = n;
+  while (hi - lo > 1) {
+    const int mid = (lo + hi) >> 1;
+    if (r[mid].compact_off <= e) lo = mid; else hi = mid;
+  }
+  const long long i = e - r[lo].compact_off;
+  return i < r[lo].count ? r[lo].param_off + i : -1;
+}
+__global__ void fx_store_kernel(const long long* __restrict__ acc, float* __restrict__ grads, const GradRange* __restrict__ r, int n,
+                                long long n_slots) {
+  const long long e = blockIdx.x * (long long)blockDim.x + threadIdx.x;
+  if (e >= n_slots) return;
+  const long long d = grad_range_dst(r, n, e);
+  if (d >= 0) grads[d] = acc[e] != 0 ? fx_value(acc[e]) : 0.f;
+}
+__global__ void zero_ranges_kernel(float* __restrict__ grads, const GradRange* __restrict__ r, int n, long long total) {
+  const long long e = blockIdx.x * (long long)blockDim.x + threadIdx.x;
+  if (e >= total) return;
+  grads[grad_range_dst(r, n, e)] = 0.f;
+}
 __global__ void f32_to_bf16_kernel(const float* __restrict__ in, bf16* __restrict__ out, long long n) {
   const long long e = blockIdx.x * (long long)blockDim.x + threadIdx.x;
   if (e < n) out[e] = __float2bfloat16(in[e]);
@@ -1090,8 +1335,8 @@
   g.epi.ptr[0] = reinterpret_cast<bf16*>(ws + lo.w_ta) + lofs;
   g.epi.ptr[1] = reinterpret_cast<bf16*>(ws + lo.w_sb) + lofs;
   g.epi.ptr[2] = reinterpret_cast<bf16*>(ws + lo.w_dg) + (long long)l * BT * lo.G;
-  g.epi.ptr[3] = grads ? grads + lo.p_dil_b[l] : nullptr;
-  g.epi.ptr[4] = (grads && lo.C > 0) ? grads + lo.p_c_b[l] : nullptr;
+  g.epi.ptr[3] = grads ? grads + lo.fxo(lo.p_dil_b[l]) : nullptr;
+  g.epi.ptr[4] = (grads && lo.C > 0) ? grads + lo.fxo(lo.p_c_b[l]) : nullptr;
   if (grads && lo.Gi > 0) {
     g.epi.ptr[3] = reinterpret_cast<long long*>(ws + lo.w_gsum) + (long long)l * lo.B * lo.G;
     g.epi.ptr[4] = nullptr;
@@ -1118,7 +1363,7 @@
   g.epi.ptr[1] = dxin + (long long)l * BT * lo.R;
   g.epi.f[0] = lo.res_scale; g.epi.f[1] = p; g.epi.i[1] = l; g.epi.seed = seed;
   g.epi.ptr[7] = const_cast<unsigned long long*>(d_step);
-  g.epi.ptr[2] = grads ? grads + (l > 0 ? lo.p_o_b[l - 1] : lo.p_in_b) : nullptr;
+  g.epi.ptr[2] = grads ? grads + lo.fxo(l > 0 ? lo.p_o_b[l - 1] : lo.p_in_b) : nullptr;
   g.epi.f[2] = l > 0 ? lo.res_scale : 1.f;
   return g;
 }
@@ -1181,6 +1426,33 @@
   a.p_k = lo.p_g_k[0]; a.p_b = lo.p_g_b[0]; a.p_stride = lo.layer_stride; a.p_emb = lo.p_emb;
   a.L = lo.L; a.B = lo.B; a.G = lo.G; a.Gi = lo.Gi; a.NS = lo.NS;
   return a;
+}
+
+int launch_derived_bias(const Layout& lo, uint8_t* ws, const float* params, uint8_t* pk, cudaStream_t st) {
+  DerivedArgs a;
+  a.params = params; a.bias_g = reinterpret_cast<float*>(pk + lo.k_bias_g); a.bias_skip = reinterpret_cast<float*>(pk + lo.k_bias_skip);
+  a.offs = reinterpret_cast<const long long*>(ws + lo.w_tables);
+  a.scales = reinterpret_cast<const float*>(ws + lo.w_tables + 3 * lo.L * sizeof(long long));
+  a.L = lo.L; a.G = lo.G; a.S = lo.S;
+  derived_bias_kernel<<<grid1d((long long)lo.L * lo.G), 256, 0, st>>>(a); t2_count_launch();
+  T2_CHECK_CUDA(cudaGetLastError());
+  return T2_OK;
+}
+
+int launch_grad_zero(const Layout& lo, uint8_t* ws, float* grads, cudaStream_t st) {
+  if (lo.n_zero <= 0) return T2_OK;
+  zero_ranges_kernel<<<grid1d(lo.n_zero), 256, 0, st>>>(grads, reinterpret_cast<const GradRange*>(ws + lo.w_zero_ranges),
+                                                        int(lo.zero_ranges.size()), lo.n_zero);
+  t2_count_launch();
+  T2_CHECK_CUDA(cudaGetLastError());
+  return T2_OK;
+}
+int launch_fx_store(const Layout& lo, const uint8_t* ws, float* grads, cudaStream_t st) {
+  fx_store_kernel<<<grid1d(lo.n_fx), 256, 0, st>>>(reinterpret_cast<const long long*>(ws + lo.w_gfx), grads,
+                                                   reinterpret_cast<const GradRange*>(ws + lo.w_fx_ranges), int(lo.fx_ranges.size()), lo.n_fx);
+  t2_count_launch();
+  T2_CHECK_CUDA(cudaGetLastError());
+  return T2_OK;
 }
 
 }
@@ -1246,6 +1518,27 @@
   T2_CHECK_CUDA(cudaMemcpyAsync(ws + lo.w_tables, offs.data(), offs.size() * sizeof(long long), cudaMemcpyHostToDevice, st));
   T2_CHECK_CUDA(cudaMemcpyAsync(ws + lo.w_tables + 3 * lo.L * sizeof(long long), lo.skip_scale.data(), lo.L * sizeof(float),
                                 cudaMemcpyHostToDevice, st));
+  T2_CHECK_CUDA(cudaMemcpyAsync(ws + lo.w_fx_ranges, lo.fx_ranges.data(), lo.fx_ranges.size() * sizeof(GradRange), cudaMemcpyHostToDevice, st));
+  T2_CHECK_CUDA(cudaMemcpyAsync(ws + lo.w_zero_ranges, lo.zero_ranges.data(), lo.zero_ranges.size() * sizeof(GradRange),
+                                cudaMemcpyHostToDevice, st));
+  T2_CHECK_CUDA(cudaMemcpyAsync(ws + lo.w_adam_jobs, lo.adam_jobs.data(), lo.adam_jobs.size() * sizeof(PackJob), cudaMemcpyHostToDevice, st));
+  T2_CHECK_CUDA(cudaMemcpyAsync(ws + lo.w_adam_groups, lo.adam_groups.data(), lo.adam_groups.size() * sizeof(AdamPackGroup),
+                                cudaMemcpyHostToDevice, st));
+  T2_CHECK_CUDA(cudaMemcpyAsync(ws + lo.w_adam_plain, lo.adam_plain.data(), lo.adam_plain.size() * sizeof(AdamRange), cudaMemcpyHostToDevice, st));
+  std::vector<long long> param_offs;
+  for (const ParamT& p : lo.params) param_offs.push_back(p.off);
+  param_offs.push_back(lo.n_params);
+  T2_CHECK_CUDA(cudaMemcpyAsync(ws + lo.w_param_offs, param_offs.data(), param_offs.size() * sizeof(long long), cudaMemcpyHostToDevice, st));
+  std::vector<long long> fx_offs;
+  if (lo.Gi > 0) {
+    fx_offs.resize(3 * lo.L);
+    for (int l = 0; l < lo.L; ++l) {
+      fx_offs[3 * l] = lo.fxo(lo.p_dil_b[l]);
+      fx_offs[3 * l + 1] = lo.C > 0 ? lo.fxo(lo.p_c_b[l]) : -1;
+      fx_offs[3 * l + 2] = lo.fxo(lo.p_g_b[l]);
+    }
+    T2_CHECK_CUDA(cudaMemcpyAsync(ws + lo.w_fx_offs, fx_offs.data(), fx_offs.size() * sizeof(long long), cudaMemcpyHostToDevice, st));
+  }
   T2_CHECK_CUDA(cudaStreamSynchronize(st));
   return T2_OK;
 }
@@ -1261,14 +1554,43 @@
   pack_kernel<<<dim3(16, lo.n_packjobs), dim3(32, 8), 0, st>>>(d_params, reinterpret_cast<bf16*>(pk),
                                                        reinterpret_cast<const PackJob*>(ws + lo.w_packjobs)); t2_count_launch();
   T2_CHECK_CUDA(cudaGetLastError());
-  long long* d_offs = reinterpret_cast<long long*>(ws + lo.w_tables);
-  float* d_scales = reinterpret_cast<float*>(ws + lo.w_tables + 3 * lo.L * sizeof(long long));
-  DerivedArgs a;
-  a.params = d_params; a.bias_g = reinterpret_cast<float*>(pk + lo.k_bias_g); a.bias_skip = reinterpret_cast<float*>(pk + lo.k_bias_skip);
-  a.offs = d_offs; a.scales = d_scales; a.L = lo.L; a.G = lo.G; a.S = lo.S;
-  derived_bias_kernel<<<grid1d((long long)lo.L * lo.G), 256, 0, st>>>(a); t2_count_launch();
+  return launch_derived_bias(lo, ws, d_params, pk, st);
+}
+
+extern "C" int t2_wn_optimizer_step(const t2_wn_config_t* cfg, float* d_params, const float* d_grads, float* d_m, float* d_v, float* d_ema,
+                                    void* d_packed, void* d_workspace, float lr, float beta1, float beta2, float eps, int step,
+                                    float grad_scale, float max_norm, float max_value, float ema_decay, float* d_scratch, void* stream) {
+  Layout lo;
+  int rc = build_layout(cfg, lo);
+  if (rc) return rc;
+  T2_REQUIRE(!lo.split, T2_ERR_INVALID_ARG, "split_bf16 (fp32-class) mode has no training step");
+  T2_REQUIRE(d_params && d_grads && d_m && d_v && d_packed && d_workspace && d_scratch, T2_ERR_INVALID_ARG, "wn_optimizer_step: null pointer");
+  T2_REQUIRE(step >= 1, T2_ERR_INVALID_ARG, "wn_optimizer_step: step must be >= 1");
+  cudaStream_t st = static_cast<cudaStream_t>(stream);
+  uint8_t* ws = static_cast<uint8_t*>(d_workspace);
+  uint8_t* pk = static_cast<uint8_t*>(d_packed);
+  if (max_norm > 0.f) {
+    rc = launch_clip_norms(d_grads, reinterpret_cast<const long long*>(ws + lo.w_param_offs), int(lo.params.size()), lo.n_params,
+                           grad_scale, d_scratch, st);
+    if (rc) return rc;
+  }
+  WnAdamArgs a;
+  a.p = d_params; a.g = d_grads; a.m = d_m; a.v = d_v; a.ema = d_ema; a.norms = d_scratch;
+  a.lr_t = float(double(lr) * sqrt(1.0 - pow(double(beta2), step)) / (1.0 - pow(double(beta1), step)));
+  a.b1 = beta1; a.b2 = beta2; a.eps = eps; a.gscale = grad_scale; a.max_norm = max_norm; a.max_value = max_value;
+  a.ema_decay = ema_decay;
+  a.packed = reinterpret_cast<bf16*>(pk);
+  a.jobs = reinterpret_cast<const PackJob*>(ws + lo.w_adam_jobs);
+  a.groups = reinterpret_cast<const AdamPackGroup*>(ws + lo.w_adam_groups);
+  a.plain = reinterpret_cast<const AdamRange*>(ws + lo.w_adam_plain);
+  a.n_plain = int(lo.adam_plain.size()); a.n_plain_total = lo.n_adam_plain;
+  wn_adam_pack_kernel<<<dim3(16, unsigned(lo.adam_groups.size())), dim3(32, 8), 0, st>>>(a); t2_count_launch();
   T2_CHECK_CUDA(cudaGetLastError());
-  return T2_OK;
+  if (lo.n_adam_plain > 0) {
+    wn_adam_plain_kernel<<<grid1d(lo.n_adam_plain), 256, 0, st>>>(a); t2_count_launch();
+    T2_CHECK_CUDA(cudaGetLastError());
+  }
+  return launch_derived_bias(lo, ws, d_params, pk, st);
 }
 
 extern "C" int t2_wn_forward(const t2_wn_config_t* cfg, const float* d_params, const void* d_packed,
@@ -1445,16 +1767,17 @@
       T2_CHECK_CUDA(cudaEventRecord(side->join, side->s));
       T2_CHECK_CUDA(cudaStreamWaitEvent(st, side->join, 0));
     }
-    return launch_fx_finalize(reinterpret_cast<const long long*>(static_cast<uint8_t*>(d_workspace) + lo.w_gfx), d_grads, lo.n_params, st);
+    return launch_fx_store(lo, static_cast<const uint8_t*>(d_workspace), d_grads, st);
   }
   uint8_t* ws = static_cast<uint8_t*>(d_workspace);
   const uint8_t* pk = static_cast<const uint8_t*>(d_packed);
   const long long BT = (long long)lo.B * lo.T;
   float* scalars = reinterpret_cast<float*>(ws + lo.w_scalars);
   const float p = cfg->dropout;
-  T2_CHECK_CUDA(cudaMemsetAsync(d_grads, 0, lo.n_params * sizeof(float), st));
+  rc = launch_grad_zero(lo, ws, d_grads, st);
+  if (rc) return rc;
   T2_CHECK_CUDA(cudaMemsetAsync(ws + lo.w_skipsum, 0, lo.S * sizeof(long long), st));
-  T2_CHECK_CUDA(cudaMemsetAsync(ws + lo.w_gfx, 0, lo.n_params * sizeof(long long), st));
+  T2_CHECK_CUDA(cudaMemsetAsync(ws + lo.w_gfx, 0, lo.n_fx * sizeof(long long), st));
   if (lo.Gi > 0) T2_CHECK_CUDA(cudaMemsetAsync(ws + lo.w_gsum, 0, (size_t)lo.L * lo.B * lo.G * sizeof(long long), st));
   long long* gfx = reinterpret_cast<long long*>(ws + lo.w_gfx);
   bf16* h1 = reinterpret_cast<bf16*>(ws + lo.w_h1);
@@ -1474,7 +1797,7 @@
     g.w = pk + lo.k_Wf2T; g.wN = lo.S; g.wK = lo.Op; g.wL = 1;
     g.T = lo.T; g.B = lo.B; g.n_tiles = 1;
     g.epi.ptr[0] = dh2; g.epi.ptr[1] = h2; g.epi.ptr[2] = scalars + 1; g.epi.f[0] = 1.f; g.epi.i[0] = lo.S;
-    g.epi.ptr[3] = gfx + lo.p_f1_b;
+    g.epi.ptr[3] = gfx + lo.fxo(lo.p_f1_b);
     rc = launch_act_gemm(EPI_SCALE_RELUMASK, lo.S, g, st);
     if (rc) return rc;
   }
@@ -1524,7 +1847,7 @@
     GinGradArgs a;
     a.params = d_params; a.spk = reinterpret_cast<const int*>(ws + lo.w_spk);
     a.S = reinterpret_cast<const long long*>(ws + lo.w_gsum); a.gfx = gfx; a.grads = d_grads;
-    a.offs = reinterpret_cast<const long long*>(ws + lo.w_tables);
+    a.fx_offs = reinterpret_cast<const long long*>(ws + lo.w_fx_offs);
     a.p_k = lo.p_g_k[0]; a.p_b = lo.p_g_b[0]; a.p_stride = lo.layer_stride; a.p_emb = lo.p_emb;
     a.L = lo.L; a.B = lo.B; a.G = lo.G; a.Gi = lo.Gi; a.NS = lo.NS;
     gin_wgrad_kernel<<<grid1d((long long)lo.L * lo.G), 256, 0, st>>>(a); t2_count_launch();
@@ -1542,7 +1865,7 @@
     rc = launch_wgrad(maps, 6, reinterpret_cast<const WgradTile*>(ws + lo.w_tiles_main), lo.n_tiles_main, d_grads, lo.T, lo.B, st);
     if (rc) return rc;
   }
-  first_conv_bwd_kernel<<<dim3((unsigned)((BT + 63) / 64)), lo.R, 0, sb>>>(d_x, lo.scalar_in ? 1 : 0, dxin, gfx + lo.p_in_k, BT, lo.R); t2_count_launch();
+  first_conv_bwd_kernel<<<dim3((unsigned)((BT + 63) / 64)), lo.R, 0, sb>>>(d_x, lo.scalar_in ? 1 : 0, dxin, gfx + lo.fxo(lo.p_in_k), BT, lo.R); t2_count_launch();
   T2_CHECK_CUDA(cudaGetLastError());
   if (lo.C > 0 && !cfg->c_pre_upsampled) {
     float* dcup = reinterpret_cast<float*>(ws + lo.w_dcup);
@@ -1565,7 +1888,7 @@
       const int W = lo.up_w[i] / s;
       const float* layer_in = i == 0 ? d_c : reinterpret_cast<const float*>(ws + lo.w_upout[i - 1]);
       const float* out = reinterpret_cast<const float*>(ws + lo.w_upout[i]);
-      rc = launch_upsample_bwd_param(layer_in, out, dout, gfx + lo.p_up_k[i], gfx + lo.p_up_b[i], lo.B, lo.C, W, s, cfg->upsample_type,
+      rc = launch_upsample_bwd_param(layer_in, out, dout, gfx + lo.fxo(lo.p_up_k[i]), gfx + lo.fxo(lo.p_up_b[i]), lo.B, lo.C, W, s, cfg->upsample_type,
                                      cfg->upsample_activation, cfg->leaky_alpha, sb);
       if (rc) return rc;
       if (i > 0) {
@@ -1583,7 +1906,7 @@
     T2_CHECK_CUDA(cudaStreamWaitEvent(st, side->join, 0));
   }
   if (phase == -1) {
-    const int rc = launch_fx_finalize(gfx, d_grads, lo.n_params, st);
+    const int rc = launch_fx_store(lo, ws, d_grads, st);
     if (rc) return rc;
   }
   return T2_OK;
diff --git a/tacotron-2_b200/wavenet.py b/tacotron-2_b200/wavenet.py
--- a/tacotron-2_b200/wavenet.py
+++ b/tacotron-2_b200/wavenet.py
@@ -203,7 +203,7 @@
             assert t.numel() == n, "%s: expected %s got %s" % (name, shape, tuple(params[name].shape))
             flat[off:off + n] = t
         self.params.copy_(flat.to(self.device))
-        self._packed_dirty = True
+        self.pack()
 
     def init_variables(self, seed=None):
         from . import init
@@ -284,7 +284,6 @@
             self._graph = torch.cuda.CUDAGraph()
             with torch.cuda.graph(self._graph):
                 self.step_dev.add_(1)
-                self.pack()
                 self.forward(x, c, targets, lengths)
                 self.backward()
         else:
@@ -294,7 +293,6 @@
                 with torch.cuda.graph(gr, pool=pool):
                     if g == 0:
                         self.step_dev.add_(1)
-                        self.pack()
                         self.forward(x, c, targets, lengths)
                         self.backward(0, G)
                         self.backward(100, G)
@@ -377,16 +375,16 @@
             self.ema = self.params.clone()
         lr = self.learning_rate()
         clip = hp.wavenet_clip_gradients
-        L.check(self.lib.t2_adam_step(
-            L.ptr(self.params), L.ptr(self.grads), L.ptr(self.m), L.ptr(self.v), L.ptr(self.ema),
-            L.ptr(self.offsets), len(self.tensors), ctypes.c_longlong(self.n_params), ctypes.c_float(lr),
+        L.check(self.lib.t2_wn_optimizer_step(
+            ctypes.byref(self.cfg), L.ptr(self.params), L.ptr(self.grads), L.ptr(self.m), L.ptr(self.v), L.ptr(self.ema),
+            L.ptr(self.packed), L.ptr(self.workspace), ctypes.c_float(lr),
             ctypes.c_float(hp.wavenet_adam_beta1), ctypes.c_float(hp.wavenet_adam_beta2),
             ctypes.c_float(hp.wavenet_adam_epsilon), self.global_step + 1, ctypes.c_float(grad_scale),
             ctypes.c_float(hp.wavenet_gradient_max_norm if clip else 0.0),
-            ctypes.c_float(hp.wavenet_gradient_max_value if clip else 0.0), ctypes.c_float(0.0),
+            ctypes.c_float(hp.wavenet_gradient_max_value if clip else 0.0),
             ctypes.c_float(hp.wavenet_ema_decay), L.ptr(self.opt_scratch), L.stream_ptr()))
         self.global_step += 1
-        self._packed_dirty = True
+        self._packed_dirty = False
         return lr
 
     def workspace_tensor(self, name, shape=None):
```
